# alex-petrenko/megaverse

Hardware: AMD Instinct MI355X
Metric: agent observations/sec (whole node), TowerBuilding 128x128 obs, random policy (higher is better)
Workload: dtype f32

## Files before the change

### include/megaverse_hip.h

```cpp
#ifndef MEGAVERSE_HIP_H
#define MEGAVERSE_HIP_H

#include <stdint.h>

#ifdef __cplusplus
extern "C" {
#endif

typedef struct mv_gym mv_gym;

typedef struct mv_config {
    const char *scenario;
    int32_t obs_width, obs_height;
    int32_t num_envs;
    int32_t num_agents_per_env;
    int32_t num_simulation_threads;
    int32_t use_vulkan;
    int32_t device;
    const char *const *param_keys;
    const float *param_vals;
    int32_t num_params;
    int32_t env_offset, total_envs;
    int32_t env_stride;
} mv_config;
// ... 81 lines not shown
int mv_get_pixel_mode(const mv_gym *g);

enum { MV_OBS_RGBA = 0, MV_OBS_RGB_PLANAR = 1 };
int mv_set_obs_layout(mv_gym *g, int32_t layout);
int mv_get_obs_layout(const mv_gym *g);

int mv_set_pipelining(mv_gym *g, int32_t on);
int mv_get_pipelining(const mv_gym *g);

int mv_set_render_resolution(mv_gym *g, int32_t w, int32_t h);
int mv_draw_hires(mv_gym *g);
int mv_get_hires_observation(mv_gym *g, int32_t env_idx, int32_t agent_idx, uint8_t *out_host);
int mv_draw_overview(mv_gym *g);

int mv_num_reward_shaping_keys(const mv_gym *g);
const char *mv_reward_shaping_key(const mv_gym *g, int32_t i);
int mv_get_reward_shaping(mv_gym *g, int32_t env_idx, int32_t agent_idx, const char *key, float *out);
int mv_set_reward_shaping(mv_gym *g, int32_t env_idx, int32_t agent_idx, const char *key, float value);

int mv_synchronize(mv_gym *g);

typedef struct mv_episode_record {
    int32_t agent;
    int32_t length;
    uint32_t end_tick;
    float true_objective;
    double ret;
} mv_episode_record;
int mv_set_episode_log(mv_gym *g, int32_t capacity);
int mv_get_episode_log_capacity(const mv_gym *g);
int mv_flush_episode_log(mv_gym *g);
int mv_episode_log_count(mv_gym *g, uint32_t *count, uint32_t *dropped);
int mv_drain_episode_log(mv_gym *g, mv_episode_record *out_host, int32_t max_records, uint32_t *dropped);
void *mv_episode_log_records_device_ptr(mv_gym *g);
void *mv_episode_log_count_device_ptr(mv_gym *g);
void *mv_episode_returns_device_ptr(mv_gym *g);
void *mv_episode_lengths_device_ptr(mv_gym *g);
int64_t mv_ticks_since_reset(const mv_gym *g);

int mv_profile_begin(mv_gym *g, int32_t max_steps);
int mv_profile_end(mv_gym *g, float *avg_ms4, int32_t *counts4);

int mv_debug_set_agent_pos(mv_gym *g, int32_t env_idx, int32_t agent_idx, float x, float y, float z);
int mv_debug_launch_counts(mv_gym *g, int64_t out[2]);
int mv_debug_set_agent_yaw(mv_gym *g, int32_t env_idx, int32_t agent_idx, float c, float s);
int mv_debug_set_agent_velocity(mv_gym *g, int32_t env_idx, int32_t agent_idx, float hvx, float hvz, float vvel);
int mv_debug_snapshot_size(const mv_gym *g);
int mv_debug_snapshot(mv_gym *g, int32_t env_idx, void *out_host);
int mv_debug_boxagone_state(mv_gym *g, int32_t env_idx, void *out_host);
int mv_debug_football_state(mv_gym *g, int32_t env_idx, void *out_host);
int mv_debug_set_football_state(mv_gym *g, int32_t env_idx, const void *in_host);
int mv_debug_rng(int32_t device, uint32_t seed, int32_t what, const int32_t *lo, const int32_t *hi, int32_t n, void *out_host);
int mv_debug_math(int32_t device, int32_t what, const float *a, const float *b, int32_t n, float *out_host);
int mv_debug_generate_episode(const char *scenario, int32_t num_agents, int32_t env_seed, int32_t n, float base_episode_len,
                              void *out, int32_t out_bytes);
int mv_debug_feeder_selftest(const char *scenario, int32_t num_envs, int32_t num_agents, int32_t threads, int32_t rounds);
int mv_debug_generate_sokoban(int32_t num_agents, int32_t env_seed, int32_t n, float base_episode_len, void *out, int32_t out_bytes);
int mv_debug_generate_football(int32_t num_agents, int32_t env_seed, int32_t n, float base_episode_len, void *out, int32_t out_bytes);

int mv_debug_collect_draw_host(int32_t num_agents, int32_t env_seed, int32_t n, float base_episode_len, void *out, int32_t out_bytes);
int mv_debug_episode_log_host(const float *rewards, const uint8_t *dones, const float *true_objectives, int32_t k, int32_t N, int32_t A, int32_t capacity,
                              uint32_t first_tick, double *ret, int32_t *len, void *records, uint32_t *count, uint32_t *dropped);
int mv_debug_episode_log_masked_host(const float *rewards, const uint8_t *dones, const float *true_objectives, int32_t k, int32_t N, int32_t A,
                                     int32_t capacity, uint32_t first_tick, double *ret, int32_t *len, void *records, uint32_t *count, uint32_t *dropped,
                                     const uint8_t *step_mask );
int mv_debug_episode_log_budget_host(const float *rewards, const uint8_t *dones, const float *true_objectives, int32_t k, int32_t N, int32_t A,
                                     int32_t capacity, uint32_t first_tick, double *ret, int32_t *len, void *records, uint32_t *count, uint32_t *dropped,
                                     const uint8_t *step_mask , int32_t *left );
int mv_debug_episode_budget_host(const uint8_t *dones, const uint8_t *mask, const int32_t *left_in, int32_t k, int32_t N, uint8_t *steps_out,
                                 int32_t *left_out);
int mv_debug_episode_log_cut_host(const uint8_t *mask, int32_t N, int32_t A, double *ret, int32_t *len);
int mv_debug_fork_plan_host(const int32_t *src_of, int32_t N, int32_t *resolved , int32_t *invalid );
int mv_debug_resample_plan_host(const int32_t *src_of, int32_t N, int32_t *resolved , int32_t *staged ,
                                int32_t *invalid );
int mv_debug_resample_apply_host(const int32_t *src_of, int32_t N, int32_t bytes_per_env, uint8_t *state, int32_t order);
int mv_debug_env_store_plan_host(const int32_t *slot_of, int32_t N, int32_t slots, int32_t is_save, int32_t *resolved , int32_t *invalid );
int64_t mv_debug_env_record_layout_host(const uint32_t *array_bytes, int32_t count, int32_t A, uint32_t *offsets);
int mv_debug_env_record_pack_host(const uint32_t *array_bytes, int32_t count, int32_t A, uint64_t layout_word, int32_t log_on, const uint8_t *env_state_in,
                                  uint8_t *record_out);
int mv_debug_env_record_unpack_host(const uint32_t *array_bytes, int32_t count, int32_t A, uint64_t layout_word, int32_t log_on, const uint8_t *record_in,
                                    uint8_t *env_state_inout);
int mv_debug_episodes_consumed(mv_gym *g, int32_t *out_host);
int mv_debug_collect_draw_device(int32_t device, int32_t num_agents, const int32_t *env_seeds, int32_t count, int32_t n, float base_episode_len, void *out,
                                 int64_t out_bytes, float *ms_per_launch);

#ifdef __cplusplus
}
#endif
#endif
```

### megaverse_amd/csrc/mv_api.hip

```cpp
#include "mv_api_internal.h"

thread_local std::string mvapi::g_err;

static const char *SHAPING_KEYS_TOWER[4] = {"teamSpirit", "towerPickedUpObject", "towerVisitedBuildingZoneWithObject",
                                           "towerBuildingReward"};
static const float SHAPING_DEFAULT_TOWER[4] = {0.1f, 0.1f, 0.1f, 1.0f};
static const char *SHAPING_KEYS_OBST[5] = {"teamSpirit", "obstaclesAgentAtExit", "obstaclesAllAgentsAtExit", "obstaclesExtraReward",
                                          "obstaclesAgentCarriedObjectToExit"};
static const float SHAPING_DEFAULT_OBST[5] = {0.0f, 1.0f, 5.0f, 0.5f, 0.0f};
static const char *SHAPING_KEYS_REARRANGE[3] = {"teamSpirit", "rearrangeOneMoreObjectCorrectPosition", "rearrangeAllObjectsCorrectPosition"};
static const float SHAPING_DEFAULT_REARRANGE[3] = {0.0f, 1.0f, 10.0f};
static const char *SHAPING_KEYS_SOKOBAN[4] = {"teamSpirit", "sokobanBoxOnTarget", "sokobanBoxLeavesTarget", "sokobanAllBoxesOnTarget"};
static const float SHAPING_DEFAULT_SOKOBAN[4] = {0.0f, 1.0f, -1.0f, 10.0f};
static const char *SHAPING_KEYS_EMPTY[1] = {"teamSpirit"};
static const char *SHAPING_KEYS_HEX_MEMORY[3] = {"teamSpirit", "memoryCollectGood", "memoryCollectBad"};
static const float SHAPING_DEFAULT_HEX_MEMORY[3] = {0.0f, 1.0f, -1.0f};
static const char *SHAPING_KEYS_HEX_EXPLORE[2] = {"teamSpirit", "exploreSolved"};
static const float SHAPING_DEFAULT_HEX_EXPLORE[2] = {0.0f, 5.0f};
static const char *SHAPING_KEYS_COLLECT[5] = {"teamSpirit", "collectSingleGood", "collectSingleBad", "collectAll", "collectAbyss"};
static const float SHAPING_DEFAULT_COLLECT[5] = {0.0f, 1.0f, -1.0f, 5.0f, -0.5f};
static const char *SHAPING_KEYS_BOXAGONE[3] = {"teamSpirit", "boxagoneTouchedFloor", "boxagonePerStepReward"};
static const float SHAPING_DEFAULT_BOXAGONE[3] = {0.0f, -0.1f, 0.01f};
static const int ACTION_SPACE[6] = {3, 3, 3, 2, 2, 3};

// ... 278 lines not shown

    mv_gym *g = new mv_gym();
    g->device = cfg->device;
    g->w = cfg->obs_width; g->h = cfg->obs_height;
    g->N = cfg->num_envs; g->A = cfg->num_agents_per_env;
    g->scenario = scenario;
    g->numShaping = scenario == SCN_TOWER || scenario == SCN_SOKOBAN ? 4 : scenario == SCN_REARRANGE || scenario == SCN_HEX_MEMORY || scenario == SCN_BOXAGONE ? 3
                  : scenario == SCN_HEX_EXPLORE ? 2 : scenario == SCN_EMPTY || scenario == SCN_FOOTBALL ? 1 : 5;
    g->shapingKeys = scenario == SCN_TOWER ? SHAPING_KEYS_TOWER : scenario == SCN_OBSTACLES ? SHAPING_KEYS_OBST
                   : scenario == SCN_COLLECT ? SHAPING_KEYS_COLLECT : scenario == SCN_SOKOBAN ? SHAPING_KEYS_SOKOBAN
                   : scenario == SCN_HEX_MEMORY ? SHAPING_KEYS_HEX_MEMORY : scenario == SCN_HEX_EXPLORE ? SHAPING_KEYS_HEX_EXPLORE
                   : scenario == SCN_EMPTY || scenario == SCN_FOOTBALL ? SHAPING_KEYS_EMPTY : scenario == SCN_BOXAGONE ? SHAPING_KEYS_BOXAGONE : SHAPING_KEYS_REARRANGE;
    g->spares = scenario == SCN_TOWER || scenario == SCN_EMPTY || scenario == SCN_FOOTBALL ? 2 : 3;
    g->envOffset = cfg->total_envs > 0 ? cfg->env_offset : 0;
    g->envStride = cfg->total_envs > 0 && cfg->env_stride > 1 ? cfg->env_stride : 1;
    g->gv.sample_on = 0; g->gv.sample_seed = g->gv.sample_step = 0;
    g->gv.env_offset = g->envOffset; g->gv.env_stride = g->envStride;
    g->totalEnvs = cfg->total_envs > 0 ? cfg->total_envs : cfg->num_envs;
    const size_t N = g->N, NA = (size_t)g->N * g->A;

    GymView &gv = g->gv;
    gv.num_envs = g->N; gv.num_agents = g->A;
    const bool obstacles = scenario == SCN_OBSTACLES || scenario == SCN_EMPTY, collect = scenario == SCN_COLLECT,
            rearrange = scenario == SCN_REARRANGE, sokoban = scenario == SCN_SOKOBAN;
    const bool hex = scenario == SCN_HEX_MEMORY || scenario == SCN_HEX_EXPLORE, boxagone = scenario == SCN_BOXAGONE, football = scenario == SCN_FOOTBALL;
    const bool hostEpisodes = obstacles || collect || rearrange || sokoban || hex || boxagone || football;
    gv.scenario = scenario;
    gv.box_stride = collect ? COLLECT_MAX_BOXES : MAX_BOXES;
    gv.reward_stride = collect ? COLLECT_MAX_REWARDS : MAX_REWARDS;
    g->blobBytes = collect ? sizeof(CollectBlob) : obstacles ? sizeof(EpisodeBlob) : rearrange ? sizeof(RearrangeBlob)
                                    : sokoban ? sizeof(SokobanBlob) : hex ? sizeof(HexBlob) : boxagone ? sizeof(BoxAGoneBlob) : football ? sizeof(FootballBlob) : sizeof(TowerBlob);
    auto up = [](size_t v) { return (v + 4095) & ~size_t(4095); };
    const size_t szHdr = up(N * sizeof(EnvHeader)), szBoxes = up(N * (size_t)gv.box_stride * sizeof(LayoutBox)),
                 szObj = up(N * MAX_OBJECTS * sizeof(MovableObject)), szAg = up(NA * sizeof(AgentState)),
                 szChunk = up(N * (size_t)CHUNK_BYTES), szAct = up(NA * sizeof(int32_t)), szRew = up(NA * sizeof(float)),
                 szDone = up(N), szObjv = up(NA * sizeof(float)), szMd = up(NA * 6 * sizeof(int32_t)),
                 szObs = up(NA * frame_bytes(g->w, g->h, MV_OBS_RGBA));
    const size_t szTerrain = obstacles ? up(N * MAX_TERRAIN * sizeof(TerrainBox)) : 0,
                 szRewObj = hostEpisodes ? up(N * (size_t)gv.reward_stride * sizeof(MovableObject)) : 0,
                 szHeight = collect ? up(N * (size_t)HM_BYTES) : 0, szItems = rearrange ? up(N * MAX_ITEMS * sizeof(ArrangementItem))
                                         : 0, szCells = sokoban ? up(N * (size_t)(SOKO_DIM * SOKO_DIM)) : 0,
                 szHexB = hex || boxagone || football ? up(N * (size_t)HEX_MAX_BOXES * sizeof(HexRec)) : 0,
                 szHexO = hex || football ? up(N * (size_t)HEX_MAX_OBJS * sizeof(HexRec)) : 0,
                 szBag = boxagone ? up(N * sizeof(BoxAGoneState)) : 0, szFb = football ? up(N * sizeof(FootballState)) : 0,
                                   szBlobs = up(N * g->blobBytes * (size_t)g->spares), szCnt = up((N + 2) * sizeof(int32_t)),
                                                szGen = hostEpisodes ? 0 : up(N * sizeof(TowerGen));
    gv.vis_stride = hex ? 2048 : collect || boxagone ? 1024 : 256;
    if (const char *e = getenv("MV_DEBUG_VIS_STRIDE")) gv.vis_stride = std::min(gv.vis_stride, std::max(8, atoi(e)));
    gv.debug_redo = getenv("MV_DEBUG_FORCE_REDO") && atoi(getenv("MV_DEBUG_FORCE_REDO")) ? 1 : 0;
    gv.spares = g->spares;
    const size_t szVisP = up(NA * (size_t)gv.vis_stride * 32), szVisR = up(NA * (size_t)gv.vis_stride * 8), szVisC = up(NA * sizeof(int32_t)),
                 szLpt = up(NA * sizeof(int32_t)) + up((NA + 1) * sizeof(int32_t)) + up(NA * (size_t)FRAME_HDR_BYTES)
                            + up((size_t)LPT_BUCKETS * LPT_SUBS * lpt_sub_capacity(NA) * sizeof(int32_t));
    const size_t szParity = szVisP + szVisR + szVisC + szLpt + szRew + szDone + szObjv;
    g->batch = (size_t)PIPE_GROUPS * 16 * szParity <= (size_t(9) << 28) ? 16 : 8;
    if (const char *e = getenv("MV_PIPE_BATCH")) g->batch = std::min((int)PIPE_BATCH_MAX, std::max(1, atoi(e)));
    g->slots = PIPE_GROUPS * g->batch;
    g->hists = g->slots + 1;
    g->histClean.assign((size_t)g->hists, 1);
    g->gvp.resize((size_t)g->slots);
    g->parity = g->slots - 1;
    g->group = PIPE_GROUPS - 1;
    const size_t szHist = up((size_t)g->hists * (LPT_BUCKETS * LPT_SUBS + 1) * sizeof(int32_t));
    gv.lpt_hists = g->hists;
    const bool depthSortOn = !(getenv("MV_DEPTH_SORT") && atoi(getenv("MV_DEPTH_SORT")) == 0);
    const size_t szSort = gv.vis_stride > 256 && depthSortOn ? up(NA * (size_t)gv.vis_stride * 40) : 0;
    const size_t total = szSort + szHdr + szBoxes + szObj + szAg + szAct + szRew + szDone + szObjv + szMd + (hostEpisodes ? 0 : szChunk) + szObs + szTerrain +
                         szRewObj + szHeight + szItems + szCells + szHexB + szHexO + szBag + szFb + szBlobs + szCnt + szGen + (size_t)g->slots * szParity + szHist;
    {
        hipError_t e_ = hipMalloc((void **)&g->arena, total);
        if (e_ != hipSuccess) {
            const int b = g->batch;
            mv_destroy(g);
            return fail("hipMalloc arena (" + std::to_string(total >> 20) + " MiB, of which "
                        + std::to_string(((size_t)PIPE_GROUPS * b * szParity) >> 20) + " MiB are the " +
                        std::to_string(PIPE_GROUPS * b) + " hand-over slots of " + std::to_string(b)
                                       + " ticks per call: a smaller MV_PIPE_BATCH shrinks them): " + hipGetErrorString(e_));
        }
        g->arenaBytes = total;
        (void)hipMemset(g->arena, 0, total);
    }
    {
        uint8_t *p = g->arena;
        gv.hdr = (EnvHeader *)p; p += szHdr;
        gv.boxes = (LayoutBox *)p; p += szBoxes;
        gv.objects = (MovableObject *)p; p += szObj;
        gv.agents = (AgentState *)p; p += szAg;
        gv.actions = (int32_t *)p; p += szAct;
        gv.rewards = (float *)p; p += szRew;
        gv.done = p; p += szDone;
        gv.true_objective = (float *)p; p += szObjv;
        g->dMultiDiscrete = (int32_t *)p; p += szMd;
        if (!hostEpisodes) { gv.chunk = p; p += szChunk; }
        g->ownedObs = (uint32_t *)p; p += szObs;
        g->dStatus = (int *)p; p += szCnt;
        gv.episode_status = g->dStatus;
        if (obstacles) { gv.terrain = (TerrainBox *)p; p += szTerrain; }
        if (hostEpisodes) { gv.rewards_obj = (MovableObject *)p; p += szRewObj; }
        g->dBlobs = p; p += szBlobs;
        gv.blobs = g->dBlobs;
        if (!hostEpisodes) { gv.tower_gen = (TowerGen *)p; p += szGen; }
        if (collect) { gv.heightmap = (int8_t *)p; p += szHeight; }
        if (rearrange) { gv.items = (ArrangementItem *)p; p += szItems; }
        if (sokoban) { gv.soko_cells = p; p += szCells; }
        if (hex) { gv.hex_boxes = (HexRec *)p; p += szHexB; gv.hex_objs = (HexRec *)p; p += szHexO; }
        if (boxagone) { gv.hex_boxes = (HexRec *)p; p += szHexB; gv.bag = (BoxAGoneState *)p; p += szBag; }
        if (football) { gv.hex_boxes = (HexRec *)p; p += szHexB; gv.hex_objs = (HexRec *)p; p += szHexO; gv.fb = (FootballState *)p; p += szFb; }
        {
            fork::Table &ft = g->forkTable;
            ft = fork::Table{};
            ft.hdr = gv.hdr;
            fork::table_add(ft, gv.boxes, (size_t)gv.box_stride * sizeof(LayoutBox));
            fork::table_add(ft, gv.objects, MAX_OBJECTS * sizeof(MovableObject));
            fork::table_add(ft, gv.agents, (size_t)g->A * sizeof(AgentState));
            fork::table_add(ft, gv.chunk, CHUNK_BYTES);
            fork::table_add(ft, gv.terrain, MAX_TERRAIN * sizeof(TerrainBox));
            fork::table_add(ft, gv.rewards_obj, (size_t)gv.reward_stride * sizeof(MovableObject));
            fork::table_add(ft, gv.heightmap, HM_BYTES);
            fork::table_add(ft, gv.items, MAX_ITEMS * sizeof(ArrangementItem));
            fork::table_add(ft, gv.soko_cells, SOKO_DIM * SOKO_DIM);
            fork::table_add(ft, gv.hex_boxes, HEX_MAX_BOXES * sizeof(HexRec));
            fork::table_add(ft, gv.hex_objs, HEX_MAX_OBJS * sizeof(HexRec));
            fork::table_add(ft, gv.bag, sizeof(BoxAGoneState));
            fork::table_add(ft, gv.fb, sizeof(FootballState));
            static_assert(13 + 2 <= fork::MAX_ARRAYS, "the table holds every per-env array and the episode log's two");
        }
        gv.lpt_hist = (int32_t *)p; p += szHist;
        gv.sort_scratch = szSort ? p : nullptr; p += szSort;
        gv.depth_sort = 0;
        for (int q = 0; q < g->slots; ++q) {
            GymView &v = g->gvp[q];
            v = gv;
            v.vis_prims = p; p += szVisP;
            v.vis_rects = p; p += szVisR;
            v.vis_count = (int32_t *)p; p += szVisC;
            v.lpt_bucket = (int32_t *)p; p += up(NA * sizeof(int32_t));
            v.lpt_order = (int32_t *)p; p += up((NA + 1) * sizeof(int32_t));
            v.vis_hdr = p; p += up(NA * (size_t)FRAME_HDR_BYTES);
            v.lpt_list = (int32_t *)p; p += up((size_t)LPT_BUCKETS * LPT_SUBS * lpt_sub_capacity(NA) * sizeof(int32_t));
            v.rewards = (float *)p; p += szRew;
            v.done = p; p += szDone;
            v.true_objective = (float *)p; p += szObjv;
        }
    }
    if (getenv("MV_TICK_TIMING") && atoi(getenv("MV_TICK_TIMING"))) {
        if (hipMalloc((void **)&g->gv.dbg, N * 64 * sizeof(unsigned long long)) == hipSuccess)
            (void)hipMemset(g->gv.dbg, 0, N * 64 * sizeof(unsigned long long));
        else g->gv.dbg = nullptr;
        for (int q = 0; q < g->slots; ++q) g->gvp[q].dbg = g->gv.dbg;
    }
    if (const char *e = getenv("MV_PIXEL_MODE")) g->fastPixels = lower(e) == "exact" ? 0 : 1;
    if (const char *e = getenv("MV_PIPELINE")) g->pipelined = atoi(e) != 0;
    g->obs = g->ownedObs;
    for (int b = 0; b < 2; ++b) {
        if (hipHostMalloc((void **)&g->hActions[b], NA * sizeof(int32_t), hipHostMallocDefault) != hipSuccess ||
            hipEventCreateWithFlags(&g->actionsCopied[b], hipEventDisableTiming) != hipSuccess) {
            mv_destroy(g);
            return fail("mv_create: pinned staging allocation failed");
        }
        std::memset(g->hActions[b], 0, NA * sizeof(int32_t));
    }
    g->hRewards.assign(NA, 0.0f); g->hTrueObj.assign(NA, 0.0f); g->hDone.assign(N, 0);

    float episodeLen = sokoban ? 80.0f : boxagone ? 300.0f : 60.0f, lookLimit = boxagone ? 0.75f : 0.2f;
    for (int k = 0; k < cfg->num_params; ++k) {
        const char *key = cfg->param_keys[k];
        const float v = cfg->param_vals[k];
        if (!std::strcmp(key, "episodeLengthSec")) episodeLen = v;
        if (!std::strcmp(key, "verticalLookLimitRad")) lookLimit = v;
        auto ip = [&](const char *name, int &dst) { if (!std::strcmp(key, name)) dst = int(std::lround(v)); };
        ip("obstaclesMinNumPlatforms", oc.min_platforms); ip("obstaclesMaxNumPlatforms", oc.max_platforms);
        ip("obstaclesMinGap", oc.min_gap); ip("obstaclesMaxGap", oc.max_gap); ip("obstaclesMinLava", oc.min_lava);
        ip("obstaclesMaxLava", oc.max_lava); ip("obstaclesMinHeight", oc.min_height); ip("obstaclesMaxHeight", oc.max_height);
        if (!std::strcmp(key, "obstaclesNumAllowedMaxDifficulty")) oc.num_allowed_max_difficulty = int(v);
    }
    g->obst = oc;
    g->baseEpisodeLen = episodeLen;
    g->envRecordLayout = env_record_layout_word(g, scen, cfg);
    {
        bool ok = hipHostMalloc((void **)&g->hStatus, (N + 2) * sizeof(int), hipHostMallocDefault) == hipSuccess &&
                  hipStreamCreateWithFlags(&g->copyStream, hipStreamNonBlocking) == hipSuccess &&
                  create_sim_stream(&g->simStream) == hipSuccess &&
                  hipEventCreateWithFlags(&g->userMark[0], hipEventDisableTiming) == hipSuccess &&
                  hipEventCreateWithFlags(&g->userMark[1], hipEventDisableTiming) == hipSuccess &&
                  hipEventCreateWithFlags(&g->userMark[2], hipEventDisableTiming) == hipSuccess &&
                  hipEventCreateWithFlags(&g->userNow, hipEventDisableTiming) == hipSuccess &&
                  hipEventCreateWithFlags(&g->simDone, hipEventDisableTiming) == hipSuccess &&
                  hipEventCreateWithFlags(&g->stepDone, hipEventDisableTiming) == hipSuccess &&
                  hipEventCreateWithFlags(&g->statusCopied, hipEventDisableTiming) == hipSuccess;
        if (!ok) {
            mv_destroy(g);
            return fail("mv_create: status staging / copy stream allocation failed");
        }
        std::memset(g->hStatus, 0, (N + 2) * sizeof(int));
    }
// ... 804 lines not shown
```

### megaverse_amd/csrc/mv_api_debug.hip

```cpp
#include "mv_api_internal.h"

__global__ void set_agent_pos_kernel(AgentState *agents, int idx, float x, float y,
                                     float z) { agents[idx].pos[0] = x; agents[idx].pos[1] = y; agents[idx].pos[2] = z; }
__global__ void set_agent_yaw_kernel(AgentState *agents, int idx, float c,
                                     float s) { agents[idx].m00 = c; agents[idx].m02 = s; agents[idx].m20 = -s; agents[idx].m22 = c; }
__global__ void set_agent_velocity_kernel(AgentState *agents, int idx, float hvx, float hvz,
                                          float vvel) { agents[idx].hvx = hvx; agents[idx].hvz = hvz; agents[idx].vvel = vvel; }

__global__ void debug_rng_kernel(uint32_t seed, int what, const int32_t *lo, const int32_t *hi, int n, void *out)
{
    __shared__ uint32_t s_mt[624];
    __shared__ uint16_t s_items[4096];
    Mt19937 g{s_mt, 624};
    mt_seed(g, seed);
    const int lane = threadIdx.x & 63;
    if (what == 0) {
        for (int i = 0; i < n; ++i) { const uint32_t v = mt_next(g); if (lane == 0) ((uint32_t *)out)[i] = v; }
    } else if (what == 1) {
        for (int i = 0; i < n; ++i) { const int v = rand_range(g, lo[i], hi[i]); if (lane == 0) ((int32_t *)out)[i] = v; }
    } else if (what == 2) {
        for (int i = 0; i < n; ++i) { const float v = frand(g); if (lane == 0) ((float *)out)[i] = v; }
    } else if (what == 3) {
        for (int i = lane; i < n; i += 64) s_items[i] = (uint16_t)i;
        __syncthreads();
// ... 326 lines not shown
int mv_debug_generate_sokoban(int32_t num_agents, int32_t env_seed, int32_t n, float base_episode_len, void *out, int32_t out_bytes)
{
    if (!out) return (int)sizeof(SokobanBlob);
    if (num_agents < 1 || num_agents > MAX_AGENTS || n < 1 || (size_t)out_bytes < (size_t)n * sizeof(SokobanBlob))
        return fail("mv_debug_generate_sokoban: bad arguments");
    const std::vector<std::string> files = find_boxoban_level_files();
    if (files.empty()) return fail("mv_debug_generate_sokoban: no Boxoban levels found (BOXOBAN_LEVELS)");
    std::mt19937 rng;
    rng.seed((unsigned long)env_seed);
    SokobanLevels levels;
    for (int i = 0; i < n; ++i)
        if (!generate_sokoban_episode(rng, levels, files, num_agents, base_episode_len, reinterpret_cast<SokobanBlob *>(out)[i]))
            return fail("mv_debug_generate_sokoban: unreadable level file");
    return n;
}

int mv_debug_rng(int32_t device, uint32_t seed, int32_t what, const int32_t *lo, const int32_t *hi, int32_t n, void *out)
{
    HIP_TRY(hipSetDevice(device));
    if (what == 3 && n > 4096) return fail("mv_debug_rng: shuffle n <= 4096");
    int32_t *dlo = nullptr, *dhi = nullptr;
    void *dout = nullptr;
    HIP_TRY(hipMalloc(&dout, (size_t)n * 4));
    if (what == 1) {
        HIP_TRY(hipMalloc((void **)&dlo, (size_t)n * 4));
        HIP_TRY(hipMalloc((void **)&dhi, (size_t)n * 4));
        HIP_TRY(hipMemcpy(dlo, lo, (size_t)n * 4, hipMemcpyHostToDevice));
        HIP_TRY(hipMemcpy(dhi, hi, (size_t)n * 4, hipMemcpyHostToDevice));
    }
    hipLaunchKernelGGL(debug_rng_kernel, dim3(1), dim3(64), 0, nullptr, seed, what, dlo, dhi, n, dout);
    HIP_TRY(hipGetLastError());
    HIP_TRY(hipMemcpy(out, dout, (size_t)n * 4, hipMemcpyDeviceToHost));
    (void)hipFree(dout); (void)hipFree(dlo); (void)hipFree(dhi);
    return 0;
}

int mv_debug_math(int32_t device, int32_t what, const float *a, const float *b, int32_t n, float *out)
{
    HIP_TRY(hipSetDevice(device));
    float *da = nullptr, *db = nullptr, *dout = nullptr;
    const size_t outN = (what == 2) ? 2 * (size_t)n : (size_t)n;
    HIP_TRY(hipMalloc((void **)&da, (size_t)n * 4));
    HIP_TRY(hipMalloc((void **)&db, (size_t)n * 4));
    HIP_TRY(hipMalloc((void **)&dout, outN * 4));
    HIP_TRY(hipMemcpy(da, a, (size_t)n * 4, hipMemcpyHostToDevice));
    HIP_TRY(hipMemcpy(db, b ? b : a, (size_t)n * 4, hipMemcpyHostToDevice));
    hipLaunchKernelGGL(debug_math_kernel, dim3((n + 255) / 256), dim3(256), 0, nullptr, what, da, db, n, dout);
    HIP_TRY(hipGetLastError());
    HIP_TRY(hipMemcpy(out, dout, outN * 4, hipMemcpyDeviceToHost));
    (void)hipFree(da); (void)hipFree(db); (void)hipFree(dout);
    return 0;
}

}
```

### megaverse_amd/csrc/mv_api_step.hip

```cpp
#include "mv_api_internal.h"

extern "C" {

enum : int { QUIET_OFF = 0, QUIET_NONE = 1, QUIET_LAST = 2 };
static int step_gyms(mv_gym *const *gs, int n, bool render, int k, int policy, uint32_t seed, uint32_t first_index, int kCall, int quiet = QUIET_OFF)
{
    mv_gym *const L = gs[0];
    int batch = L->batch;
    bool mustWait = false, allFast = true, anyHostEpisodes = false, anyLog = false;
    for (int i = 0; i < n; ++i) {
        mv_gym *g = gs[i];
        if (check(g)) return -1;
        if (!g->wasReset) return fail("mv_step: call mv_reset first");
        batch = std::min(batch, g->batch);
        mustWait = mustWait || g->simMustWaitUser;
        allFast = allFast && g->fastPixels != 0;
        anyHostEpisodes = anyHostEpisodes || g->hostEpisodes();
        anyLog = anyLog || g->logCapacity > 0;
        if (policy == POLICY_SEQUENCE && (!g->actRing || g->actRingCount < 1))
            return fail(n > 1 ? "mv_group_step: MV_POLICY_SEQUENCE: gym " + std::to_string(i) + " of the group has no action ring (mv_set_action_ring)"
                              : std::string("mv_step_n: MV_POLICY_SEQUENCE: the gym has no action ring (mv_set_action_ring)"));
    }
    if (k < 1 || k > batch) return fail("mv_step_n: 1 <= k <= " + std::to_string(batch) + " (MV_PIPE_BATCH) required");
    HIP_TRY(hipSetDevice(L->device));
// ... 51 lines not shown
    const bool profiling = render && L->profCount < L->profMax;
    hipEvent_t *callEv = nullptr;
    if (profiling && canMultiTick && canBatchRaster && k <= MAX_STEP_TICKS) {
        callEv = &L->profEvents[(size_t)L->profCount * 5];
        L->profTicks[(size_t)L->profCount] = k;
        ++L->profCount;
    }
    const bool multiTick = canMultiTick && (!profiling || callEv);
    bool groupBatch = n > 1 && !ticksOff && own && render && allFast && k >= 2 && k <= MAX_STEP_TICKS && policy != POLICY_NONE
            && !profiling && raster_union_batch_applicable(k, n, L->w, L->h);
    for (int i = 0; i < n && groupBatch; ++i) groupBatch = gs[i]->A == 1 && gs[i]->ringObs && gs[i]->ringCount >= k && !gs[i]->gv.dbg;
    {
        int envs = 0;
        for (int i = 0; i < n; ++i) envs += gs[i]->N;
        groupBatch = groupBatch && envs <= 1024;
    }
    bool sideWaits = anyHostEpisodes;
    for (int i = 0; i < n; ++i)
        sideWaits = sideWaits || (gs[i]->genStream && gs[i]->ticksSinceDraw + k >= gs[i]->drawPeriod) || gs[i]->stepsSinceStatus + k >= gs[i]->statusPeriod;
    bool stepDoneRodeAlong = false;
    for (int j = 0; j < k; ++j) {
        const bool prof = !callEv && render && L->profCount < L->profMax;
        evs[j] = prof ? &L->profEvents[(size_t)L->profCount * 5] : nullptr;
        if (prof) { L->profTicks[(size_t)L->profCount] = 1; ++L->profCount; }
        UnionStepArgs ua;
        ua.n = n;
        int envs = 0;
        for (int i = 0; i < n; ++i) {
            mv_gym *g = gs[i];
            if (policy == POLICY_SEQUENCE) g->gv.sample_on = POLICY_NONE;
            else if (policy != POLICY_NONE) { g->gv.sample_on = policy; g->gv.sample_seed = seed; g->gv.sample_step = first_index + (uint32_t)j; }
            else { g->gv.sample_on = (j == 0 && g->samplePending) ? g->samplePolicy : (int)POLICY_NONE; }
            g->parity = g->group * g->batch + j;
            if ((render || (drawLast && j == k - 1)) && take_hist(g, sim, !(multiTick || groupBatch || simTicks))) return -1;
            OutPtrs &o = outs[(size_t)j * n + i];
            o = outputs_of(g, g->ringTick++);
            GymView &v = views[(size_t)j * n + i];
            v = view(g, g->parity, staged ? nullptr : &o);
            v.step_mask = g->stepMask;
            if (g->budgetOn) { v.budget = g->budgetLeft; v.halted = g->budgetHalted; }
            if (policy == POLICY_SEQUENCE)
                v.md_actions = g->actRing + (size_t)action_ring_entry(first_index, j, (uint32_t)g->actRingCount) * ((size_t)g->N * g->A * 6);
            else if (j == 0 && g->gv.sample_on == POLICY_NONE) v.md_actions = g->mdActions;
            if (groupBatch) v.lpt_no_clear = 1;
            if (n > 1) { ua.first[i] = envs; ua.gv[i] = v; envs += g->N; }
        }
        if (evs[j]) HIP_TRY(hipEventRecord(evs[j][0], sim));
        bool simDoneRides = false;
        if (multiTick) {
            views[(size_t)j].lpt_no_clear = 1;
            if (j == k - 1) {
                if (callEv) HIP_TRY(hipEventRecord(callEv[0], sim));
                hipEvent_t rides = own && !callEv ? L->simDone : nullptr;
                const int chunkTicks = 8;
                for (int j0 = 0; j0 < k; j0 += chunkTicks) {
                    const int kk = std::min(chunkTicks, k - j0);
                    const GymView *vw = views.data() + j0;
                    hipEvent_t r = j0 + kk == k ? rides : nullptr;
                    launch_step_ticks(vw, kk, sim, L->w, L->h, r);
                    ++L->launchCount[0];
                }
                if (callEv) HIP_TRY(hipEventRecord(callEv[1], sim));
                simDoneRides = rides != nullptr;
            }
        } else if (simTicks) {
            if (drawLast && j == k - 1) views[(size_t)j].lpt_no_clear = 1;
            if (j == k - 1) {
                hipEvent_t rides = own ? L->simDone : nullptr;
                const int chunkTicks = 8;
                for (int j0 = 0; j0 < k; j0 += chunkTicks) {
                    const int kk = std::min(chunkTicks, k - j0);
                    const bool last = j0 + kk == k;
                    launch_step_ticks_sim(views.data() + j0, kk, last && drawLast ? 1u << (kk - 1) : 0u, sim, L->w, L->h, last ? rides : nullptr);
                    ++L->launchCount[0];
                }
                simDoneRides = rides != nullptr;
            }
        } else if (n == 1) {
            hipEvent_t rides = j == k - 1 && !evs[j] ? (own ? L->simDone : sideWaits ? L->stepDone : nullptr) : nullptr;
            const bool rode = launch_step(views[(size_t)j * n], sim, L->w, L->h, drawLast && j == k - 1 ? 1 : fused, rides);
            ++L->launchCount[0];
            simDoneRides = rode && own;
            stepDoneRodeAlong = rode && !own;
        }
        else if (groupBatch) {
            if (j == k - 1) {
                UnionTicksArgs ta;
                ta.n = n; ta.k = k;
                ta.act_first = first_index;
                for (int i = 0; i < n; ++i) {
                    ta.first[i] = ua.first[i];
                    ta.gv[i] = views[(size_t)i];
                    ta.slot_stride[i] = (int64_t)((const uint8_t *)views[(size_t)n + i].vis_prims - (const uint8_t *)views[(size_t)i].vis_prims);
                    const bool seq = policy == POLICY_SEQUENCE;
                    ta.act_base[i] = seq ? gs[i]->actRing : nullptr;
                    ta.act_count[i] = seq ? (uint32_t)gs[i]->actRingCount : 0u;
                    ta.act_stride[i] = gs[i]->N * gs[i]->A * 6;
                }
                for (int i = n; i <= MAX_UNION; ++i) ta.first[i] = envs;
                for (int i = n; i < MAX_UNION; ++i) {
                    ta.gv[i] = views[0]; ta.slot_stride[i] = 0;
                    ta.act_base[i] = nullptr; ta.act_count[i] = 0; ta.act_stride[i] = 0;
                }
                launch_step_union_ticks(ta, sim, L->w, L->h, own ? L->simDone : nullptr);
                ++L->launchCount[0];
                simDoneRides = own;
            }
        } else {
            for (int i = n; i <= MAX_UNION; ++i) ua.first[i] = envs;
            launch_step_union(ua, sim, L->w, L->h, fused);
            ++L->launchCount[0];
        }
        if (evs[j]) HIP_TRY(hipEventRecord(evs[j][1], sim));
        simDoneRodeAlong = simDoneRodeAlong || simDoneRides;
// ... 381 lines not shown
```

### megaverse_amd/csrc/mv_raster.h

```cpp
#pragma once
#include <hip/hip_runtime.h>

#include "mv_types.h"

namespace mv {

struct PublishTo { float *rewards; uint8_t *done; float *true_objective; };
int launch_raster(const GymView &gv, uint32_t *obs, int W, int H, hipStream_t stream, hipEvent_t between = nullptr, int fast = 1, int setup_done = 0,
                  const PublishTo *publish = nullptr, hipEvent_t done = nullptr);

int launch_raster_union(const GymView *views, uint32_t *const *obs, const PublishTo *publish, int n,
                        int W, int H, hipStream_t stream, hipEvent_t between = nullptr,
                        hipEvent_t done = nullptr);

int launch_raster_batch(const GymView *views, uint32_t *const *obs, const PublishTo *publish, int k,
                        int W, int H, hipStream_t stream, hipEvent_t done = nullptr);

bool raster_union_batch_applicable(int k, int n, int W, int H);
int launch_raster_union_batch(const GymView *views, uint32_t *const *obs, const PublishTo *publish, int k,
                              int n, int W, int H, hipStream_t stream, hipEvent_t done = nullptr);

}
```

### megaverse_amd/csrc/mv_raster.hip

```cpp
#include <hip/hip_runtime.h>
#include <hip/hip_ext.h>
#include <math.h>
#include <stdlib.h>

#include <algorithm>
#include <cstring>
#include <numeric>
#include <type_traits>
#include <vector>
#include <stdio.h>

#include "../../include/megaverse_hip.h"
#include "mv_frame.h"
#include "mv_math.h"
#include "mv_raster.h"
#include "mv_rearrange.h"
#include "mv_types.h"
#include "mv_union.h"

namespace mv {

namespace {

template <bool ANYZERO>
// ... 168 lines not shown

__device__ __forceinline__ unsigned to_u8(float v)
{
    v = fmin_sel(fmax_sel(v, 0.0f), 1.0f);
    return (unsigned)(int)(v * 255.0f + 0.5f);
}

__device__ __forceinline__ V3 safe_inv(V3 d)
{
    return v3(d.x == 0.0f ? 0.0f : 1.0f / d.x, d.y == 0.0f ? 0.0f : 1.0f / d.y, d.z == 0.0f ? 0.0f : 1.0f / d.z);
}


}


__global__ __launch_bounds__(256) void frame_setup_kernel(GymView gv, int W, int H)
{
    __shared__ FrameScratch s_fs;
    __shared__ DepthSortScratch s_ds;
    frame_setup_body<256, false>(gv, blockIdx.x, W, H, s_fs, &s_ds);
}

__global__ __launch_bounds__(1024) void frame_order_kernel(GymView gv, int frames, int *order)
{
    __shared__ int s_hist[LPT_BUCKETS], s_start[LPT_BUCKETS], s_wsum[LPT_BUCKETS / 64];
    const int tid = threadIdx.x;
    if (tid < LPT_BUCKETS) s_hist[tid] = 0;
    __syncthreads();
    for (int f = tid; f < frames; f += 1024) atomicAdd(&s_hist[gv.lpt_bucket[f]], 1);
    __syncthreads();
    {
        const int lane = tid & 63, wave = tid >> 6;
        const int b = LPT_BUCKETS - 1 - tid;
        const int h = tid < LPT_BUCKETS ? s_hist[b] : 0;
        int x = h;
#pragma unroll
        for (int off = 1; off < 64; off <<= 1) {
            const int y = __shfl_up(x, off, 64);
            if (lane >= off) x += y;
        }
        if (lane == 63 && tid < LPT_BUCKETS) s_wsum[wave] = x;
        __syncthreads();
        if (tid < LPT_BUCKETS) {
            int base = 0;
            for (int w = 0; w < wave; ++w) base += s_wsum[w];
            s_start[b] = base + x - h;
        }
    }
    __syncthreads();
    for (int f = tid; f < frames; f += 1024) order[atomicAdd(&s_start[gv.lpt_bucket[f]], 1)] = f;
}

namespace {

template <bool CHW>
struct PixOutT {
    __amdgpu_buffer_rsrc_t rsrc;
    int W, H, W4;
    bool edgeless;
    int plane;
};
typedef PixOutT<false> PixOut;
#ifndef MV_PIXEL_PLAIN
constexpr int PIXEL_AUX = 2;
#else
constexpr int PIXEL_AUX = 0;
#endif
#ifndef MV_PLANAR_PIXEL_AUX
#define MV_PLANAR_PIXEL_AUX 0
#endif
constexpr int PLANAR_AUX = MV_PLANAR_PIXEL_AUX;

template <bool CHW>
__device__ __forceinline__ PixOutT<CHW> frame_out(uint32_t *obs, int frame, int W, int H, bool edgeless)
{
    PixOutT<CHW> po;
    const unsigned bytes = CHW ? 3u * W * H : 4u * W * H;
    po.rsrc = __builtin_amdgcn_make_buffer_rsrc(reinterpret_cast<unsigned char *>(obs) + (size_t)frame * bytes,  0, (int)bytes, 0x00020000);
    po.W = W; po.H = H; po.W4 = CHW ? W : 4 * W;
    po.edgeless = edgeless;
    po.plane = W * H;
    return po;
}

__device__ __forceinline__ void put_px(const PixOut &po, int px, int py, unsigned rgba)
{
    const unsigned off = (unsigned)(__mul24(py, po.W4) + px * 4);
    if (__builtin_expect(po.edgeless, 1)) __builtin_amdgcn_raw_buffer_store_b32(rgba, po.rsrc, off, 0, PIXEL_AUX);
    else {
        asm volatile("" ::: "memory");
        if (px < po.W && py < po.H) __builtin_amdgcn_raw_buffer_store_b32(rgba, po.rsrc, off, 0, PIXEL_AUX);
    }
}

__device__ __forceinline__ unsigned quad_transpose_bytes(unsigned x, int q)
{
    const unsigned y = (unsigned)__builtin_amdgcn_mov_dpp((int)x, 0x4e, 0xf, 0xf, false);
    const unsigned s = __builtin_amdgcn_perm(y, x, q < 2 ? 0x05040100u : 0x03020706u);
    const unsigned z = (unsigned)__builtin_amdgcn_mov_dpp((int)s, 0xb1, 0xf, 0xf, false);
    return __builtin_amdgcn_perm(z, s, (q & 1) ? 0x03070105u : 0x06020400u);
}

__device__ __forceinline__ void put_px(const PixOutT<true> &po, int px, int py, unsigned rgba)
{
    const unsigned row = (unsigned)__mul24(py, po.W);
    if ((po.W & 3) == 0) {
        const int q = px & 3;
        const unsigned t = quad_transpose_bytes(rgba, q);
        const unsigned off = (unsigned)__mul24(q, po.plane) + row + (unsigned)(px - q);
        if (q < 3 && (po.edgeless || (px < po.W && py < po.H))) __builtin_amdgcn_raw_buffer_store_b32(t, po.rsrc, off, 0, PLANAR_AUX);
        return;
    }
    if (px < po.W && py < po.H) {
        const unsigned off = row + (unsigned)px;
        __builtin_amdgcn_raw_buffer_store_b8((unsigned char)rgba, po.rsrc, off, 0, PLANAR_AUX);
        __builtin_amdgcn_raw_buffer_store_b8((unsigned char)(rgba >> 8), po.rsrc, off + (unsigned)po.plane, 0, PLANAR_AUX);
        __builtin_amdgcn_raw_buffer_store_b8((unsigned char)(rgba >> 16), po.rsrc, off + 2u * (unsigned)po.plane, 0, PLANAR_AUX);
    }
}

}

template <int MAXVIS, bool SHAPES, bool CHW = false>
__global__ __launch_bounds__(256, MAXVIS <= 256 && !SHAPES ? MV_RASTER_WAVES : MAXVIS <= 256 ? 5 : MAXVIS <= 1024 ? 2
                             : 1) void raster_kernel(GymView gv, uint32_t *obs, int W, int H, int split, const int *order)
{
    constexpr int ROUNDS = MAXVIS / 64;
    extern __shared__ __attribute__((aligned(16))) unsigned char s_dyn[];
    __shared__ Prim s_vis[MAXVIS];
    __shared__ short4 s_rect[MAXVIS];
    __shared__ CamL s_cam[MAX_CAMS];
    __shared__ float s_lutA[256], s_lutD[256];

    float4 *s_col = reinterpret_cast<float4 *>(s_dyn);
    float4 *s_row = s_col + W;
    float *s_colinv = reinterpret_cast<float *>(s_row + H);
    float *s_rowinv = s_colinv + W;

    const int A = gv.num_agents;
    int frame, part;
    {
// ... 186 lines not shown
                unsigned ch[3];
#pragma unroll
                for (int c = 0; c < 3; ++c) {
                    const unsigned byte = (q.color >> (16 - 8 * c)) & 255u;
                    ch[c] = to_u8((s_lutA[byte] + s_lutD[byte] * intensity) + spec);
                }
                rgba = ch[0] | (ch[1] << 8) | (ch[2] << 16) | 0xff000000u;
            }
            const int py = pyBase + TILE_H * k;
            if constexpr (CHW) put_px(frame_out<true>(obs, frame, W, H, false), px, py, rgba);
            else if (px < W && py < H) out[(size_t)py * W + px] = rgba;
        }
    }
}

namespace {

#ifndef MV_GLIST_WAVES_NP2
#define MV_GLIST_WAVES_NP2 5
#endif
#ifndef MV_GLIST_WAVES_NP1
#define MV_GLIST_WAVES_NP1 6
#endif
constexpr int GLIST_WAVES_NP2 = MV_GLIST_WAVES_NP2, GLIST_WAVES_NP1 = MV_GLIST_WAVES_NP1;
#ifndef MV_FAST_PPL_DEFAULT
#define MV_FAST_PPL_DEFAULT 2
#endif
constexpr float SPEC_COS2 = 0.97f * 0.97f;

#ifndef MV_PIXEL_PLAIN
#define PIXEL_STORE(dst, v) __builtin_nontemporal_store((uint32_t)(v), &(dst))
#else
#define PIXEL_STORE(dst, v) ((dst) = (v))
#endif

struct FastArgs {
    const unsigned char *vis_hdr;
    const Prim *vis_prims;
    const short4 *vis_rects;
    const int *hist, *list;
    int num_agents, vis_stride, frames;
    const float *stage_rewards, *stage_true;
    const uint8_t *stage_done;
    float *pub_rewards, *pub_true;
    uint8_t *pub_done;
    int pub_n;
#ifdef MV_RASTER_TIMING
    unsigned long long *rdbg;
#endif
    int *hist_done;
    int wg_total;
    int tail_div, tail_split;
    int planar;
};

__device__ __forceinline__ void fast_publish(const FastArgs &fa, int blk)
{
    if (fa.pub_n == 0) return;
    const int i = blk * (int)blockDim.x + (int)threadIdx.x;
    if (i >= fa.pub_n) return;
    fa.pub_rewards[i] = fa.stage_rewards[i];
    const int e = i / fa.num_agents;
    if (fa.stage_done[e]) fa.pub_true[i] = fa.stage_true[i];
    if (i < fa.pub_n / fa.num_agents) fa.pub_done[i] = fa.stage_done[i];
}

__device__ __forceinline__ unsigned long long uniform_u64(unsigned long long v)
{
    const unsigned lo = (unsigned)__builtin_amdgcn_readfirstlane((unsigned)v), hi = (unsigned)__builtin_amdgcn_readfirstlane((unsigned)(v >> 32));
    return ((unsigned long long)hi << 32) | lo;
}

__device__ __forceinline__ float uniform_f32(float v)
{
    return __uint_as_float(__builtin_amdgcn_readfirstlane(__float_as_uint(v)));
}

typedef __attribute__((address_space(3))) const float lds_float;
__device__ __forceinline__ lds_float *local_lds(const float *p)
{
    lds_float *q = (lds_float *)p;
    asm volatile("" : "+v"(q));
    return q;
}
__device__ __forceinline__ V3 lds_tmul(lds_float *m, V3 v)
{
    return v3((m[0] * v.x + m[3] * v.y) + m[6] * v.z, (m[1] * v.x + m[4] * v.y) + m[7] * v.z, (m[2] * v.x + m[5] * v.y) + m[8] * v.z);
}
__device__ __forceinline__ V3 lds_mul(lds_float *m, V3 v)
{
    return v3((m[0] * v.x + m[1] * v.y) + m[2] * v.z, (m[3] * v.x + m[4] * v.y) + m[5] * v.z, (m[6] * v.x + m[7] * v.y) + m[8] * v.z);
}

constexpr unsigned KEY_NEAR = 0x3c23d70au;
constexpr unsigned KEY_FAR = 0x42f00000u - KEY_NEAR;
static_assert(NEAR_Z == 0.01f && FAR_Z == 120.0f, "update KEY_NEAR / KEY_FAR");

template <unsigned POS_MASK>
__device__ __forceinline__ unsigned box_key(V3 inv, const float4 lo, const float4 hi, int pos, unsigned depthMask = ~POS_MASK)
{
    const float t1x = lo.x * inv.x, t2x = hi.x * inv.x, t1y = lo.y * inv.y, t2y = hi.y * inv.y, t1z = lo.z * inv.z, t2z = hi.z * inv.z;
    const float tn = __builtin_fmaxf(__builtin_fmaxf(__builtin_fminf(t1x, t2x), __builtin_fminf(t1y, t2y)), __builtin_fminf(t1z, t2z));
    const float tf = __builtin_fminf(__builtin_fminf(__builtin_fmaxf(t1x, t2x), __builtin_fmaxf(t1y, t2y)), __builtin_fmaxf(t1z, t2z));
    const unsigned key = ((__float_as_uint(tn) - KEY_NEAR) & depthMask) | (unsigned)pos;
    return tn <= tf ? key : ~0u;
}
template <unsigned POS_MASK>
__device__ __forceinline__ unsigned hit_key(bool hit, float t, int pos)
{
    return hit ? (((__float_as_uint(t) - KEY_NEAR) & ~POS_MASK) | (unsigned)pos) : ~0u;
}

__device__ __forceinline__ bool fast_box(V3 inv, const float4 lo, const float4 hi, float &t_out)
{
    const float t1x = lo.x * inv.x, t2x = hi.x * inv.x, t1y = lo.y * inv.y, t2y = hi.y * inv.y, t1z = lo.z * inv.z, t2z = hi.z * inv.z;
    const float tn = __builtin_fmaxf(__builtin_fmaxf(__builtin_fminf(t1x, t2x), __builtin_fminf(t1y, t2y)), __builtin_fminf(t1z, t2z));
    const float tf = __builtin_fminf(__builtin_fminf(__builtin_fmaxf(t1x, t2x), __builtin_fmaxf(t1y, t2y)), __builtin_fmaxf(t1z, t2z));
    t_out = tn;
// ... 86 lines not shown
            const int axis = tnx == t ? 0 : tny == t ? 1 : 2;
            const float dk = axis == 0 ? d.x : axis == 1 ? d.y : d.z;
            const float lk = s_hdr[FH_LREL + 4 * qfr + axis];
            nv = t * __builtin_fabsf(dk);
            ndl = nv - __uint_as_float(__float_as_uint(lk) ^ (__float_as_uint(dk) & 0x80000000u));
        } else {
            t = tkey;
            V3 N;
            lds_float *cc = local_lds(camv + 3);
            if (!SHAPES || qkind < PRIM_SPHERE_S || qfr == 0) N = lds_tmul(cc, bn);
            else if (qfr == 1 + viewer) N = bn;
            else N = lds_tmul(cc, lds_mul(local_lds(s_hdr + FH_CAM + FH_CAM_STRIDE * (qfr - 1) + 3), bn));
            const V3 P = dc * t;
            nv = -dot(N, P);
            ndl = dot(N, v3(0.0f - P.x, 4.0f - P.y, 2.0f - P.z));
        }
        rgba = phong_tail(t, ndl, nv, a2, ldc, float((color >> 16) & 255u), float((color >> 8) & 255u), float(color & 255u));
    }
    return rgba;
}

template <bool SHAPES, unsigned POS_MASK>
__device__ __forceinline__ unsigned fast_shade(unsigned best, V3 bn, const float4 *s_vis, const float *s_hdr, const float *camv,
                                               int viewer, V3 dw, V3 inv, float dcx, float dcy, float a2, float ldc)
{
    unsigned rgba = 0xff000000u;
    if (best <= (KEY_FAR | POS_MASK)) {
        const int pos = (int)(best & POS_MASK);
        rgba = shade_rec<SHAPES>(s_vis[2 * pos], s_vis[2 * pos + 1], __uint_as_float((best & ~POS_MASK) + KEY_NEAR),
                                 bn, s_hdr, camv, viewer, dw, inv, dcx, dcy, a2, ldc);
    }
    return rgba;
}

struct FastFrame { int frame, part, viewer, nVis, split; };

__host__ __device__ inline int tail_frames(int frames, int div) { return (frames / div) & ~7; }

template <int MAXVIS, bool GLIST = false, int NT = 256>
__device__ __forceinline__ FastFrame fast_prologue(const FastArgs &fa, int blk, int W, int H, int split,
                                                   float4 *s_vis, short4 *s_rect, float *s_hdr, float4 *s_col,
                                                   float4 *s_row, float2 *s_rowq, float *s_colq, unsigned char *s_cls = nullptr)
{
    const int A = fa.num_agents;
    const int tid = threadIdx.x, lane = tid & 63, wave = __builtin_amdgcn_readfirstlane(tid >> 6);
    int position, part;
    {
        int b = blk, first = 0, frames = fa.frames;
        if (fa.tail_div) {
            const int q = tail_frames(frames, fa.tail_div), head = frames - q;
            if (b < split * head) frames = head;
            else { b -= split * head; first = head; split = fa.tail_split; frames = q; }
        }
        const int per = 8 * split, group = b / per, r = b - group * per;
        position = group * 8 + (r & 7); part = r >> 3;
        if (group * 8 + 8 > frames) { const int nf = frames - group * 8; position = group * 8 + r % nf; part = r / nf; }
        position += first;
    }
    __shared__ int s_wsum[4], s_frame, s_lastWG;
    {
        static_assert(LPT_SUBS == 4, "the bin's counters are read as one int4");
        const bool binThread = NT == 256 || tid < LPT_BUCKETS;
        const int4 c0 = binThread ? *reinterpret_cast<const int4 *>(fa.hist + (LPT_BUCKETS - 1 - tid) * LPT_SUBS) : make_int4(0, 0, 0, 0);
        const int h = (c0.x + c0.y) + (c0.z + c0.w);
        int x = h;
#pragma unroll
        for (int off = 1; off < 64; off <<= 1) {
            const int y = __shfl_up(x, off, 64);
            if (lane >= off) x += y;
        }
        if (lane == 63 && binThread) s_wsum[wave] = x;
        __syncthreads();
        int base = 0;
        for (int w = 0; w < wave && w < 4; ++w) base += s_wsum[w];
        const int end = base + x, start = end - h;
        if (binThread && position >= start && position < end) {
            const int cs[LPT_SUBS] = {c0.x, c0.y, c0.z, c0.w};
            int off = position - start, sub = 0;
#pragma unroll
            for (int q = 0; q < LPT_SUBS - 1; ++q)
                if (sub == q && off >= cs[q]) { off -= cs[q]; sub = q + 1; }
            s_frame = fa.list[(size_t)((LPT_BUCKETS - 1 - tid) * LPT_SUBS + sub) * lpt_sub_capacity(fa.frames) + off];
        }
        __syncthreads();
    }
#ifdef MV_HIST_FENCE
    if (tid == 0) s_lastWG = fa.hist_done != nullptr && __hip_atomic_fetch_add(fa.hist_done, 1, __ATOMIC_ACQ_REL, __HIP_MEMORY_SCOPE_AGENT) == fa.wg_total - 1;
#else
    if (tid == 0) s_lastWG = fa.hist_done != nullptr && __hip_atomic_fetch_add(fa.hist_done, 1, __ATOMIC_RELAXED, __HIP_MEMORY_SCOPE_AGENT) == fa.wg_total - 1;
#endif
    const int frame = __builtin_amdgcn_readfirstlane(s_frame);
    const int viewer = frame % A;
    const float *gh = reinterpret_cast<const float *>(fa.vis_hdr + (size_t)frame * FRAME_HDR_BYTES);
    const int nVis = __builtin_amdgcn_readfirstlane(min(__float_as_int(gh[FH_COUNT]), (int)MAXVIS));

    if (tid < FH_FLOATS) s_hdr[tid] = gh[tid];
    {
        const float4 *src = reinterpret_cast<const float4 *>(fa.vis_prims + (size_t)frame * fa.vis_stride);
        if (!GLIST) for (int i = tid; i < nVis * 2; i += NT) s_vis[i] = src[i];
        else
            for (int i = tid; i < nVis; i += NT) {
                const unsigned ml = __float_as_uint(reinterpret_cast<const float *>(src)[8 * i + 3]);
                const unsigned fl = (ml >> 4) & 15u;
                s_cls[i] = (ml & 15u) != (unsigned)PRIM_BOX ? 4 : fl == 0u ? 0 : fl > (unsigned)MAX_AGENTS ? (unsigned char)(fl - (unsigned)MAX_AGENTS) : 4;
            }
        const short4 *rs = fa.vis_rects + (size_t)frame * fa.vis_stride;
        for (int i = tid; i < nVis; i += NT) s_rect[i] = rs[i];
        const float *c = gh + FH_CAM + FH_CAM_STRIDE * viewer + 3;
        for (int i = tid; i < W; i += NT) {
            const float dcx = (((float(i) + 0.5f) / float(W)) * 2.0f - 1.0f) * TAN_HALF_FOV;
            s_col[i] = make_float4(dcx, c[0] * dcx, c[3] * dcx, c[6] * dcx);
            s_colq[i] = dcx * dcx;
        }
        for (int j = tid; j < H; j += NT) {
            const float dcy = (((float(j) + 0.5f) / float(H)) * 2.0f - 1.0f) * TAN_HALF_FOV_Y;
            s_row[j] = make_float4(dcy, c[1] * dcy, c[4] * dcy, c[7] * dcy);
            s_rowq[j] = make_float2(dcy * dcy + 1.0f, 4.0f * dcy - 2.0f);
        }
    }
    __syncthreads();
    if (s_lastWG) {
        int *h = const_cast<int *>(fa.hist);
        for (int i = tid; i < LPT_BUCKETS * LPT_SUBS; i += NT) h[i] = 0;
        if (tid == 0) __hip_atomic_store(fa.hist_done, 0, __ATOMIC_RELAXED, __HIP_MEMORY_SCOPE_AGENT);
    }

    return FastFrame{frame, part, viewer, nVis, split};
}

template <unsigned POS_MASK, int SGN>
__device__ __forceinline__ unsigned box_key_signed(V3 inv, const float4 lo, const float4 hi, int pos, unsigned depthMask)
{
    const float nx = (SGN & 1) ? hi.x : lo.x, fx = (SGN & 1) ? lo.x : hi.x, ny = (SGN & 2) ? hi.y : lo.y, fy = (SGN & 2)
                      ? lo.y : hi.y, nz = (SGN & 4) ? hi.z : lo.z, fz = (SGN & 4) ? lo.z : hi.z;
    const float tn = __builtin_fmaxf(__builtin_fmaxf(nx * inv.x, ny * inv.y), nz * inv.z);
    const float tf = __builtin_fminf(__builtin_fminf(fx * inv.x, fy * inv.y), fz * inv.z);
    const unsigned key = ((__float_as_uint(tn) - KEY_NEAR) & depthMask) | (unsigned)pos;
    return tn <= tf ? key : ~0u;
}

template <unsigned POS_MASK, int NP, int SGN = -1>
__device__ __forceinline__ void box_run(unsigned long long m, int k, const V3 (&inv)[NP], const float4 *s_vis, unsigned (&best)[NP])
{
    if (!m) return;
    int p0 = __ffsll((long long)m) - 1 + 64 * k, p1 = 0;
    m &= m - 1;
    float4 lo0 = s_vis[2 * p0], hi0 = s_vis[2 * p0 + 1], lo1 = lo0, hi1 = hi0;
    unsigned depthMask = ~POS_MASK;
    asm volatile("" : "+v"(depthMask));
    for (;;) {
        bool more = m != 0ull;
        if (more) { p1 = __ffsll((long long)m) - 1 + 64 * k; m &= m - 1; lo1 = s_vis[2 * p1]; hi1 = s_vis[2 * p1 + 1]; }
#pragma unroll
        for (int j = 0; j < NP; ++j) best[j] = min(best[j], SGN >= 0 ? box_key_signed<POS_MASK, (SGN >= 0 ? SGN : 0)>(inv[j], lo0, hi0, p0, depthMask)
             : box_key<POS_MASK>(inv[j], lo0, hi0, p0, depthMask));
        if (!more) break;
        more = m != 0ull;
        if (more) { p0 = __ffsll((long long)m) - 1 + 64 * k; m &= m - 1; lo0 = s_vis[2 * p0]; hi0 = s_vis[2 * p0 + 1]; }
#pragma unroll
        for (int j = 0; j < NP; ++j) best[j] = min(best[j], SGN >= 0 ? box_key_signed<POS_MASK, (SGN >= 0 ? SGN : 0)>(inv[j], lo1, hi1, p1, depthMask)
             : box_key<POS_MASK>(inv[j], lo1, hi1, p1, depthMask));
        if (!more) break;
    }
}

}

constexpr float PLANAR_MARGIN = 2e-4f;
enum : unsigned { TC_EMPTY = 0, TC_PLANAR = 1, TC_PLANAR_SPEC = 2, TC_OVERLAY = 3, TC_GENERAL = 4 };
constexpr int CLS_MAX_TILES = 128;

template <int TH, int NT>
__device__ __forceinline__ void classify_tiles(uint4 *s_tile, float4 *s_line, const float4 *s_vis, const short4 *s_rect,
                                               const float *s_hdr, const float *camv, int nVis, unsigned long long wb0,
                                               int W, int H, int part, int split, int tilesX, int numTiles,
                                                       int perWG, bool overlayOn, int *s_cnt, unsigned *s_txy, bool bulkClear)
{
    constexpr int NW = NT / 64;
    constexpr int PPR = 16 / NW;
    const int tid = threadIdx.x, lane = tid & 63, wave = __builtin_amdgcn_readfirstlane(tid >> 6);
    if (tid < CLS_MAX_TILES) s_tile[tid] = make_uint4(0u, 0u, 0u, 0u);
    if (tid < 8) s_cnt[tid] = 0;
    const float sx = 2.0f * TAN_HALF_FOV / float(W), ox = (1.0f / float(W) - 1.0f) * TAN_HALF_FOV;
    const float sy = 2.0f * TAN_HALF_FOV_Y / float(H), oy = (1.0f / float(H) - 1.0f) * TAN_HALF_FOV_Y;
    const int q = lane & 15, es = lane >> 4;
    const int ek = min(q >> 2, 2);
    int em = ek + 1 + ((q >> 1) & 1);
    em = em >= 3 ? em - 3 : em;
    const bool ehi = q & 1, eactive = q < 12;
    const float Ak = camv[3 + 3 * ek] * sx, Bk = camv[4 + 3 * ek] * sy, Ck = (camv[3 + 3 * ek] * ox + camv[4 + 3 * ek] * oy) - camv[5 + 3 * ek];
    const float Am = camv[3 + 3 * em] * sx, Bm = camv[4 + 3 * em] * sy, Cm = (camv[3 + 3 * em] * ox + camv[4 + 3 * em] * oy) - camv[5 + 3 * em];
    float4 *myLines = s_line + 16 * PPR * wave;
    constexpr float WX = float(TILE_W - 1), WY = float(TH - 1);
    __syncthreads();
    constexpr int CH = CLS_MAX_TILES / 64;
    int tX0[CH], tY0[CH], tX1[CH], tY1[CH];
    bool tvalid[CH];
    unsigned mlo[CH], mhi[CH], cover[CH];
#pragma unroll
    for (int c = 0; c < CH; ++c) {
        const int u = 64 * c + lane;
        const int tile = ((u >> 2) * split + part) * 4 + (u & 3);
        tvalid[c] = u < perWG && tile < numTiles;
        const int tyi = tile / tilesX, txi = tile - tyi * tilesX;
        tX0[c] = txi * TILE_W; tY0[c] = tyi * TH;
        tX1[c] = min(tX0[c] + TILE_W, W) - 1; tY1[c] = min(tY0[c] + TH, H) - 1;
        mlo[c] = mhi[c] = cover[c] = 0u;
    }
    for (int base = PPR * wave; base < nVis; base += 16) {
        const int P = min(base + min(es, PPR - 1), nVis - 1);
        const bool isBox = es < PPR && base + es < nVis && ((wb0 >> P) & 1ull) != 0ull;
        const float4 lo4 = s_vis[2 * P], hi4 = s_vis[2 * P + 1];
        const float lok = ek == 0 ? lo4.x : ek == 1 ? lo4.y : lo4.z, hik = ek == 0 ? hi4.x : ek == 1 ? hi4.y : hi4.z;
        const float lom = em == 0 ? lo4.x : em == 1 ? lo4.y : lo4.z, him = em == 0 ? hi4.x : em == 1 ? hi4.y : hi4.z;
        const float bnd = ehi ? him : lom;
        const bool cand = isBox && eactive && (lok > 0.0f || hik < 0.0f);
        const float pk = lok > 0.0f ? lok : hik;
        const float far1 = (__builtin_fmaxf(__builtin_fabsf(lo4.x), __builtin_fabsf(hi4.x)) + __builtin_fmaxf(__builtin_fabsf(lo4.y), __builtin_fabsf(hi4.y))) +
                           __builtin_fmaxf(__builtin_fabsf(lo4.z), __builtin_fabsf(hi4.z));
        const bool coverOK = cand && __builtin_fabsf(pk) >= 4.0f * NEAR_Z && far1 <= 0.5f * FAR_Z;
        const float sg = ((pk > 0.0f) != ehi) ? 1.0f : -1.0f;
        const float ea = sg * (pk * Am - bnd * Ak), eb = sg * (pk * Bm - bnd * Bk), ec = sg * (pk * Cm - bnd * Ck);
        const float mg = PLANAR_MARGIN * (__builtin_fabsf(pk) + __builtin_fabsf(bnd));
        const float cin = ((ec + __builtin_fminf(0.0f, ea * WX)) + __builtin_fminf(0.0f, eb * WY)) - mg;
        const float span = (__builtin_fabsf(ea) * WX + __builtin_fabsf(eb) * WY) + 2.0f * mg;
        if (es < PPR) myLines[lane] = cand ? make_float4(ea, eb, cin, span) : make_float4(0.0f, 0.0f, -1.0f, 0.0f);
        const unsigned long long candMask = __ballot(cand), coverMask = __ballot(coverOK);
        __builtin_amdgcn_fence(__ATOMIC_RELEASE, "wavefront");
        __builtin_amdgcn_wave_barrier();
        __builtin_amdgcn_fence(__ATOMIC_ACQUIRE, "wavefront");
#pragma unroll
        for (int sl = 0; sl < PPR; ++sl) {
            const int Q = base + sl;
            if (Q >= nVis) break;
            const uint2 rr = *reinterpret_cast<const uint2 *>(&s_rect[Q]);
            const bool worldBox = (wb0 >> Q) & 1ull;
#pragma unroll
            for (int c = 0; c < CH; ++c) {
                if (64 * c >= perWG) break;
                const bool ov = tvalid[c] & ((int)(rr.x & 0xffffu) <= tX1[c]) & ((int)(rr.x >> 16) >= tX0[c])
                                             & ((int)(rr.y & 0xffffu) <= tY1[c]) & ((int)(rr.y >> 16) >= tY0[c]);
                if (!__any(ov)) continue;
                bool hit = ov;
                unsigned cov = 0u;
                if (worldBox) {
                    const float fx0 = float(tX0[c]), fy0 = float(tY0[c]);
                    bool missAll = true;
#pragma unroll
                    for (int f = 0; f < 3; ++f) {
                        if (!((candMask >> (16 * sl + 4 * f)) & 1ull)) continue;
                        bool ins = true, mis = false;
#pragma unroll
                        for (int e = 0; e < 4; ++e) {
                            const float4 L = myLines[16 * sl + 4 * f + e];
                            const float g = __builtin_fmaf(L.x, fx0, __builtin_fmaf(L.y, fy0, L.z));
                            ins = ins && g >= 0.0f;
                            mis = mis || g + L.w <= 0.0f;
                        }
                        if (ins && ((coverMask >> (16 * sl + 4 * f)) & 1ull)) cov = (unsigned)f + 1u;
// ... 45 lines not shown
                        const float plane = lok > 0.0f ? lok : hik;
                        const float m0 = k == 0 ? 2.0f * plane - L0 : L0, m1 = k == 1 ? 2.0f * plane - L1 : L1, m2 = k == 2 ? 2.0f * plane - L2 : L2;
                        const float xc = float(tX0[c]) + 0.5f * WX, yc = float(tY0[c]) + 0.5f * WY;
                        const float dcx = sx * xc + ox, dcy = sy * yc + oy;
                        const float d0 = (camv[3] * dcx + camv[4] * dcy) - camv[5], d1 = (camv[6] * dcx + camv[7] * dcy) - camv[8],
                                          d2 = (camv[9] * dcx + camv[10] * dcy) - camv[11];
                        const float dot = (d0 * m0 + d1 * m1) + d2 * m2;
                        const float dd = (d0 * d0 + d1 * d1) + d2 * d2, mm = (m0 * m0 + m1 * m1) + m2 * m2;
                        maybe = dot > 0.0f && dot * dot >= cosT2 * (dd * mm);
                    }
                    info = (maybe ? (unsigned)TC_PLANAR_SPEC : (unsigned)TC_PLANAR) | ((unsigned)k << 3) | ((unsigned)pos << 5);
                } else if ((others & nonBox) == 0ull && overlayOn) info = (unsigned)TC_OVERLAY | ((unsigned)k << 3) | ((unsigned)pos << 5);
            }
            if (info == TC_GENERAL) {
                const float xa = float(tX0[c]), xb = float(tX1[c]), ya = float(tY0[c]), yb = float(tY1[c]);
                unsigned sg = 8u;
#pragma unroll
                for (int a = 0; a < 3; ++a) {
                    const float Aa = camv[3 + 3 * a] * sx, Ba = camv[4 + 3 * a] * sy, Ca = (camv[3 + 3 * a] * ox + camv[4 + 3 * a] * oy) - camv[5 + 3 * a];
                    const float v00 = __builtin_fmaf(Aa, xa, __builtin_fmaf(Ba, ya, Ca)), v10 = __builtin_fmaf(Aa, xb, __builtin_fmaf(Ba, ya, Ca));
                    const float v01 = __builtin_fmaf(Aa, xa, __builtin_fmaf(Ba, yb, Ca)), v11 = __builtin_fmaf(Aa, xb, __builtin_fmaf(Ba, yb, Ca));
                    const float lo4 = __builtin_fminf(__builtin_fminf(v00, v10), __builtin_fminf(v01, v11)),
                                                      hi4 = __builtin_fmaxf(__builtin_fmaxf(v00, v10), __builtin_fmaxf(v01, v11));
                    if (hi4 < -1e-4f) sg |= 1u << a;
                    else if (!(lo4 > 1e-4f)) sg = 0u;
                    if (sg == 0u) break;
                }
                info |= sg << 11;
            }
            s_tile[u].w = info;
            const unsigned tclass = info & 7u, cat = tclass == TC_GENERAL ? 0u : tclass == TC_OVERLAY ? 1u
                    : tclass == TC_PLANAR_SPEC ? 2u : tclass == TC_PLANAR ? 3u : 4u;
            const bool runs = tclass == TC_PLANAR || tclass == TC_PLANAR_SPEC || (tclass == TC_EMPTY && !bulkClear);
            const unsigned txy = (unsigned)tX0[c] | ((unsigned)tY0[c] << 16);
            const unsigned prevInfo = (unsigned)__shfl_up((int)info, 1, 64), prevTxy = (unsigned)__shfl_up((int)txy, 1, 64);
            const bool natHead = !runs || lane == 0 || prevInfo != info || prevTxy + (unsigned)TILE_W != txy;
            const unsigned long long nat = __ballot(natHead), below = nat & ((2ull << lane) - 1ull);
            const int posInRun = lane - (63 - __clzll((long long)below));
            const bool head = natHead || (posInRun & 7) == 0;
            const unsigned long long heads = __ballot(head), valid = __ballot(true), above = lane < 63 ? heads >> (lane + 1) : 0ull;
            const int nextHead = above ? lane + __ffsll((long long)above) : 64;
            const int len = min(nextHead, (int)__popcll(valid)) - lane;
            s_tile[u].z = head ? cat | ((unsigned)len << 3) | ((unsigned)atomicAdd(&s_cnt[cat], 1) << 7) : 7u;
            s_txy[u] = txy;
        }
        __syncthreads();
    }
}

template <int NP, bool SPEC, class PO>
__device__ __forceinline__ void planar_run(int pos, int k, int n, const float4 *s_vis, const float *s_hdr, const float4 *s_col, const float4 *s_row,
                                           const float2 *s_rowq, const float *s_colq, float nzk, int tx0, int ty0, int lane, const PO &po)
{
    const int W = po.W, H = po.H;
    const float lok = uniform_f32(reinterpret_cast<const float *>(s_vis)[8 * pos + k]),
                                  hik = uniform_f32(reinterpret_cast<const float *>(s_vis)[8 * pos + 4 + k]);
    const float plane = lok > 0.0f ? lok : hik;
    const unsigned color = (unsigned)__builtin_amdgcn_readfirstlane(__float_as_uint(reinterpret_cast<const float *>(s_vis)[8 * pos + 7]));
    const float cr = float((color >> 16) & 255u), cg = float((color >> 8) & 255u), cb = float(color & 255u);
    const float lk = uniform_f32(s_hdr[FH_LREL + k]);
    const float lks = plane > 0.0f ? lk : 0.0f - lk;
    int lpx = lane;
    asm volatile("" : "+v"(lpx));
    const int lx = lpx & (TILE_W - 1), py0 = ty0 + lpx / TILE_W;
    float rowk[NP];
    float2 rq[NP];
#pragma unroll
    for (int j = 0; j < NP; ++j) {
        const int pyc = min(py0 + TILE_H * j, H - 1);
        rowk[j] = reinterpret_cast<const float *>(s_row)[4 * pyc + 1 + k];
        rq[j] = s_rowq[pyc];
    }
#pragma unroll 1
    for (int q = 0; q < n; ++q) {
        const int px = tx0 + TILE_W * q + lx, pxc = min(px, W - 1);
        const float colk = reinterpret_cast<const float *>(s_col)[4 * pxc + 1 + k];
        const float cq = s_colq[pxc];
#pragma unroll
        for (int j = 0; j < NP; ++j) {
            const float dk = (colk + rowk[j]) + nzk;
            const float t = plane * __builtin_amdgcn_rcpf(dk);
            const float nv = t * __builtin_fabsf(dk);
            const unsigned rgba = phong_tail<SPEC>(t, nv - lks, nv, cq + rq[j].x, rq[j].y, cr, cg, cb);
            put_px(po, px, py0 + TILE_H * j, rgba);
        }
    }
}

template <int NP, bool SPEC, class PO>
__device__ __forceinline__ void planar_tile(int pos, int k, const float4 *s_vis, const float *s_hdr, const float4 *s_col, const float4 *s_row,
                                            const float2 *s_rowq, const float *s_colq, float nzk, int px, int py0, const PO &po)
{
    const int W = po.W, H = po.H;
    const float lok = uniform_f32(reinterpret_cast<const float *>(s_vis)[8 * pos + k]),
                                  hik = uniform_f32(reinterpret_cast<const float *>(s_vis)[8 * pos + 4 + k]);
    const float plane = lok > 0.0f ? lok : hik;
    const unsigned color = (unsigned)__builtin_amdgcn_readfirstlane(__float_as_uint(reinterpret_cast<const float *>(s_vis)[8 * pos + 7]));
    const float cr = float((color >> 16) & 255u), cg = float((color >> 8) & 255u), cb = float(color & 255u);
    const float lk = uniform_f32(s_hdr[FH_LREL + k]);
    const float lks = plane > 0.0f ? lk : 0.0f - lk;
    const int pxc = min(px, W - 1);
    const float colk = reinterpret_cast<const float *>(s_col)[4 * pxc + 1 + k];
    const float cq = s_colq[pxc];
#pragma unroll
    for (int j = 0; j < NP; ++j) {
        const int py = py0 + TILE_H * j, pyc = min(py, H - 1);
        const float rowk = reinterpret_cast<const float *>(s_row)[4 * pyc + 1 + k];
        const float2 rq = s_rowq[pyc];
        const float dk = (colk + rowk) + nzk;
        const float t = plane * __builtin_amdgcn_rcpf(dk);
        const float nv = t * __builtin_fabsf(dk);
        const unsigned rgba = phong_tail<SPEC>(t, nv - lks, nv, cq + rq.x, rq.y, cr, cg, cb);
        put_px(po, px, py, rgba);
    }
}

typedef unsigned v4u_t __attribute__((ext_vector_type(4)));
template <int NP>
__device__ __forceinline__ void clear_tile(const PixOut &po, int tx0, int ty0, int lane)
{
    constexpr int TH = TILE_H * NP;
    unsigned c = 0xff000000u;
    asm volatile("" : "+v"(lane), "+v"(c));
    if ((po.W & 3) == 0 && tx0 + TILE_W <= po.W) {
        const int row = ty0 + (lane >> 2), col = tx0 + 4 * (lane & 3);
        const v4u_t v = {c, c, c, c};
        if (lane < 4 * TH && row < po.H) __builtin_amdgcn_raw_buffer_store_b128(v, po.rsrc, (unsigned)(__mul24(row, po.W4) + col * 4), 0, PIXEL_AUX);
        return;
    }
    const int px = tx0 + (lane & (TILE_W - 1)), py0 = ty0 + lane / TILE_W;
#pragma unroll
    for (int j = 0; j < NP; ++j) {
        const int py = py0 + TILE_H * j;
        if (px < po.W && py < po.H) __builtin_amdgcn_raw_buffer_store_b32(c, po.rsrc, (unsigned)(__mul24(py, po.W4) + px * 4), 0, PIXEL_AUX);
    }
}
template <int NP>
__device__ __forceinline__ void clear_tile(const PixOutT<true> &po, int tx0, int ty0, int lane)
{
    constexpr int TH = TILE_H * NP;
    if ((po.W & 15) == 0 && tx0 + TILE_W <= po.W) {
        const int c = lane / TH, row = ty0 + (lane - c * TH);
        const v4u_t z = {0u, 0u, 0u, 0u};
        if (c < 3 && row < po.H)
            __builtin_amdgcn_raw_buffer_store_b128(z, po.rsrc, (unsigned)(__mul24(c, po.plane) + __mul24(row, po.W) + tx0), 0, PLANAR_AUX);
        return;
    }
    const int px = tx0 + (lane & (TILE_W - 1)), py0 = ty0 + lane / TILE_W;
#pragma unroll
    for (int j = 0; j < NP; ++j) put_px(po, px, py0 + TILE_H * j, 0xff000000u);
}

template <bool SHAPES, unsigned POS_MASK, int NP, class PO>
__device__ __forceinline__ void overlay_tile(int posA, int k, unsigned long long rest, const float4 *s_vis,
                                             const float *s_hdr, const float *camv, int viewer, const float4 *s_col,
                                             const float4 *s_row, const float2 *s_rowq, const float *s_colq,
                                                     float nzm0, float nzm1, float nzm2, int px, int py0, const PO &po)
{
    const int W = po.W, H = po.H;
    const float lok = uniform_f32(reinterpret_cast<const float *>(s_vis)[8 * posA + k]),
                                  hik = uniform_f32(reinterpret_cast<const float *>(s_vis)[8 * posA + 4 + k]);
    const float plane = lok > 0.0f ? lok : hik;
    const unsigned color = (unsigned)__builtin_amdgcn_readfirstlane(__float_as_uint(reinterpret_cast<const float *>(s_vis)[8 * posA + 7]));
    const float cr = float((color >> 16) & 255u), cg = float((color >> 8) & 255u), cb = float(color & 255u);
    const float lk = uniform_f32(s_hdr[FH_LREL + k]);
    const float lks = plane > 0.0f ? lk : 0.0f - lk;
    const int pxc = min(px, W - 1);
    const float4 cx = s_col[pxc];
    const float cq = s_colq[pxc];
#pragma unroll
    for (int j = 0; j < NP; ++j) {
        const int py = py0 + TILE_H * j, pyc = min(py, H - 1);
        const float4 ry = s_row[pyc];
        const float2 rq = s_rowq[pyc];
        const V3 dw = v3((cx.y + ry.y) + nzm0, (cx.z + ry.z) + nzm1, (cx.w + ry.w) + nzm2);
        const float dk = k == 0 ? dw.x : k == 1 ? dw.y : dw.z;
        const float t = plane * __builtin_amdgcn_rcpf(dk);
        const unsigned keyA = ((__float_as_uint(t) - KEY_NEAR) & ~POS_MASK) | (unsigned)posA;
        unsigned best = keyA;
        unsigned long long m = rest;
        while (m) {
            const int pos = __ffsll((long long)m) - 1;
            m &= m - 1;
            const float4 lo = s_vis[2 * pos], hi = s_vis[2 * pos + 1];
            const int qfr = (int)((__builtin_amdgcn_readfirstlane(__float_as_uint(lo.w)) >> 4) & 15);
            float tb;
            const bool hit = other_box(lo, hi, qfr, s_hdr, viewer, dw, cx.x, ry.x, tb);
            best = min(best, hit_key<POS_MASK>(hit, tb, pos));
        }
        const float a2 = cq + rq.x, ldc = rq.y;
        unsigned rgba;
        if (best == keyA) {
            const float nv = t * __builtin_fabsf(dk);
            rgba = phong_tail<true>(t, nv - lks, nv, a2, ldc, cr, cg, cb);
        } else rgba = fast_shade<SHAPES, POS_MASK>(best, v3(0.0f, 0.0f, 0.0f), s_vis, s_hdr, camv, viewer, dw, v3(0.0f, 0.0f, 0.0f), cx.x, ry.x, a2, ldc);
        put_px(po, px, py, rgba);
    }
}

template <bool SHAPES, unsigned POS_MASK, int NP, class PO>
__device__ __forceinline__ void general_tile(unsigned long long mv0, unsigned long long wb0, unsigned signs, const float4 *s_vis,
                                             const float *s_hdr, const float *camv, int viewer, const float4 *s_col,
                                             const float4 *s_row, const float2 *s_rowq, const float *s_colq,
                                                     float nzm0, float nzm1, float nzm2, int px, int py0, const PO &po)
{
    const int W = po.W, H = po.H;
    const int pxc = min(px, W - 1);
    const float4 cx = s_col[pxc];
    const float cq = s_colq[pxc];
    const float dcx = cx.x;
    V3 dw[NP], inv[NP], bn[NP];
    float dcy[NP], a2[NP], ldc[NP];
    unsigned best[NP];
#pragma unroll
    for (int j = 0; j < NP; ++j) {
        const int pyc = min(py0 + TILE_H * j, H - 1);
        const float4 ry = s_row[pyc];
        const float2 rq = s_rowq[pyc];
        dcy[j] = ry.x;
        dw[j] = v3((cx.y + ry.y) + nzm0, (cx.z + ry.z) + nzm1, (cx.w + ry.w) + nzm2);
        inv[j] = v3(__builtin_amdgcn_rcpf(dw[j].x), __builtin_amdgcn_rcpf(dw[j].y), __builtin_amdgcn_rcpf(dw[j].z));
        a2[j] = cq + rq.x; ldc[j] = rq.y;
        bn[j] = v3(0.0f, 0.0f, 0.0f);
        best[j] = ~0u;
    }
    const unsigned long long wbm = mv0 & wb0;
    switch (signs) {
    case 8: box_run<POS_MASK, NP, 0>(wbm, 0, inv, s_vis, best); break;
    case 9: box_run<POS_MASK, NP, 1>(wbm, 0, inv, s_vis, best); break;
    case 10: box_run<POS_MASK, NP, 2>(wbm, 0, inv, s_vis, best); break;
    case 11: box_run<POS_MASK, NP, 3>(wbm, 0, inv, s_vis, best); break;
    case 12: box_run<POS_MASK, NP, 4>(wbm, 0, inv, s_vis, best); break;
    case 13: box_run<POS_MASK, NP, 5>(wbm, 0, inv, s_vis, best); break;
    case 14: box_run<POS_MASK, NP, 6>(wbm, 0, inv, s_vis, best); break;
    case 15: box_run<POS_MASK, NP, 7>(wbm, 0, inv, s_vis, best); break;
    default: box_run<POS_MASK, NP>(wbm, 0, inv, s_vis, best); break;
    }
    unsigned long long rest = mv0 & ~wb0;
    while (rest) {
        const int pos = __ffsll((long long)rest) - 1;
        rest &= rest - 1;
#pragma unroll
        for (int j = 0; j < NP; ++j) {
            V3 n = v3(0, 0, 0);
            const unsigned key = fast_other<SHAPES, POS_MASK>(pos, s_vis, s_hdr, camv, viewer, dw[j], dcx, dcy[j], n);
            if (key < best[j]) { best[j] = key; bn[j] = n; }
        }
    }
#pragma unroll
    for (int j = 0; j < NP; ++j) {
        const unsigned rgba = fast_shade<SHAPES, POS_MASK>(best[j], bn[j], s_vis, s_hdr, camv, viewer, dw[j], inv[j], dcx, dcy[j], a2[j], ldc[j]);
        put_px(po, px, py0 + TILE_H * j, rgba);
    }
}

constexpr int fast_lds_bytes(int maxvis) { return 40 * maxvis + 4 * FH_FLOATS; }
constexpr int glist_lds_bytes(int maxvis) { return 9 * maxvis + 4 * FH_FLOATS; }

#ifdef MV_RASTER_TIMING
#define RT_COUNT(i, n) do { const unsigned long long n_ = (unsigned long long)(n); if (fa.rdbg && lane == 0) atomicAdd(fa.rdbg + (size_t)16384 * 4 * 8 + (i), n_); } while (0)
#else
#define RT_COUNT(i, n) do { } while (0)
#endif
template <bool SHAPES, unsigned POS_MASK, int NP, bool LISTED, class PO>
__device__ __forceinline__ void classified_tile(const FastArgs &fa, const int u, const int tx0, const int ty0, const uint4 *s_tile,
                                                const float4 *s_vis, const float *s_hdr, const float *camv, int viewer,
                                            const float4 *s_col, const float4 *s_row, const float2 *s_rowq,
                                                    const float *s_colq, float nzm0, float nzm1, float nzm2, unsigned long long wb0,
                                            int lane, const PO &po)
{
    const unsigned info = (unsigned)__builtin_amdgcn_readfirstlane(s_tile[u].w), tclass = info & 7u;
    const int run = LISTED ? (int)(((unsigned)__builtin_amdgcn_readfirstlane(s_tile[u].z) >> 3) & 15u) : 1;
    RT_COUNT(0, run);
    if (tclass == TC_EMPTY) {
        RT_COUNT(1, run);
        for (int q = 0; q < run; ++q) clear_tile<NP>(po, tx0 + TILE_W * q, ty0, lane);
        return;
    }
    if (LISTED && tclass <= TC_PLANAR_SPEC) {
        const int k = (int)((info >> 3) & 3u), posA = (int)(info >> 5);
        const float nzk = k == 0 ? nzm0 : k == 1 ? nzm1 : nzm2;
        RT_COUNT(2, run);
        RT_COUNT(12, tclass == TC_PLANAR ? run : 0);
        if (tclass == TC_PLANAR) planar_run<NP, false>(posA, k, run, s_vis, s_hdr, s_col, s_row, s_rowq, s_colq, nzk, tx0, ty0, lane, po);
        else planar_run<NP, true>(posA, k, run, s_vis, s_hdr, s_col, s_row, s_rowq, s_colq, nzk, tx0, ty0, lane, po);
        return;
    }
    int lpx = lane;
    asm volatile("" : "+v"(lpx));
    const int px = tx0 + (lpx & (TILE_W - 1)), py0 = ty0 + lpx / TILE_W;
    if (tclass <= TC_OVERLAY) {
#if defined(MV_RASTER_DEBUG_SKIP) && MV_RASTER_DEBUG_SKIP == 3
        return;
#endif
        const int k = (int)((info >> 3) & 3u), posA = (int)(info >> 5);
        const float nzk = k == 0 ? nzm0 : k == 1 ? nzm1 : nzm2;
        RT_COUNT(2, tclass != TC_OVERLAY);
        RT_COUNT(12, tclass == TC_PLANAR);
        RT_COUNT(13, tclass == TC_OVERLAY);
        if (tclass == TC_PLANAR) planar_tile<NP, false>(posA, k, s_vis, s_hdr, s_col, s_row, s_rowq, s_colq, nzk, px, py0, po);
        else if (tclass == TC_PLANAR_SPEC) planar_tile<NP, true>(posA, k, s_vis, s_hdr, s_col, s_row, s_rowq, s_colq, nzk, px, py0, po);
        else {
            const uint2 tm = *reinterpret_cast<const uint2 *>(&s_tile[u]);
            const unsigned long long others = (((unsigned long long)(unsigned)__builtin_amdgcn_readfirstlane(tm.y) << 32)
                                               | (unsigned)__builtin_amdgcn_readfirstlane(tm.x)) & ~wb0;
            overlay_tile<SHAPES, POS_MASK, NP>(posA, k, others, s_vis, s_hdr, camv, viewer, s_col, s_row, s_rowq, s_colq, nzm0, nzm1, nzm2, px, py0, po);
        }
        return;
    }
#if defined(MV_RASTER_DEBUG_SKIP) && MV_RASTER_DEBUG_SKIP == 2
    return;
#endif
    const uint2 tm = *reinterpret_cast<const uint2 *>(&s_tile[u]);
    const unsigned long long mv0 = ((unsigned long long)(unsigned)__builtin_amdgcn_readfirstlane(tm.y) << 32) | (unsigned)__builtin_amdgcn_readfirstlane(tm.x);
    RT_COUNT(4, 1);
    RT_COUNT(5, __popcll(mv0 & wb0));
    RT_COUNT(6, __popcll(mv0 & ~wb0));
    general_tile<SHAPES, POS_MASK, NP>(mv0, wb0, fa.planar == 3 ? 0u : (info >> 11) & 15u, s_vis, s_hdr, camv,
                                       viewer, s_col, s_row, s_rowq, s_colq, nzm0, nzm1, nzm2, px, py0, po);
}

template <int MAXVIS, bool SHAPES, bool HEXF, int NP, bool CLS = true, int NT = 256, bool CHW = false>
__device__ __forceinline__ void raster_fast_body(const FastArgs &fa, uint32_t *obs, int W, int H, int split, int blk, unsigned char *lds)
{
    constexpr unsigned POS_MASK = MAXVIS - 1;
    constexpr int TH = TILE_H * NP;
    extern __shared__ __attribute__((aligned(16))) unsigned char s_dyn[];
    float4 *s_vis = reinterpret_cast<float4 *>(lds);
    short4 *s_rect = reinterpret_cast<short4 *>(lds + 32 * MAXVIS);
    float *s_hdr = reinterpret_cast<float *>(lds + 40 * MAXVIS);
    static_assert(MAXVIS / 64 <= 16, "world-box masks: 16 x 64 positions");

    float4 *s_col = reinterpret_cast<float4 *>(s_dyn);
    float4 *s_row = s_col + W;
    float2 *s_rowq = reinterpret_cast<float2 *>(s_row + H);
    float *s_colq = reinterpret_cast<float *>(s_rowq + H);

    const int tid = threadIdx.x, lane = tid & 63, wave = __builtin_amdgcn_readfirstlane(tid >> 6);
#ifdef MV_RASTER_TIMING
    unsigned long long rt_[6];
    rt_[0] = __builtin_amdgcn_s_memtime(); rt_[5] = __builtin_amdgcn_s_memrealtime();
#define RT_MARK(i) rt_[i] = __builtin_amdgcn_s_memtime()
#else
#define RT_MARK(i) do { } while (0)
#endif
    fast_publish(fa, blk);
    const FastFrame ff = fast_prologue<MAXVIS, false, NT>(fa, blk, W, H, split, s_vis, s_rect, s_hdr, s_col, s_row, s_rowq, s_colq);
    RT_MARK(1);
    const int frame = ff.frame, part = ff.part, viewer = ff.viewer, nVis = ff.nVis;
    split = ff.split;

    const float *camv = s_hdr + FH_CAM + FH_CAM_STRIDE * viewer;
    const float nzm0 = uniform_f32(-camv[3 + 2]), nzm1 = uniform_f32(-camv[3 + 5]), nzm2 = uniform_f32(-camv[3 + 8]);
    uint32_t *out = obs + (size_t)frame * W * H;
    const int tilesX = (W + TILE_W - 1) / TILE_W, tilesY = (H + TH - 1) / TH;
    const int numTiles = tilesX * tilesY;
    PixOutT<CHW> po;
    if constexpr (CHW) po = frame_out<true>(obs, frame, W, H, (W % TILE_W) == 0 && (H % TH) == 0);
    else {
        po.rsrc = __builtin_amdgcn_make_buffer_rsrc(out,  0, W * H * 4, 0x00020000);
        po.W = W; po.H = H; po.W4 = 4 * W;
        po.edgeless = (W % TILE_W) == 0 && (H % TH) == 0;
    }

    uint2 rr0 = make_uint2(0u, 0u);
    if (NP == 1) rr0 = *reinterpret_cast<const uint2 *>(&s_rect[min(lane, max(nVis - 1, 0))]);
    const unsigned long long wb0 = uniform_u64(*reinterpret_cast<const unsigned long long *>(s_hdr + FH_WB));

    constexpr bool PLANAR = !HEXF && CLS;
    static_assert(!PLANAR || (MAXVIS == 256 && CLS_MAX_TILES == 128), "classification tables: 256 edge functions + 128 tiles = 192 records");
    float4 *s_line = s_vis + 2 * 64;
    uint4 *s_tile = reinterpret_cast<uint4 *>(s_vis + 2 * 64 + 256);
    const int perWG = (numTiles - part * 4 + 4 * split - 1) / (4 * split) * 4;
    const bool cls = PLANAR && fa.planar && nVis <= 64 && perWG <= CLS_MAX_TILES && perWG >= 32;
    __shared__ int s_next;
    __shared__ int s_cnt[8];
    __shared__ unsigned s_txy[CLS_MAX_TILES];
    __shared__ unsigned short s_order[CLS_MAX_TILES], s_empty[CLS_MAX_TILES];
    if (tid == 0) s_next = NT / 64;
    int nList = 0;
#ifndef MV_TILE_LIST
#define MV_TILE_LIST 1
#endif
    constexpr bool LISTED = PLANAR && MV_TILE_LIST != 0;
    const bool bulk = LISTED && po.edgeless && (W & 3) == 0;
    if (PLANAR && cls && !LISTED) classify_tiles<TH, NT>(s_tile, s_line, s_vis, s_rect, s_hdr, camv, nVis, wb0, W, H,
        part, split, tilesX, numTiles, perWG, fa.planar != 2, s_cnt, s_txy, true);
    else if (PLANAR && cls) {
        classify_tiles<TH, NT>(s_tile, s_line, s_vis, s_rect, s_hdr, camv, nVis, wb0, W, H, part, split,
                               tilesX, numTiles, perWG, fa.planar != 2, s_cnt, s_txy, bulk);
        const int c0 = s_cnt[0], c1 = s_cnt[1], c2 = s_cnt[2], c3 = s_cnt[3], nE = s_cnt[4];
        nList = __builtin_amdgcn_readfirstlane(c0 + c1 + c2 + c3 + (bulk ? 0 : nE));
        if (tid < CLS_MAX_TILES) {
            const int tile = ((tid >> 2) * split + part) * 4 + (tid & 3);
            if (tid < perWG && tile < numTiles) {
                const unsigned z = s_tile[tid].z, cat = z & 7u, place = z >> 7;
                const int base = cat == 0u ? 0 : cat == 1u ? c0 : cat == 2u ? c0 + c1 : cat == 3u ? c0 + c1 + c2 : c0 + c1 + c2 + c3;
                if (cat == 4u && bulk) s_empty[place] = (unsigned short)tid;
                else if (cat != 7u) s_order[base + (int)place] = (unsigned short)tid;
            }
        }
        __syncthreads();
        if (bulk) {
            constexpr int CPT = TH * 4;
            static_assert(NT % CPT == 0, "threads per empty tile");
            const int sub = tid % CPT;
            unsigned c = 0xff000000u;
            asm volatile("" : "+v"(c));
            const v4u_t v = {c, c, c, c};
            if constexpr (CHW) {
                const v4u_t z = {0u, 0u, 0u, 0u};
                const int c = sub / TH;
                const unsigned inoff = (unsigned)__mul24(c, po.plane) + (unsigned)__mul24(sub - c * TH, po.W);
                if (c < 3)
                    for (int e = tid / CPT; e < nE; e += NT / CPT) {
                        const unsigned txy = s_txy[s_empty[e]];
                        __builtin_amdgcn_raw_buffer_store_b128(z, po.rsrc, (unsigned)__mul24((int)(txy >> 16), po.W) + (txy & 0xffffu) + inoff, 0, PLANAR_AUX);
                    }
            } else {
            const unsigned inoff = (unsigned)__mul24(sub >> 2, po.W4) + (unsigned)(sub & 3) * 16u;
            for (int e = tid / CPT; e < nE; e += NT / CPT) {
                const unsigned txy = s_txy[s_empty[e]];
                __builtin_amdgcn_raw_buffer_store_b128(v, po.rsrc, (unsigned)__mul24((int)(txy >> 16), po.W4) + (txy & 0xffffu) * 4u + inoff, 0, PIXEL_AUX);
            }
            }
            if (wave == 0) { RT_COUNT(0, nE); RT_COUNT(1, nE); }
        }
    } else __syncthreads();
    RT_MARK(2);
#if defined(MV_RASTER_DEBUG_SKIP) && MV_RASTER_DEBUG_SKIP == 1
    return;
#endif

    int unext = 0;
    if (LISTED && cls)
        for (int it = wave; it < nList; it = __builtin_amdgcn_readfirstlane(unext)) {
            const int u = __builtin_amdgcn_readfirstlane((int)s_order[it]);
            if (lane == 0) unext = atomicAdd(&s_next, 1);
            const unsigned txy = (unsigned)__builtin_amdgcn_readfirstlane(s_txy[u]);
            classified_tile<SHAPES, POS_MASK, NP, LISTED>(fa, u, (int)(txy & 0xffffu), (int)(txy >> 16), s_tile, s_vis, s_hdr,
                                                          camv, viewer, s_col, s_row, s_rowq, s_colq, nzm0, nzm1, nzm2, wb0, lane, po);
        }
    const unsigned tilesXinv = (unsigned)((0x100000000ull + (unsigned)tilesX - 1u) / (unsigned)tilesX);
    for (int u = wave; !(LISTED && cls); u = __builtin_amdgcn_readfirstlane(unext)) {
        const int tile = ((u >> 2) * split + part) * 4 + (u & 3);
        if (tile >= numTiles) break;
        if (lane == 0) unext = atomicAdd(&s_next, 1);
        const int ty = (int)__umulhi((unsigned)tile, tilesXinv), tx = tile - ty * tilesX;
        const int tx0 = tx * TILE_W, ty0 = ty * TH;
        const int tx1 = min(tx0 + TILE_W, W) - 1, ty1 = min(ty0 + TH, H) - 1;
        if (PLANAR && !LISTED && cls) {
            classified_tile<SHAPES, POS_MASK, NP, LISTED>(fa, u, tx0, ty0, s_tile, s_vis, s_hdr, camv, viewer,
                                                          s_col, s_row, s_rowq, s_colq, nzm0, nzm1, nzm2, wb0, lane, po);
            continue;
        }
        unsigned long long mv0;
        int lpx = lane;
        asm volatile("" : "+v"(lpx));
        const int px = tx0 + (lpx & (TILE_W - 1)), py0 = ty0 + lpx / TILE_W;
        const int pxc = min(px, W - 1);
        {
            int l2 = lane;
            asm volatile("" : "+v"(l2));
            const int cpos = min(l2, max(nVis - 1, 0));
            const uint2 rr = NP == 1 ? rr0 : *reinterpret_cast<const uint2 *>(&s_rect[cpos]);
            const bool v = (lane < nVis) & ((int)(rr.x & 0xffffu) <= tx1) & ((int)(rr.x >> 16) >= tx0)
                            & ((int)(rr.y & 0xffffu) <= ty1) & ((int)(rr.y >> 16) >= ty0);
            mv0 = __ballot(v);
            RT_COUNT(3, 1);
        }
        RT_COUNT(4, 1);
        RT_COUNT(5, __popcll(mv0 & wb0));
        RT_COUNT(6, __popcll(mv0 & ~wb0));
        V3 dw[NP], inv[NP];
        V3 ih0[NP], ih1[NP], ih2[NP];
        float dcx = 0.0f, dcy[NP], a2[NP], ldc[NP];
        unsigned best[NP];
        V3 bn[NP];
#pragma unroll
        for (int j = 0; j < NP; ++j) {
            dw[j] = inv[j] = bn[j] = v3(0, 0, 0);
            ih0[j] = ih1[j] = ih2[j] = v3(0, 0, 0);
            dcy[j] = a2[j] = ldc[j] = 0.0f;
            best[j] = ~0u;
        }
        bool rayReady = false;
#pragma unroll 1
        for (int k = 0; k * 64 < nVis; ++k) {
            const int cpos = min(lane + 64 * k, nVis - 1);
            unsigned long long mvis = mv0;
            bool v = (mv0 >> lane) & 1ull;
            if (k > 0) {
                const uint2 rr = *reinterpret_cast<const uint2 *>(&s_rect[cpos]);
                v = (lane + 64 * k < nVis) & ((int)(rr.x & 0xffffu) <= tx1) & ((int)(rr.x >> 16) >= tx0)
                     & ((int)(rr.y & 0xffffu) <= ty1) & ((int)(rr.y >> 16) >= ty0);
                mvis = __ballot(v);
            }
            if (mvis == 0ull) continue;
            if (!rayReady) {
                rayReady = true;
                const float4 cx = s_col[pxc];
                const float cq = s_colq[pxc];
                dcx = cx.x;
#pragma unroll
                for (int j = 0; j < NP; ++j) {
                    const int pyc = min(py0 + TILE_H * j, H - 1);
                    const float4 ry = s_row[pyc];
                    const float2 rq = s_rowq[pyc];
                    dcy[j] = ry.x;
                    dw[j] = v3((cx.y + ry.y) + nzm0, (cx.z + ry.z) + nzm1, (cx.w + ry.w) + nzm2);
                    inv[j] = v3(__builtin_amdgcn_rcpf(dw[j].x), __builtin_amdgcn_rcpf(dw[j].y), __builtin_amdgcn_rcpf(dw[j].z));
                    a2[j] = cq + rq.x; ldc[j] = rq.y;
                    if (HEXF) {
                        const float cx8 = 0.8660254f * dw[j].x, cz8 = 0.8660254f * dw[j].z, hx5 = 0.5f * dw[j].x, hz5 = 0.5f * dw[j].z;
                        ih0[j] = v3(__builtin_amdgcn_rcpf(cx8 - hz5), inv[j].y, __builtin_amdgcn_rcpf(hx5 + cz8));
                        ih1[j] = v3(__builtin_amdgcn_rcpf(cx8 + hz5), inv[j].y, __builtin_amdgcn_rcpf(cz8 - hx5));
                        ih2[j] = v3(0.0f - inv[j].z, inv[j].y, inv[j].x);
                    }
                }
            }
            unsigned long long rest;
            if (HEXF) {
                const unsigned ml = __float_as_uint(s_vis[2 * cpos].w);
                const bool box = v && (ml & 15u) == (unsigned)PRIM_BOX;
                const unsigned fl = (ml >> 4) & 15u;
                const unsigned long long m0 = __ballot(box && fl == 0u), m1 = __ballot(box && fl == (unsigned)MAX_AGENTS + 1u),
                                         m2 = __ballot(box && fl == (unsigned)MAX_AGENTS + 2u), m3 = __ballot(box && fl == (unsigned)MAX_AGENTS + 3u);
                box_run<POS_MASK, NP>(m0, k, inv, s_vis, best);
                box_run<POS_MASK, NP>(m1, k, ih0, s_vis, best);
                box_run<POS_MASK, NP>(m2, k, ih1, s_vis, best);
                box_run<POS_MASK, NP>(m3, k, ih2, s_vis, best);
                rest = mvis & ~(m0 | m1 | m2 | m3);
            } else {
                const unsigned long long wb = k == 0 ? wb0 : uniform_u64(*reinterpret_cast<const unsigned long long *>(s_hdr + FH_WB + 2 * k));
                box_run<POS_MASK, NP>(mvis & wb, k, inv, s_vis, best);
                rest = mvis & ~wb;
            }
            while (rest) {
                const int pos = __ffsll((long long)rest) - 1 + 64 * k;
                rest &= rest - 1;
#pragma unroll
                for (int j = 0; j < NP; ++j) {
                    V3 n = v3(0, 0, 0);
                    const unsigned key = fast_other<SHAPES, POS_MASK>(pos, s_vis, s_hdr, camv, viewer, dw[j], dcx, dcy[j], n);
                    if (key < best[j]) { best[j] = key; bn[j] = n; }
                }
            }
        }
#pragma unroll
        for (int j = 0; j < NP; ++j) {
            RT_COUNT(7, __ballot(best[j] <= (KEY_FAR | POS_MASK)) != 0ull);
            RT_COUNT(8, __popcll(__ballot(best[j] <= (KEY_FAR | POS_MASK))));
            RT_COUNT(9, __ballot(best[j] <= (KEY_FAR | POS_MASK) && !((wb0 >> (best[j] & 63u)) & 1ull)) != 0ull);
            const unsigned rgba = fast_shade<SHAPES, POS_MASK>(best[j], bn[j], s_vis, s_hdr, camv, viewer, dw[j], inv[j], dcx, dcy[j], a2[j], ldc[j]);
            put_px(po, px, py0 + TILE_H * j, rgba);
        }
    }
#ifdef MV_RASTER_TIMING
    if (fa.rdbg && lane == 0 && blk < 16384 / (NT / 256)) {
// ... 205 lines not shown
#endif
            more = false;
#pragma unroll 1
            for (++k; k * 64 < nVis; ++k) {
                if (depthSorted && k < 31) {
                    const unsigned wd = (unsigned)__builtin_amdgcn_readfirstlane(__float_as_uint(s_hdr[FH_WB + k]));
                    const float floorD = __uint_as_float(((wd & 63u) + (120u << 2)) << 21) * (1.0f - 1e-4f);
                    const unsigned bound = floorD > NEAR_Z ? __float_as_uint(floorD) - KEY_NEAR : 0u;
                    bool covered = true;
#pragma unroll
                    for (int j = 0; j < NP; ++j) covered = covered && (best[j].d < bound || px >= W || py0 + GT_H * j >= H);
                    if (__all(covered)) { RT_COUNT(15, 1); break; }
                }
                RT_COUNT(11, 1);
                mvis = cull_round_g(s_rect, lane, k, nVis, tx0, tx1, ty0, ty1, cpos, v);
                if (mvis) { more = true; break; }
            }
        }
#ifdef MV_RASTER_TIMING
        RT_COUNT(9, metTotal == 1 && metWorld == 1);
        RT_COUNT(8, metTotal == 2);
        RT_COUNT(7, metTotal >= 3 && metTotal <= 5);
        RT_COUNT(6, metTotal >= 6);
#endif
#pragma unroll
        for (int j = 0; j < NP; ++j) {
            unsigned rgba = 0xff000000u;
#if defined(MV_GLIST_DEBUG_SKIP) && MV_GLIST_DEBUG_SKIP >= 1
            rgba = best[j].d ^ best[j].p;
            if (false)
#else
            if (best[j].d <= KEY_FAR)
#endif
            {
                const unsigned wpos = best[j].p & 2047u;
                const float4 lo = gp[2 * wpos], hi = gp[2 * wpos + 1];
                rgba = shade_rec<SHAPES>(lo, hi, __uint_as_float(best[j].d + KEY_NEAR), bn[j], s_hdr, camv, viewer, dw[j], inv[j], dcx, dcy[j], a2[j], ldc[j]);
            }
            RT_COUNT(3, __popcll(__ballot(best[j].d <= KEY_FAR)));
            const int py = py0 + GT_H * j;
            if constexpr (CHW) put_px(pc, px, py, rgba);
            else if (px < W && py < H) PIXEL_STORE(out[(unsigned)(py * W + px)], rgba);
        }
    }
}

template <int MAXVIS, bool SHAPES, int WAVES, bool HEXF, int NP, bool CHW = false>
__global__ __launch_bounds__(256, WAVES) void raster_glist_kernel(FastArgs fa, uint32_t *obs, int W, int H, int split)
{
    __shared__ __attribute__((aligned(16))) unsigned char s_buf[glist_lds_bytes(MAXVIS)];
    raster_glist_body<MAXVIS, SHAPES, HEXF, NP, CHW>(fa, obs, W, H, split, (int)blockIdx.x, s_buf);
}

template <int MAXVIS, bool SHAPES, int WAVES, bool HEXF = false, int NP = 1, int NT = 256, bool CHW = false>
__global__ __launch_bounds__(NT, WAVES) void raster_fast_kernel(FastArgs fa, uint32_t *obs, int W, int H, int split)
{
    __shared__ __attribute__((aligned(16))) unsigned char s_buf[fast_lds_bytes(MAXVIS)];
    raster_fast_body<MAXVIS, SHAPES, HEXF, NP, true, NT, CHW>(fa, obs, W, H, split, (int)blockIdx.x, s_buf);
}

struct UnionRasterArgs {
    int32_t n;
    int32_t first[MAX_UNION + 1];
    uint32_t *obs[MAX_UNION];
    FastArgs fa[MAX_UNION];
};

template <int MAXVIS, bool SHAPES, int WAVES, bool HEXF, int NP, bool CHW = false>
__global__ __launch_bounds__(256, WAVES) void raster_fast_union_kernel(UnionRasterArgs ua, int W, int H, int split)
{
    int s = 0;
#pragma unroll
    for (int i = 1; i < MAX_UNION; ++i)
        if (i < ua.n && (int)blockIdx.x >= ua.first[i]) s = i;
    __shared__ __attribute__((aligned(16))) unsigned char s_buf[fast_lds_bytes(MAXVIS)];
    raster_fast_body<MAXVIS, SHAPES, HEXF, NP, true, 256, CHW>(ua.fa[s], ua.obs[s], W, H, split, (int)blockIdx.x - ua.first[s], s_buf);
}

struct TicksRasterArgs {
    int32_t k, per_tick;
    int32_t hists, parity0;
    int64_t slot_stride;
    const int *hist_base;
    int *done_base;
    uint32_t *obs[MAX_STEP_TICKS];
    float *pub_rewards[MAX_STEP_TICKS];
    uint8_t *pub_done[MAX_STEP_TICKS];
    FastArgs fa;
};

__device__ __forceinline__ FastArgs ticks_raster_args(const TicksRasterArgs &a, int t)
{
    FastArgs f = a.fa;
    const int64_t d = a.slot_stride * t;
    f.vis_hdr += d;
    f.vis_prims = reinterpret_cast<const Prim *>(reinterpret_cast<const unsigned char *>(f.vis_prims) + d);
    f.vis_rects = reinterpret_cast<const short4 *>(reinterpret_cast<const unsigned char *>(f.vis_rects) + d);
    f.list = reinterpret_cast<const int *>(reinterpret_cast<const unsigned char *>(f.list) + d);
    f.stage_rewards = reinterpret_cast<const float *>(reinterpret_cast<const unsigned char *>(f.stage_rewards) + d);
    f.stage_true = reinterpret_cast<const float *>(reinterpret_cast<const unsigned char *>(f.stage_true) + d);
    f.stage_done += d;
    const int par = (a.parity0 + t) % a.hists;
    f.hist = a.hist_base + par * (LPT_BUCKETS * LPT_SUBS);
    f.hist_done = a.done_base ? a.done_base + par : nullptr;
    f.pub_rewards = a.pub_rewards[t];
    f.pub_done = a.pub_done[t];
    return f;
}

template <int MAXVIS, bool SHAPES, int WAVES, int NP, int NT = 256, bool CHW = false>
__global__ __launch_bounds__(NT, WAVES) void raster_fast_batch_kernel(TicksRasterArgs a, int W, int H, int split)
{
    int j = 0, r = (int)blockIdx.x;
    while (r >= a.per_tick) { r -= a.per_tick; ++j; }
    if (j == 0)
        for (int t = 0; t < a.k; ++t) fast_publish(ticks_raster_args(a, t), r);
    __shared__ __attribute__((aligned(16))) unsigned char s_buf[fast_lds_bytes(MAXVIS)];
    FastArgs fa = ticks_raster_args(a, j);
    fa.pub_n = 0;
    raster_fast_body<MAXVIS, SHAPES, false, NP, true, NT, CHW>(fa, a.obs[j], W, H, split, r, s_buf);
}

template <int MAXVIS, bool SHAPES, int WAVES, bool HEXF, int NP, bool CHW = false>
__global__ __launch_bounds__(256, WAVES) void raster_glist_batch_kernel(TicksRasterArgs a, int W, int H, int split)
{
    int j = 0, r = (int)blockIdx.x;
    while (r >= a.per_tick) { r -= a.per_tick; ++j; }
    if (j == 0)
        for (int t = 0; t < a.k; ++t) fast_publish(ticks_raster_args(a, t), r);
    __shared__ __attribute__((aligned(16))) unsigned char s_buf[glist_lds_bytes(MAXVIS)];
    FastArgs fa = ticks_raster_args(a, j);
    fa.pub_n = 0;
    raster_glist_body<MAXVIS, SHAPES, HEXF, NP, CHW>(fa, a.obs[j], W, H, split, r, s_buf);
}

template <int MAXVIS, bool SHAPES, int WAVES, bool HEXF, int NP, bool CHW = false>
__global__ __launch_bounds__(256, WAVES) void raster_glist_union_kernel(UnionRasterArgs ua, int W, int H, int split)
{
    int s = 0;
#pragma unroll
    for (int i = 1; i < MAX_UNION; ++i)
        if (i < ua.n && (int)blockIdx.x >= ua.first[i]) s = i;
    __shared__ __attribute__((aligned(16))) unsigned char s_buf[glist_lds_bytes(MAXVIS)];
    raster_glist_body<MAXVIS, SHAPES, HEXF, NP, CHW>(ua.fa[s], ua.obs[s], W, H, split, (int)blockIdx.x - ua.first[s], s_buf);
}

struct UnionRasterAllArgs {
    UnionRasterArgs u;
    int32_t large[MAX_UNION];
    int32_t split_small, split_large;
};

#ifndef MV_UNION_CLS
#define MV_UNION_CLS (NPS >= 2)
#endif
template <int WAVES, int NPS, bool CHW = false>
__global__ __launch_bounds__(256, WAVES) void raster_union_all_kernel(UnionRasterAllArgs a, int W, int H)
{
    int s = 0;
#pragma unroll
    for (int i = 1; i < MAX_UNION; ++i)
        if (i < a.u.n && (int)blockIdx.x >= a.u.first[i]) s = i;
    constexpr int LDS = fast_lds_bytes(VIS_SMALL) > glist_lds_bytes(VIS_XL) ? fast_lds_bytes(VIS_SMALL) : glist_lds_bytes(VIS_XL);
    __shared__ __attribute__((aligned(16))) unsigned char s_buf[LDS];
    const int blk = (int)blockIdx.x - a.u.first[s];
    if (a.large[s]) raster_glist_body<VIS_XL, true, true, 1, CHW>(a.u.fa[s], a.u.obs[s], W, H, a.split_large, blk, s_buf);
    else raster_fast_body<VIS_SMALL, true, false, NPS, MV_UNION_CLS, 256, CHW>(a.u.fa[s], a.u.obs[s], W, H, a.split_small, blk, s_buf);
}

struct UnionBatchArgs {
    int32_t n, k, per_tick;
    int32_t first[MAX_UNION + 1];
    int32_t large[MAX_UNION];
// ... 102 lines not shown
    if (!spread.empty()) fprintf(stderr, "raster timing: within a workgroup, last wave's end - first wave's end (us): mean %.1f p50 %.1f p90 %.1f max %.1f\n",
                                 std::accumulate(spread.begin(), spread.end(), 0.0) / spread.size(),
                                                 spread[spread.size() / 2], spread[spread.size() * 9 / 10], spread.back());
    {
        std::vector<std::pair<double, size_t>> byLife;
        for (size_t w = 0; w < (size_t)16384 * 4; ++w) { const unsigned long long *o = &h[w * 8]; if (o[0]) byLife.push_back({double(o[5] - o[4]) * 0.01, w}); }
        std::sort(byLife.begin(), byLife.end(), [](auto &a, auto &b) { return a.first > b.first; });
        for (size_t q = 0; q < std::min<size_t>(byLife.size(), 12); q += 1) {
            const size_t w = byLife[q].second; const unsigned long long *o = &h[w * 8];
            fprintf(stderr, "raster timing: long wave #%zu: life %.1f us (start +%.1f us), workgroup %zu of the launch, frame %llu, nVis %llu, classified "
                    "%llu, cycles prologue %llu cls %llu tiles %llu\n", q,
                    byLife[q].first, double(o[4] - r0) * 0.01, w / 4, o[7], o[6] & 0xffffffffull, o[6] >> 32, o[1] - o[0], o[2] - o[1], o[3] - o[2]);
        }
        const size_t nw = byLife.size();
        std::vector<double> sum(10, 0.0); std::vector<int> cnt(10, 0);
        size_t maxw = 0; for (auto &p : byLife) maxw = std::max(maxw, p.second);
        for (auto &p : byLife) { const int d = (int)std::min<size_t>(9, p.second * 10 / (maxw + 1)); sum[d] += p.first; ++cnt[d]; }
        fprintf(stderr, "raster timing: mean wave life by decile of the launch order (us):");
        for (int d = 0; d < 10; ++d) fprintf(stderr, " %.1f", cnt[d] ? sum[d] / cnt[d] : 0.0);
        fprintf(stderr, "  (%zu waves)\n", nw);
        {
            std::vector<double> pp(10, 0.0), pc(10, 0.0), pt(10, 0.0), ps(10, 0.0), pn(10, 0.0);
            for (auto &p : byLife) {
                const int d = (int)std::min<size_t>(9, p.second * 10 / (maxw + 1)); const unsigned long long *o = &h[p.second * 8];
                pp[d] += double(o[1] - o[0]); pc[d] += double(o[2] - o[1]); pt[d] += double(o[3] - o[2]);
                                ps[d] += double(o[4] - r0) * 0.01; pn[d] += double(o[6] & 0xffffffffull);
            }
            fprintf(stderr, "raster timing: by decile: prologue kcyc");
            for (int d = 0; d < 10; ++d) fprintf(stderr, " %.1f", cnt[d] ? pp[d] / cnt[d] / 1e3 : 0.0);
            fprintf(stderr, " | classification kcyc");
            for (int d = 0; d < 10; ++d) fprintf(stderr, " %.1f", cnt[d] ? pc[d] / cnt[d] / 1e3 : 0.0);
            fprintf(stderr, " | tiles kcyc");
            for (int d = 0; d < 10; ++d) fprintf(stderr, " %.1f", cnt[d] ? pt[d] / cnt[d] / 1e3 : 0.0);
            fprintf(stderr, " | start us");
            for (int d = 0; d < 10; ++d) fprintf(stderr, " %.1f", cnt[d] ? ps[d] / cnt[d] : 0.0);
            fprintf(stderr, " | nVis");
            for (int d = 0; d < 10; ++d) fprintf(stderr, " %.0f", cnt[d] ? pn[d] / cnt[d] : 0.0);
            fprintf(stderr, "\n");
        }
    }
    std::sort(life.begin(), life.end()); std::sort(endAt.begin(), endAt.end());
    auto pct = [](const std::vector<double> &v, double p) { return v[std::min(v.size() - 1, (size_t)(p * v.size()))]; };
    fprintf(stderr, "raster timing (last launch, %zu waves): cycles per wave: prologue %.0f, classification %.0f, tile loop %.0f | wave life us: mean %.1f "
            "p10 %.1f p50 %.1f p90 %.1f max %.1f | "
                    "launch %.1f us; waves ended by (us): 10%% %.1f, 25%% %.1f, 50%% %.1f, 75%% %.1f, 90%% %.1f, 99%% %.1f\n",
            n, sumP / n, sumC / n, sumT / n, std::accumulate(life.begin(), life.end(), 0.0) / life.size(),
                                                             pct(life, 0.1), pct(life, 0.5), pct(life, 0.9), life.back(),
            double(r1 - r0) * 0.01, pct(endAt, 0.1), pct(endAt, 0.25), pct(endAt, 0.5), pct(endAt, 0.75), pct(endAt, 0.9), pct(endAt, 0.99));
}
#endif

static void self_clear(struct FastArgs &fa, const GymView &gv, int workgroups);

static FastArgs fast_args_of(const GymView &gv, const PublishTo *publish)
{
    const int frames = gv.num_envs * gv.num_agents;
    FastArgs fa;
    fa.vis_hdr = gv.vis_hdr; fa.vis_prims = reinterpret_cast<const Prim *>(gv.vis_prims); fa.vis_rects = reinterpret_cast<const short4 *>(gv.vis_rects);
    fa.hist = gv.lpt_hist + gv.lpt_parity * (LPT_BUCKETS * LPT_SUBS); fa.list = gv.lpt_list; fa.num_agents = gv.num_agents;
                                             fa.vis_stride = gv.vis_stride; fa.frames = frames;
    fa.stage_rewards = gv.rewards; fa.stage_true = gv.true_objective; fa.stage_done = gv.done;
    fa.pub_rewards = publish ? publish->rewards : nullptr; fa.pub_true = publish ? publish->true_objective
            : nullptr; fa.pub_done = publish ? publish->done : nullptr;
    fa.pub_n = publish ? frames : 0;
    const char *pe = getenv("MV_PLANAR");
    fa.planar = pe && *pe ? atoi(pe) : 1;
    fa.tail_div = 0; fa.tail_split = 0;
    fa.hist_done = nullptr; fa.wg_total = 0;
#ifdef MV_RASTER_TIMING
    if (!g_rdbg && hipMalloc((void **)&g_rdbg, (size_t)(16384 * 4 * 8 + 64) * 8) == hipSuccess) { (void)hipMemset(g_rdbg,
        0, (size_t)(16384 * 4 * 8 + 64) * 8); atexit(rdbg_dump); }
    fa.rdbg = g_rdbg;
#endif
    return fa;
}

static void self_clear(FastArgs &fa, const GymView &gv, int workgroups)
{
    if (!gv.lpt_no_clear) return;
    fa.hist_done = gv.lpt_hist + (size_t)gv.lpt_hists * (LPT_BUCKETS * LPT_SUBS) + gv.lpt_parity;
    fa.wg_total = workgroups;
}

static int fast_pixels_per_lane(int W, int H, bool longList = false, bool batch = false)
{
    const char *e = getenv("MV_FAST_PPL");
    if (e && *e) return atoi(e) >= 2 ? 2 : 1;
    return (!longList || batch) && MV_FAST_PPL_DEFAULT >= 2 && W * H >= 8192 ? 2 : 1;
}

static int fast_split(int W, int H, int np, int frames, bool longList = false, bool batch = false)
{
    const int ftiles = ((W + TILE_W - 1) / TILE_W) * ((H + TILE_H * np - 1) / (TILE_H * np));
    const int want = ((np >= 2 ? 2048 : 4096) + frames - 1) / std::max(frames, 1), lo = (batch || frames >= 4096) && np >= 2
                      && !longList ? 1 : batch && !longList ? 1 : np >= 2 ? 2 : 4, hi = np >= 2 ? 8 : 16;
    int split = lo;
    while (split < hi && split < want) split <<= 1;
    while (split > 1 && ftiles < 4 * split * (longList ? 1 : 2)) split >>= 1;
    return split;
}

template <class K, class... A>
static void launch_done(K kernel, dim3 grid, dim3 block, size_t dyn, hipStream_t stream, hipEvent_t done, A... args)
{
    if (done) hipExtLaunchKernelGGL(kernel, grid, block, dyn, stream, nullptr, done, 0, args...);
    else hipLaunchKernelGGL(kernel, grid, block, dyn, stream, args...);
}

template <class Pick>
static auto by_layout(int layout, Pick pick)
{
    return layout == MV_OBS_RGB_PLANAR ? pick(std::true_type{}) : pick(std::false_type{});
}

int launch_raster_union(const GymView *views, uint32_t *const *obs, const PublishTo *publish, int n, int W,
                        int H, hipStream_t stream, hipEvent_t between, hipEvent_t done)
{
    if (W > MAX_W || H > MAX_H || n > MAX_UNION) return -1;
    const size_t dyn = (size_t)(W + H) * sizeof(float4) + (size_t)W * sizeof(float) + (size_t)H * sizeof(float2);
    const int np = fast_pixels_per_lane(W, H);
    const int layout = n > 0 ? views[0].obs_layout : MV_OBS_RGBA;
    int unionFrames[2] = {0, 0};
    for (int i = 0; i < n; ++i) unionFrames[views[i].vis_stride > VIS_SMALL ? 1 : 0] += views[i].num_envs * views[i].num_agents;
    if (between) (void)hipEventRecord(between, stream);
    if (unionFrames[0] > 0 && unionFrames[1] > 0) {
        UnionRasterAllArgs a;
        a.u.n = 0;
        a.split_small = fast_split(W, H, np, unionFrames[0] + unionFrames[1], false);
        a.split_large = fast_split(W, H, 1, unionFrames[0] + unionFrames[1], true);
        int wgs = 0;
        for (int large = 1; large >= 0; --large)
            for (int i = 0; i < n; ++i) {
                if ((views[i].vis_stride > VIS_SMALL) != (large != 0)) continue;
                a.u.first[a.u.n] = wgs;
                a.u.obs[a.u.n] = obs[i];
                a.u.fa[a.u.n] = fast_args_of(views[i], publish ? &publish[i] : nullptr);
                a.large[a.u.n] = large;
                wgs += views[i].num_envs * views[i].num_agents * (large ? a.split_large : a.split_small);
                ++a.u.n;
            }
        for (int i = a.u.n; i <= MAX_UNION; ++i) a.u.first[i] = wgs;
        for (int i = a.u.n; i < MAX_UNION; ++i) a.large[i] = 0;
        const auto fn = by_layout(layout, [&](auto chw) {
            return np == 2 ? raster_union_all_kernel<6, 2, decltype(chw)::value> : raster_union_all_kernel<7, 1, decltype(chw)::value>;
        });
        launch_done(fn, dim3(wgs), dim3(256), dyn, stream, done, a, W, H);
        return 0;
    }
    for (int large = 1; large >= 0; --large) {
        UnionRasterArgs ua;
        ua.n = 0;
        int wgs = 0;
        const int lnp = large ? fast_pixels_per_lane(W, H, true) : np;
        const int split = fast_split(W, H, lnp, unionFrames[large], large != 0);
        for (int i = 0; i < n; ++i) {
            const bool isLarge = views[i].vis_stride > VIS_SMALL;
            if (isLarge != (large != 0)) continue;
            ua.first[ua.n] = wgs;
            ua.obs[ua.n] = obs[i];
            ua.fa[ua.n] = fast_args_of(views[i], publish ? &publish[i] : nullptr);
            wgs += views[i].num_envs * views[i].num_agents * split;
            ++ua.n;
        }
        if (!ua.n) continue;
        for (int i = ua.n; i <= MAX_UNION; ++i) ua.first[i] = wgs;
        const auto fn = by_layout(layout, [&](auto chw) {
            constexpr bool C = decltype(chw)::value;
            return large ? (lnp == 2 ? raster_glist_union_kernel<VIS_XL, true, GLIST_WAVES_NP2, true, 2, C> : raster_glist_union_kernel<VIS_XL, true, GLIST_WAVES_NP1, true, 1, C>)
                         : (lnp == 2 ? raster_fast_union_kernel<VIS_SMALL, true, 6, false, 2, C> : raster_fast_union_kernel<VIS_SMALL, true, 8, false, 1, C>);
        });
        launch_done(fn, dim3(wgs), dim3(256), dyn, stream, nullptr, ua, W, H, split);
    }
    if (done) (void)hipEventRecord(done, stream);
    return 0;
}

bool raster_union_batch_applicable(int k, int n, int W, int H)
{
    static const int off = getenv("MV_RASTER_BATCH") && atoi(getenv("MV_RASTER_BATCH")) == 0;
    return !off && W <= MAX_W && H <= MAX_H && k >= 2 && k <= MAX_GROUP_TICKS && n >= 1 && n <= MAX_UNION;
}

int launch_raster_union_batch(const GymView *views, uint32_t *const *obs, const PublishTo *publish,
                              int k, int n, int W, int H, hipStream_t stream, hipEvent_t done)
{
    if (!raster_union_batch_applicable(k, n, W, H)) return 1;
    const size_t dyn = (size_t)(W + H) * sizeof(float4) + (size_t)W * sizeof(float) + (size_t)H * sizeof(float2);
    const int np = fast_pixels_per_lane(W, H);
    int unionFrames[2] = {0, 0};
    for (int i = 0; i < n; ++i) unionFrames[views[i].vis_stride > VIS_SMALL ? 1 : 0] += views[i].num_envs * views[i].num_agents;
    UnionBatchArgs a;
    std::memset(&a, 0, sizeof a);
    a.n = 0; a.k = k;
    a.split_small = fast_split(W, H, np, (unionFrames[0] + unionFrames[1]) * k, false, true);
    a.split_large = fast_split(W, H, 1, (unionFrames[0] + unionFrames[1]) * k, true, true);
    if (const char *e = getenv("MV_UNION_SPLIT_SMALL")) a.split_small = std::max(1, atoi(e));
    if (const char *e = getenv("MV_UNION_SPLIT_LARGE")) a.split_large = std::max(1, atoi(e));
    int wgs = 0;
    for (int large = 1; large >= 0; --large)
        for (int i = 0; i < n; ++i) {
            const GymView &v0 = views[i];
            if ((v0.vis_stride > VIS_SMALL) != (large != 0)) continue;
            const int q = a.n++;
            const int frames = v0.num_envs * v0.num_agents, split = large ? a.split_large : a.split_small;
            a.first[q] = wgs;
            a.large[q] = large;
            a.fa[q] = fast_args_of(v0, publish ? &publish[i] : nullptr);
            a.fa[q].wg_total = frames * split;
            a.hists[q] = v0.lpt_hists; a.parity0[q] = v0.lpt_parity;
            a.hist_base[q] = v0.lpt_hist;
            a.done_base[q] = v0.lpt_no_clear ? v0.lpt_hist + (size_t)v0.lpt_hists * (LPT_BUCKETS * LPT_SUBS) : nullptr;
            a.slot_stride[q] = k > 1 ? (int64_t)(reinterpret_cast<const unsigned char *>(views[n + i].vis_prims) - reinterpret_cast<const unsigned char *>(v0.vis_prims)) : 0;
            for (int j = 0; j < k; ++j) {
                const GymView &vj = views[(size_t)j * n + i], want = tick_view(v0, a.slot_stride[q], j);
                if (vj.vis_prims != want.vis_prims || vj.vis_hdr != want.vis_hdr || vj.lpt_list != want.lpt_list
                    || vj.rewards != want.rewards || vj.done != want.done ||
                    vj.true_objective != want.true_objective || vj.lpt_parity != want.lpt_parity || vj.lpt_no_clear != v0.lpt_no_clear)
                    return -2;
                a.obs[j][q] = obs[(size_t)j * n + i];
                a.pub_rewards[j][q] = publish ? publish[(size_t)j * n + i].rewards : nullptr;
                a.pub_done[j][q] = publish ? publish[(size_t)j * n + i].done : nullptr;
            }
            wgs += frames * split;
        }
    for (int i = a.n; i <= MAX_UNION; ++i) a.first[i] = wgs;
    a.per_tick = wgs;
    const auto fn = by_layout(views[0].obs_layout, [&](auto chw) {
        return np == 2 ? raster_union_batch_kernel<6, 2, decltype(chw)::value> : raster_union_batch_kernel<7, 1, decltype(chw)::value>;
    });
    launch_done(fn, dim3(wgs * k), dim3(256), dyn, stream, done, a, W, H);
    return 0;
}

int launch_raster_batch(const GymView *views, uint32_t *const *obs, const PublishTo *publish, int k, int W, int H, hipStream_t stream, hipEvent_t done)
{
    if (W > MAX_W || H > MAX_H || k < 2 || k > MAX_STEP_TICKS) return 1;
    const GymView &gv = views[0];
    static const int off = getenv("MV_RASTER_BATCH") && atoi(getenv("MV_RASTER_BATCH")) == 0;
    if (off) return 1;
    const size_t dyn = (size_t)(W + H) * sizeof(float4) + (size_t)W * sizeof(float) + (size_t)H * sizeof(float2);
    const int frames = gv.num_envs * gv.num_agents;
    const bool hexScen = gv.scenario == SCN_HEX_MEMORY || gv.scenario == SCN_HEX_EXPLORE, longList = gv.vis_stride > VIS_SMALL || hexScen;
    const int np = longList ? fast_pixels_per_lane(W, H, true, true) : fast_pixels_per_lane(W, H);
    const int split = fast_split(W, H, np, frames * k, longList, true);
    int64_t slotStride = 0;
    if (!slot_stride_of(views, k, slotStride)) return 1;
    TicksRasterArgs a;
    std::memset(&a, 0, sizeof a);
    a.k = k; a.per_tick = frames * split;
    a.hists = gv.lpt_hists; a.parity0 = gv.lpt_parity;
    a.slot_stride = slotStride;
    a.hist_base = gv.lpt_hist;
    a.done_base = gv.lpt_no_clear ? gv.lpt_hist + (size_t)gv.lpt_hists * (LPT_BUCKETS * LPT_SUBS) : nullptr;
    a.fa = fast_args_of(gv, publish ? &publish[0] : nullptr);
    a.fa.wg_total = frames * split;
    for (int j = 0; j < k; ++j) {
        a.obs[j] = obs[j];
        a.pub_rewards[j] = publish ? publish[j].rewards : nullptr;
        a.pub_done[j] = publish ? publish[j].done : nullptr;
    }
    const dim3 grid(k * frames * split), block(256);
    const bool shapes = gv.scenario == SCN_REARRANGE || gv.scenario == SCN_FOOTBALL;
    const auto fn = by_layout(gv.obs_layout, [&](auto chw) {
        constexpr bool C = decltype(chw)::value;
        if (longList)
            return np == 2 ? (hexScen ? raster_glist_batch_kernel<VIS_XL, true, GLIST_WAVES_NP2, true, 2, C> : raster_glist_batch_kernel<VIS_LARGE, false, GLIST_WAVES_NP2, false, 2, C>)
                           : (hexScen ? raster_glist_batch_kernel<VIS_XL, true, GLIST_WAVES_NP1, true, 1, C> : raster_glist_batch_kernel<VIS_LARGE, false, GLIST_WAVES_NP1, false, 1, C>);
        return np == 2 ? (shapes ? raster_fast_batch_kernel<VIS_SMALL, true, 6, 2, 256, C> : raster_fast_batch_kernel<VIS_SMALL, false, 7, 2, 256, C>)
                       : (shapes ? raster_fast_batch_kernel<VIS_SMALL, true, 8, 1, 256, C> : raster_fast_batch_kernel<VIS_SMALL, false, 8, 1, 256, C>);
    });
    launch_done(fn, grid, block, dyn, stream, done, a, W, H, split);
    return 0;
}

int launch_raster(const GymView &gv, uint32_t *obs, int W, int H, hipStream_t stream, hipEvent_t between,
                  int fast, int setup_done, const PublishTo *publish, hipEvent_t done)
{
    if (W > MAX_W || H > MAX_H) return -1;
    const int tiles = ((W + TILE_W - 1) / TILE_W) * ((H + TILE_H * PPL - 1) / (TILE_H * PPL));
    const int frames = gv.num_envs * gv.num_agents;
    if (!setup_done) hipLaunchKernelGGL(frame_setup_kernel, dim3(frames), dim3(256), 0, stream, gv, W, H);
    if (!fast) hipLaunchKernelGGL(frame_order_kernel, dim3(1), dim3(1024), 0, stream, gv, frames, gv.lpt_order);
    if (between) (void)hipEventRecord(between, stream);
    if (fast) {
        const size_t dyn = (size_t)(W + H) * sizeof(float4) + (size_t)W * sizeof(float) + (size_t)H * sizeof(float2);
        const int np = fast_pixels_per_lane(W, H, gv.vis_stride > VIS_SMALL);
        const int split = fast_split(W, H, np, frames, gv.vis_stride > VIS_SMALL);
        using KernelFn = void (*)(FastArgs, uint32_t *, int, int, int);
        FastArgs fa = fast_args_of(gv, publish);
        const bool hexScen = gv.scenario == SCN_HEX_MEMORY || gv.scenario == SCN_HEX_EXPLORE;
        const bool shapes = gv.scenario == SCN_REARRANGE || gv.scenario == SCN_FOOTBALL, large = gv.vis_stride > VIS_SMALL;
        const KernelFn fn = by_layout(gv.obs_layout, [&](auto chw) -> KernelFn {
            constexpr bool C = decltype(chw)::value;
            if (np == 2)
                return hexScen ? raster_glist_kernel<VIS_XL, true, GLIST_WAVES_NP2, true, 2, C> : large ? raster_glist_kernel<VIS_LARGE, false, GLIST_WAVES_NP2, false, 2, C>
                     : shapes ? raster_fast_kernel<VIS_SMALL, true, 6, false, 2, 256, C> : raster_fast_kernel<VIS_SMALL, false, 7, false, 2, 256, C>;
            return hexScen ? raster_glist_kernel<VIS_XL, true, GLIST_WAVES_NP1, true, 1, C> : large ? raster_glist_kernel<VIS_LARGE, false, GLIST_WAVES_NP1, false, 1, C>
                 : shapes ? raster_fast_kernel<VIS_SMALL, true, 8, false, 1, 256, C> : raster_fast_kernel<VIS_SMALL, false, 8, false, 1, 256, C>;
        });
        const int ftiles = ((W + TILE_W - 1) / TILE_W) * ((H + TILE_H * np - 1) / (TILE_H * np));
        constexpr int TAIL_DIV = 8, TAIL_SPLIT = 8;
        if (split <= 2 && gv.vis_stride <= VIS_SMALL && ftiles >= 16 * TAIL_SPLIT && tail_frames(frames, TAIL_DIV) > 0) {
            const int q = tail_frames(frames, TAIL_DIV);
            fa.tail_div = TAIL_DIV; fa.tail_split = TAIL_SPLIT;
            self_clear(fa, gv, (frames - q) * split + q * TAIL_SPLIT);
            launch_done(fn, dim3((frames - q) * split + q * TAIL_SPLIT), dim3(256), dyn, stream, done, fa, obs, W, H, split);
            return 0;
        }
        self_clear(fa, gv, frames * split);
        launch_done(fn, dim3(frames * split), dim3(256), dyn, stream, done, fa, obs, W, H, split);
        return 0;
    }
    const size_t dyn = (size_t)(W + H) * sizeof(float4) + (size_t)(W + H) * sizeof(float);
    int split = 4;
    while (split > 1 && tiles < 4 * split * 2) split >>= 1;
    const dim3 grid(frames * split), block(256);
    const bool hexScen = gv.scenario == SCN_HEX_MEMORY || gv.scenario == SCN_HEX_EXPLORE, shapes = gv.scenario == SCN_REARRANGE || gv.scenario == SCN_FOOTBALL;
    const auto fn = by_layout(gv.obs_layout, [&](auto chw) {
        constexpr bool C = decltype(chw)::value;
        return hexScen ? raster_kernel<VIS_XL, true, C> : gv.vis_stride > VIS_SMALL ? raster_kernel<VIS_LARGE, false, C>
             : shapes ? raster_kernel<VIS_SMALL, true, C> : raster_kernel<VIS_SMALL, false, C>;
    });
    launch_done(fn, grid, block, dyn, stream, nullptr, gv, obs, W, H, split, (const int *)gv.lpt_order);
    if (done) (void)hipEventRecord(done, stream);
    return 0;
}

}
```

### megaverse_amd/csrc/mv_types.h

```cpp
#pragma once
#include <hip/hip_runtime.h>
#include <stdint.h>

namespace mv {

enum : int {
    CX = 32, CY = 16, CZ = 32, CHUNK_BYTES = CX * CY * CZ,
    MAX_BOXES = 128,
    TOWER_BOXES = 16,
    MAX_OBJECTS = 80, MAX_AGENTS = 8, MAX_TERRAIN = 16, MAX_REWARDS = 16,
    NUM_SHAPING = 8,
    COLLECT_MAX_BOXES = 1024, COLLECT_MAX_REWARDS = 96, HM_DIM = 42, HM_BYTES = 1792,
    HEX_MAX_BOXES = 2048, HEX_MAX_OBJS = 128, HEX_FRAMES = 3,
    MAX_CAMS = MAX_AGENTS + HEX_FRAMES,
};

enum : int { FRAME_HDR_BYTES = 1024 };
enum : int { PIPE_GROUPS = 3, PIPE_BATCH_MAX = 16 };
enum : int { POLICY_NONE = 0, POLICY_MULTIDISCRETE = 1, POLICY_SINGLE_BIT = 2, POLICY_SEQUENCE = 3 };
__host__ __device__ inline uint32_t action_ring_entry(uint32_t first, int j, uint32_t count) { return (first + (uint32_t)j) % count; }

enum : int { ST_STARVED = 1, ST_CANDIDATES = 2, ST_VISIBLE = 4, ST_CHUNK = 8, ST_FORK = 32, ST_RESAMPLE = 64, ST_ENV_STORE = 128 };

enum : int { SCN_TOWER = 0, SCN_OBSTACLES = 1, SCN_COLLECT = 2, SCN_REARRANGE = 3, SCN_SOKOBAN = 4,
// ... 77 lines not shown
__host__ __device__ constexpr int lpt_sub_capacity(int frames) { return (frames + LPT_SUBS - 1) / LPT_SUBS; }


struct GymView {
    int32_t num_envs, num_agents;
    int32_t box_stride, reward_stride;
    int32_t scenario;
    int32_t env_offset, env_stride;
    int32_t sample_on;
    uint32_t sample_seed, sample_step;
    EnvHeader *hdr;
    LayoutBox *boxes;
    MovableObject *objects;
    AgentState *agents;
    uint8_t *chunk;
    TerrainBox *terrain;
    MovableObject *rewards_obj;
    int8_t *heightmap;
    ArrangementItem *items;
    uint8_t *soko_cells;
    HexRec *hex_boxes;
    HexRec *hex_objs;
    int32_t *episode_status;
    const void *blobs;
    int32_t spares;
    int32_t *actions;
    const int32_t *md_actions;
    float *rewards;
    uint8_t *done;
    float *true_objective;
    void *vis_prims;
    void *vis_rects;
    int32_t *vis_count;
    int32_t vis_stride;
    int32_t *lpt_bucket;
    int32_t *lpt_order;
    int32_t *lpt_hist;
    int32_t lpt_hists;
    int32_t *lpt_list;
    int32_t lpt_parity;
    uint8_t *vis_hdr;
    unsigned long long *dbg;
    int32_t debug_redo;
    int32_t obs_layout;
    uint8_t *sort_scratch;
    int32_t depth_sort;
    int32_t lpt_no_clear;
    struct TowerGen *tower_gen;
    struct BoxAGoneState *bag;
    struct FootballState *fb;
    const uint8_t *step_mask;
    int32_t *budget;
    uint32_t *halted;
};

struct StepTicksArgs8 {
    int32_t n, pad;
    GymView gv[8];
    __host__ __device__ const GymView &view(int j) const { return gv[j]; }
};
static_assert(sizeof(StepTicksArgs8) + 16 <= 4096, "StepTicksArgs8 + (W, H) must fit the 4 KB kernel-argument segment");

__host__ __device__ inline GymView tick_view(const GymView &base, int64_t slot_stride, int j)
{
    GymView v = base;
    const int64_t d = slot_stride * j;
    v.vis_prims = (uint8_t *)base.vis_prims + d;
    v.vis_rects = (uint8_t *)base.vis_rects + d;
    v.vis_count = (int32_t *)((uint8_t *)base.vis_count + d);
    v.lpt_bucket = (int32_t *)((uint8_t *)base.lpt_bucket + d);
    v.lpt_order = (int32_t *)((uint8_t *)base.lpt_order + d);
    v.vis_hdr = base.vis_hdr + d;
    v.lpt_list = (int32_t *)((uint8_t *)base.lpt_list + d);
    v.rewards = (float *)((uint8_t *)base.rewards + d);
    v.done = base.done + d;
    v.true_objective = (float *)((uint8_t *)base.true_objective + d);
    v.sample_step = base.sample_step + (uint32_t)j;
    v.lpt_parity = (base.lpt_parity + j) % base.lpt_hists;
    return v;
}
inline bool slot_stride_of(const GymView *views, int k, int64_t &stride)
{
    stride = k > 1 ? (int64_t)((const uint8_t *)views[1].vis_prims - (const uint8_t *)views[0].vis_prims) : 0;
    for (int j = 1; j < k; ++j) {
        const GymView w = tick_view(views[0], stride, j);
        if (views[j].vis_prims != w.vis_prims || views[j].vis_hdr != w.vis_hdr || views[j].lpt_list != w.lpt_list
            || views[j].rewards != w.rewards || views[j].done != w.done ||
            views[j].true_objective != w.true_objective || views[j].lpt_parity != w.lpt_parity || views[j].lpt_no_clear != w.lpt_no_clear)
            return false;
    }
    return true;
}

struct alignas(16) TowerBlob {
    int32_t seq;
    int32_t L, H, W;
    int32_t bz[4];
    int32_t layout_color, wall_color, draw_walls, num_objects;
    float bz_reward;
    int32_t pad[3];
    int32_t spawn[MAX_AGENTS];
    float yaw_rot[MAX_AGENTS];
    MovableObject objects[MAX_OBJECTS];
};
static_assert(sizeof(TowerBlob) == 448, "TowerBlob: 448 B");

struct alignas(16) TowerGen {
    uint32_t seed;
    int32_t seed_is_env_seed;
    int32_t generated;
    int32_t pad;
};

struct alignas(16) EpisodeBlob {
    int32_t seq;
    int32_t num_boxes, num_terrain, num_objects, num_rewards, num_platforms;
    int32_t layout_color, wall_color, draw_walls;
    int32_t dim[3], org[3];
    float episode_len;
    int32_t spawn[MAX_AGENTS][3];
    float yaw_frand[MAX_AGENTS];
    LayoutBox boxes[MAX_BOXES];
    TerrainBox terrain[MAX_TERRAIN];
    MovableObject objects[MAX_OBJECTS];
    MovableObject rewards[MAX_REWARDS];
};

struct alignas(16) RearrangeBlob {
    int32_t seq;
    int32_t num_boxes, num_items, max_matching, draw_walls;
    int32_t dim[3];
    float episode_len;
    int32_t pad[3];
    int32_t spawn[MAX_AGENTS][3];
    float yaw_frand[MAX_AGENTS];
    LayoutBox boxes[TOWER_BOXES];
    ArrangementItem items[MAX_ITEMS];
    MovableObject objects[MAX_ITEMS];
};

struct alignas(16) SokobanBlob {
// ... 102 lines not shown
```

### megaverse_amd/extension.py

```python
import ctypes as C
import os
import warnings

import numpy as np

from . import build as _build

_LIB = None


class _Config(C.Structure):
    _fields_ = [
        ("scenario", C.c_char_p), ("obs_width", C.c_int32), ("obs_height", C.c_int32), ("num_envs", C.c_int32),
        ("num_agents_per_env", C.c_int32), ("num_simulation_threads", C.c_int32), ("use_vulkan", C.c_int32),
        ("device", C.c_int32), ("param_keys", C.POINTER(C.c_char_p)), ("param_vals", C.POINTER(C.c_float)),
        ("num_params", C.c_int32), ("env_offset", C.c_int32), ("total_envs", C.c_int32), ("env_stride", C.c_int32),
    ]


_P, _I, _U, _F = C.c_void_p, C.c_int32, C.c_uint32, C.c_float
SYMBOLS = [
    ("mv_last_error", C.c_char_p, []), ("mv_device_count", C.c_int, []), ("mv_abi_version", C.c_int, []),
    ("mv_create", C.c_int, [C.POINTER(_Config), C.POINTER(_P)]),
    ("mv_close", C.c_int, [_P]), ("mv_destroy", C.c_int, [_P]),
# ... 13 lines not shown
    ("mv_debug_resample_plan_host", C.c_int, [_P, _I, _P, _P, _P]), ("mv_debug_resample_apply_host", C.c_int, [_P, _I, _I, _P, _I]),
    ("mv_env_record_bytes", C.c_int64, [_P]), ("mv_env_record_layout", C.c_uint64, [_P]),
    ("mv_save_envs", C.c_int, [_P, _P, _P, _I]), ("mv_save_envs_host", C.c_int, [_P, _P, _P, _I]),
    ("mv_load_envs", C.c_int, [_P, _P, _P, _I]), ("mv_load_envs_host", C.c_int, [_P, _P, _P, _I]),
    ("mv_debug_env_store_plan_host", C.c_int, [_P, _I, _I, _I, _P, _P]), ("mv_debug_env_record_layout_host", C.c_int64, [_P, _I, _I, _P]),
    ("mv_debug_env_record_pack_host", C.c_int, [_P, _I, _I, C.c_uint64, _I, _P, _P]),
    ("mv_debug_env_record_unpack_host", C.c_int, [_P, _I, _I, C.c_uint64, _I, _P, _P]),
    ("mv_reset_envs", C.c_int, [_P, _P, _I]), ("mv_reset_envs_host", C.c_int, [_P, _P, _I]), ("mv_debug_episode_log_cut_host", C.c_int, [_P, _I, _I, _P, _P]),
    ("mv_set_output_ring", C.c_int, [_P, _I, _P, _P, _P]),
    ("mv_set_pass_overlap", C.c_int, [_P, _I]),
    ("mv_recommended_ticks_per_call", C.c_int, [_P]), ("mv_recommended_pass_overlap", C.c_int, [_P]), ("mv_arena_bytes", C.c_int64, [_P]),
    ("mv_host_generator_threads", C.c_int, [_P]),
    ("mv_is_done", C.c_int, [_P, _I]), ("mv_get_dones", C.c_int, [_P, _P]),
    ("mv_get_last_rewards", C.c_int, [_P, _P]),
    ("mv_true_objective", C.c_int, [_P, _I, _I, C.POINTER(_F)]), ("mv_get_true_objectives", C.c_int, [_P, _P]),
    ("mv_get_observation", C.c_int, [_P, _I, _I, _P]),
    ("mv_obs_device_ptr", _P, [_P]), ("mv_rewards_device_ptr", _P, [_P]), ("mv_dones_device_ptr", _P, [_P]),
    ("mv_true_objectives_device_ptr", _P, [_P]),
    ("mv_set_obs_buffer", C.c_int, [_P, _P]), ("mv_set_stream", C.c_int, [_P, _P]),
    ("mv_set_pixel_mode", C.c_int, [_P, _I]), ("mv_get_pixel_mode", C.c_int, [_P]),
    ("mv_set_obs_layout", C.c_int, [_P, _I]), ("mv_get_obs_layout", C.c_int, [_P]),
    ("mv_set_render_resolution", C.c_int, [_P, _I, _I]), ("mv_draw_hires", C.c_int, [_P]),
    ("mv_get_hires_observation", C.c_int, [_P, _I, _I, _P]), ("mv_draw_overview", C.c_int, [_P]),
    ("mv_num_reward_shaping_keys", C.c_int, [_P]), ("mv_reward_shaping_key", C.c_char_p, [_P, _I]),
    ("mv_get_reward_shaping", C.c_int, [_P, _I, _I, C.c_char_p, C.POINTER(_F)]),
    ("mv_set_reward_shaping", C.c_int, [_P, _I, _I, C.c_char_p, _F]),
    ("mv_synchronize", C.c_int, [_P]),
    ("mv_profile_begin", C.c_int, [_P, _I]), ("mv_profile_end", C.c_int, [_P, _P, _P]),
    ("mv_set_pipelining", C.c_int, [_P, _I]), ("mv_get_pipelining", C.c_int, [_P]),
    ("mv_debug_set_agent_pos", C.c_int, [_P, _I, _I, _F, _F, _F]),
    ("mv_debug_set_agent_yaw", C.c_int, [_P, _I, _I, _F, _F]), ("mv_debug_set_agent_velocity", C.c_int, [_P, _I, _I, _F, _F, _F]),
    ("mv_debug_snapshot_size", C.c_int, [_P]), ("mv_debug_snapshot", C.c_int, [_P, _I, _P]),
    ("mv_debug_boxagone_state", C.c_int, [_P, _I, _P]),
    ("mv_debug_football_state", C.c_int, [_P, _I, _P]), ("mv_debug_set_football_state", C.c_int, [_P, _I, _P]),
    ("mv_debug_rng", C.c_int, [_I, _U, _I, _P, _P, _I, _P]),
    ("mv_debug_math", C.c_int, [_I, _I, _P, _P, _I, _P]),
    ("mv_debug_generate_episode", C.c_int, [C.c_char_p, _I, _I, _I, _F, _P, _I]),
    ("mv_debug_feeder_selftest", C.c_int, [C.c_char_p, _I, _I, _I, _I]),
    ("mv_debug_generate_sokoban", C.c_int, [_I, _I, _I, _F, _P, _I]),
    ("mv_debug_generate_football", C.c_int, [_I, _I, _I, _F, _P, _I]),
    ("mv_debug_collect_draw_host", C.c_int, [_I, _I, _I, _F, _P, _I]),
    ("mv_debug_collect_draw_device", C.c_int, [_I, _I, _P, _I, _I, _F, _P, C.c_int64, _P]),
    ("mv_set_episode_log", C.c_int, [_P, _I]), ("mv_get_episode_log_capacity", C.c_int, [_P]), ("mv_flush_episode_log", C.c_int, [_P]),
    ("mv_episode_log_count", C.c_int, [_P, C.POINTER(_U), C.POINTER(_U)]), ("mv_drain_episode_log", C.c_int, [_P, _P, _I, C.POINTER(_U)]),
    ("mv_episode_log_records_device_ptr", _P, [_P]), ("mv_episode_log_count_device_ptr", _P, [_P]),
    ("mv_episode_returns_device_ptr", _P, [_P]), ("mv_episode_lengths_device_ptr", _P, [_P]), ("mv_ticks_since_reset", C.c_int64, [_P]),
    ("mv_debug_episode_log_host", C.c_int, [_P, _P, _P, _I, _I, _I, _I, _U, _P, _P, _P, C.POINTER(_U), C.POINTER(_U)]),
    ("mv_set_step_mask", C.c_int, [_P, _P]), ("mv_set_step_mask_host", C.c_int, [_P, _P]), ("mv_get_step_mask", C.c_int, [_P]),
    ("mv_debug_episode_log_masked_host", C.c_int, [_P, _P, _P, _I, _I, _I, _I, _U, _P, _P, _P, C.POINTER(_U), C.POINTER(_U), _P]),
    ("mv_set_episode_budget", C.c_int, [_P, _P]), ("mv_set_episode_budget_host", C.c_int, [_P, _P]), ("mv_get_episode_budget", C.c_int, [_P]),
    ("mv_episode_budget_device_ptr", _P, [_P]), ("mv_halted_count_device_ptr", _P, [_P]), ("mv_halted_count", C.c_int, [_P, C.POINTER(_I)]),
    ("mv_debug_episode_log_budget_host", C.c_int, [_P, _P, _P, _I, _I, _I, _I, _U, _P, _P, _P, C.POINTER(_U), C.POINTER(_U), _P, _P]),
    ("mv_debug_episode_budget_host", C.c_int, [_P, _P, _P, _I, _I, _P, _P]),
]

EPISODE_RECORD_DTYPE = np.dtype({"names": ["agent", "length", "end_tick", "true_objective", "ret"],
                                 "formats": ["<i4", "<i4", "<u4", "<f4", "<f8"], "offsets": [0, 4, 8, 12, 16], "itemsize": 24})


class _DeviceArray:

    def __init__(self, ptr, shape, typestr):
        self.__cuda_array_interface__ = {"shape": tuple(shape), "typestr": typestr, "data": (int(ptr), False), "version": 2, "strides": None}


def debug_episode_log_host(rewards, dones, true_objectives, agents_per_env, capacity, first_tick=0, state=None):
    return _episode_log_host(False, None, rewards, dones, true_objectives, agents_per_env, capacity, first_tick, state)


def debug_episode_log_masked_host(step_mask, rewards, dones, true_objectives, agents_per_env, capacity, first_tick=0, state=None):
    return _episode_log_host(True, step_mask, rewards, dones, true_objectives, agents_per_env, capacity, first_tick, state)


def debug_episode_log_budget_host(step_mask, left, rewards, dones, true_objectives, agents_per_env, capacity, first_tick=0, state=None):
    if left is not None and not (isinstance(left, np.ndarray) and left.dtype == np.int32 and left.flags.c_contiguous and left.ndim == 1):
        raise ValueError("debug_episode_log_budget_host: left is a contiguous int32 numpy array [N], advanced in place")
    return _episode_log_host(True, step_mask, rewards, dones, true_objectives, agents_per_env, capacity, first_tick, state, budget=(left,))


def debug_episode_budget_host(dones, mask, left):
    lib = load_library()
    dones = np.ascontiguousarray(dones, np.uint8)
    k, N = dones.shape
    left = np.ascontiguousarray(left, np.int32).reshape(-1)
    m = None if mask is None else np.ascontiguousarray(mask, np.uint8).reshape(-1)
    if left.size != N or (m is not None and m.size != N):
        raise ValueError("debug_episode_budget_host: dones is [k][N], mask and left are [N]")
    steps, out = np.full((k, N), 9, np.uint8), np.full(N, -9, np.int32)
    if lib.mv_debug_episode_budget_host(dones.ctypes.data, None if m is None else m.ctypes.data, left.ctypes.data, k, N, steps.ctypes.data, out.ctypes.data) != 0:
        raise RuntimeError(lib.mv_last_error().decode())
    return steps, out


def _episode_log_host(masked, step_mask, rewards, dones, true_objectives, agents_per_env, capacity, first_tick, state, budget=None):
    lib = load_library()
    rewards = np.ascontiguousarray(rewards, np.float32)
    dones = np.ascontiguousarray(dones, np.uint8)
    true_objectives = np.ascontiguousarray(true_objectives, np.float32)
    k, N = dones.shape
    A = int(agents_per_env)
    if rewards.shape != (k, N * A) or true_objectives.shape != (k, N * A):
        raise ValueError("debug_episode_log_host: rewards and true_objectives are [k][N*A], dones [k][N]")
    if state is None:
        state = {"ret": np.zeros(N * A, np.float64), "len": np.zeros(N, np.int32), "records": np.zeros(max(int(capacity), 0), EPISODE_RECORD_DTYPE),
                 "count": 0, "dropped": 0}
    count, dropped = _U(state["count"]), _U(state["dropped"])
# ... 692 lines not shown
```

Baseline: 28.81 million.

## Precompute frame order, ray table and raster constants; specialize whole-tile kernels

Adds a separate kernel that builds each tick's LPT frame order once from the histograms, so raster workgroups read their frame index directly instead of each rescanning the histogram. It also uploads a per-column and per-row ray direction table, passes precomputed projection constants, replaces several divisions with shifts or magic multiplies, and adds template variants that drop edge clamping when the image divides evenly into tiles. These aim to cut per-workgroup prologue work in the raster kernels. The cost is an extra kernel launch per step batch, more arena memory, and new debug entry points.

```diff
diff --git a/include/megaverse_hip.h b/include/megaverse_hip.h
--- a/include/megaverse_hip.h
+++ b/include/megaverse_hip.h
@@ -157,6 +157,8 @@
 int mv_debug_set_football_state(mv_gym *g, int32_t env_idx, const void *in_host);
 int mv_debug_rng(int32_t device, uint32_t seed, int32_t what, const int32_t *lo, const int32_t *hi, int32_t n, void *out_host);
 int mv_debug_math(int32_t device, int32_t what, const float *a, const float *b, int32_t n, float *out_host);
+int mv_debug_raster_consts_host(int32_t W, int32_t H, float *consts, uint32_t *tiles_x_inv, float *dcx, float *dcy);
+int mv_debug_raster_div_host(uint32_t d, uint32_t n_end, uint32_t *magic, uint32_t *q);
 int mv_debug_generate_episode(const char *scenario, int32_t num_agents, int32_t env_seed, int32_t n, float base_episode_len,
                               void *out, int32_t out_bytes);
 int mv_debug_feeder_selftest(const char *scenario, int32_t num_envs, int32_t num_agents, int32_t threads, int32_t rounds);
diff --git a/megaverse_amd/csrc/mv_api.hip b/megaverse_amd/csrc/mv_api.hip
--- a/megaverse_amd/csrc/mv_api.hip
+++ b/megaverse_amd/csrc/mv_api.hip
@@ -354,7 +354,9 @@
     const size_t szVisP = up(NA * (size_t)gv.vis_stride * 32), szVisR = up(NA * (size_t)gv.vis_stride * 8), szVisC = up(NA * sizeof(int32_t)),
                  szLpt = up(NA * sizeof(int32_t)) + up((NA + 1) * sizeof(int32_t)) + up(NA * (size_t)FRAME_HDR_BYTES)
                             + up((size_t)LPT_BUCKETS * LPT_SUBS * lpt_sub_capacity(NA) * sizeof(int32_t));
-    const size_t szParity = szVisP + szVisR + szVisC + szLpt + szRew + szDone + szObjv;
+    const bool frameOrderOn = !(getenv("MV_FRAME_ORDER") && atoi(getenv("MV_FRAME_ORDER")) == 0);
+    const size_t szFOrder = frameOrderOn ? up(NA * sizeof(int32_t)) : 0;
+    const size_t szParity = szVisP + szVisR + szVisC + szLpt + szRew + szDone + szObjv + szFOrder;
     g->batch = (size_t)PIPE_GROUPS * 16 * szParity <= (size_t(9) << 28) ? 16 : 8;
     if (const char *e = getenv("MV_PIPE_BATCH")) g->batch = std::min((int)PIPE_BATCH_MAX, std::max(1, atoi(e)));
     g->slots = PIPE_GROUPS * g->batch;
@@ -367,8 +369,10 @@
     gv.lpt_hists = g->hists;
     const bool depthSortOn = !(getenv("MV_DEPTH_SORT") && atoi(getenv("MV_DEPTH_SORT")) == 0);
     const size_t szSort = gv.vis_stride > 256 && depthSortOn ? up(NA * (size_t)gv.vis_stride * 40) : 0;
+    const bool rayTabOn = !(getenv("MV_RAY_TABLE") && atoi(getenv("MV_RAY_TABLE")) == 0);
+    const size_t szRay = rayTabOn ? up((size_t)(g->w + g->h) * sizeof(float)) : 0;
     const size_t total = szSort + szHdr + szBoxes + szObj + szAg + szAct + szRew + szDone + szObjv + szMd + (hostEpisodes ? 0 : szChunk) + szObs + szTerrain +
-                         szRewObj + szHeight + szItems + szCells + szHexB + szHexO + szBag + szFb + szBlobs + szCnt + szGen + (size_t)g->slots * szParity + szHist;
+                         szRewObj + szHeight + szItems + szCells + szHexB + szHexO + szBag + szFb + szBlobs + szCnt + szGen + (size_t)g->slots * szParity + szHist + szRay;
     {
         hipError_t e_ = hipMalloc((void **)&g->arena, total);
         if (e_ != hipSuccess) {
@@ -429,6 +433,14 @@
         }
         gv.lpt_hist = (int32_t *)p; p += szHist;
         gv.sort_scratch = szSort ? p : nullptr; p += szSort;
+        if (szRay) {
+            std::vector<float> tab((size_t)(g->w + g->h));
+            raster_ray_table(g->w, g->h, tab.data());
+            hipError_t e_ = hipMemcpy(p, tab.data(), tab.size() * sizeof(float), hipMemcpyHostToDevice);
+            if (e_ != hipSuccess) { mv_destroy(g); return fail(std::string("mv_create: ray table upload: ") + hipGetErrorString(e_)); }
+            gv.ray_tab = (const float *)p; gv.ray_w = g->w; gv.ray_h = g->h;
+            p += szRay;
+        }
         gv.depth_sort = 0;
         for (int q = 0; q < g->slots; ++q) {
             GymView &v = g->gvp[q];
@@ -443,6 +455,7 @@
             v.rewards = (float *)p; p += szRew;
             v.done = p; p += szDone;
             v.true_objective = (float *)p; p += szObjv;
+            v.lpt_forder = szFOrder ? (int32_t *)p : nullptr; p += szFOrder;
         }
     }
     if (getenv("MV_TICK_TIMING") && atoi(getenv("MV_TICK_TIMING"))) {
diff --git a/megaverse_amd/csrc/mv_api_debug.hip b/megaverse_amd/csrc/mv_api_debug.hip
--- a/megaverse_amd/csrc/mv_api_debug.hip
+++ b/megaverse_amd/csrc/mv_api_debug.hip
@@ -402,4 +402,28 @@
     return 0;
 }
 
-}
+int mv_debug_raster_consts_host(int32_t W, int32_t H, float *consts, uint32_t *tiles_x_inv, float *dcx, float *dcy)
+{
+    if (W < 1 || H < 1 || W > 1024 || H > 1024) return fail("mv_debug_raster_consts_host: size must be within 1..1024");
+    const RasterConsts rc = raster_launch_consts(W, H);
+    if (consts) { consts[0] = rc.sx; consts[1] = rc.ox; consts[2] = rc.sy; consts[3] = rc.oy; }
+    if (tiles_x_inv) *tiles_x_inv = rc.tiles_x_inv;
+    if (dcx && dcy) {
+        std::vector<float> tab((size_t)(W + H));
+        raster_ray_table(W, H, tab.data());
+        std::memcpy(dcx, tab.data(), (size_t)W * sizeof(float));
+        std::memcpy(dcy, tab.data() + W, (size_t)H * sizeof(float));
+    }
+    return 0;
+}
+
+int mv_debug_raster_div_host(uint32_t d, uint32_t n_end, uint32_t *magic, uint32_t *q)
+{
+    if (d < 1) return fail("mv_debug_raster_div_host: d >= 1");
+    const uint32_t m = raster_div_magic(d);
+    if (magic) *magic = m;
+    if (q) for (uint32_t n = 0; n < n_end; ++n) q[n] = raster_div_by_magic(n, m);
+    return 0;
+}
+
+}
diff --git a/megaverse_amd/csrc/mv_api_step.hip b/megaverse_amd/csrc/mv_api_step.hip
--- a/megaverse_amd/csrc/mv_api_step.hip
+++ b/megaverse_amd/csrc/mv_api_step.hip
@@ -127,14 +127,16 @@
             if (j == k - 1) {
                 if (callEv) HIP_TRY(hipEventRecord(callEv[0], sim));
                 hipEvent_t rides = own && !callEv ? L->simDone : nullptr;
+                const bool frameOrder = allFast && views[0].lpt_forder != nullptr;
                 const int chunkTicks = 8;
                 for (int j0 = 0; j0 < k; j0 += chunkTicks) {
                     const int kk = std::min(chunkTicks, k - j0);
                     const GymView *vw = views.data() + j0;
-                    hipEvent_t r = j0 + kk == k ? rides : nullptr;
+                    hipEvent_t r = j0 + kk == k && !frameOrder ? rides : nullptr;
                     launch_step_ticks(vw, kk, sim, L->w, L->h, r);
                     ++L->launchCount[0];
                 }
+                if (frameOrder) launch_frame_order_ticks(views.data(), k, sim, rides);
                 if (callEv) HIP_TRY(hipEventRecord(callEv[1], sim));
                 simDoneRides = rides != nullptr;
             }
diff --git a/megaverse_amd/csrc/mv_raster.h b/megaverse_amd/csrc/mv_raster.h
--- a/megaverse_amd/csrc/mv_raster.h
+++ b/megaverse_amd/csrc/mv_raster.h
@@ -20,4 +20,12 @@
 int launch_raster_union_batch(const GymView *views, uint32_t *const *obs, const PublishTo *publish, int k,
                               int n, int W, int H, hipStream_t stream, hipEvent_t done = nullptr);
 
+void launch_frame_order_ticks(GymView *views, int k, hipStream_t stream, hipEvent_t done = nullptr);
+
+struct RasterConsts { float sx, ox, sy, oy; uint32_t tiles_x_inv; };
+RasterConsts raster_launch_consts(int W, int H);
+void raster_ray_table(int W, int H, float *out);
+inline uint32_t raster_div_magic(uint32_t d) { return d <= 1u ? 0u : (uint32_t)((0x100000000ull + d - 1u) / d); }
+inline uint32_t raster_div_by_magic(uint32_t n, uint32_t m) { return m ? (uint32_t)(((uint64_t)n * m) >> 32) : n; }
+
 }
diff --git a/megaverse_amd/csrc/mv_raster.hip b/megaverse_amd/csrc/mv_raster.hip
--- a/megaverse_amd/csrc/mv_raster.hip
+++ b/megaverse_amd/csrc/mv_raster.hip
@@ -244,16 +244,84 @@
     for (int f = tid; f < frames; f += 1024) order[atomicAdd(&s_start[gv.lpt_bucket[f]], 1)] = f;
 }
 
+struct FrameOrderTicksArgs {
+    int32_t k, frames;
+    int32_t *hist[MAX_STEP_TICKS];
+    const int32_t *list[MAX_STEP_TICKS];
+    int32_t *order[MAX_STEP_TICKS];
+};
+
+__global__ __launch_bounds__(LPT_BUCKETS) void frame_order_ticks_kernel(FrameOrderTicksArgs a)
+{
+    static_assert(LPT_SUBS == 4 && LPT_BUCKETS == 256, "one thread per bin, its counters as one int4");
+    constexpr int ENDS = LPT_BUCKETS * LPT_SUBS;
+    __shared__ int s_end[ENDS], s_wsum[LPT_BUCKETS / 64];
+    const int t = (int)blockIdx.x;
+    if (t >= a.k) return;
+    int32_t *hist = a.hist[t];
+    const int32_t *list = a.list[t];
+    int32_t *order = a.order[t];
+    const int tid = threadIdx.x, lane = tid & 63, wave = tid >> 6;
+    const int4 c0 = *reinterpret_cast<const int4 *>(hist + (LPT_BUCKETS - 1 - tid) * LPT_SUBS);
+    const int h = (c0.x + c0.y) + (c0.z + c0.w);
+    int x = h;
+#pragma unroll
+    for (int off = 1; off < 64; off <<= 1) {
+        const int y = __shfl_up(x, off, 64);
+        if (lane >= off) x += y;
+    }
+    if (lane == 63) s_wsum[wave] = x;
+    __syncthreads();
+    int base = 0;
+    for (int w = 0; w < wave; ++w) base += s_wsum[w];
+    const int start = base + x - h;
+    s_end[4 * tid] = start + c0.x;
+    s_end[4 * tid + 1] = start + c0.x + c0.y;
+    s_end[4 * tid + 2] = start + c0.x + c0.y + c0.z;
+    s_end[4 * tid + 3] = start + h;
+    __syncthreads();
+    const int total = min(s_end[ENDS - 1], a.frames), cap = lpt_sub_capacity(a.frames);
+    for (int pos = tid; pos < total; pos += LPT_BUCKETS) {
+        int lo = 0, hi = ENDS - 1;
+        while (lo < hi) {
+            const int mid = (lo + hi) >> 1;
+            if (s_end[mid] > pos) hi = mid; else lo = mid + 1;
+        }
+        const int off = pos - (lo ? s_end[lo - 1] : 0), bin = LPT_BUCKETS - 1 - (lo >> 2), sub = lo & 3;
+        order[pos] = off < cap ? list[(size_t)(bin * LPT_SUBS + sub) * cap + off] : 0;
+    }
+    for (int pos = total + tid; pos < a.frames; pos += LPT_BUCKETS) order[pos] = 0;
+    for (int i = tid; i < ENDS; i += LPT_BUCKETS) hist[i] = 0;
+}
+
+void launch_frame_order_ticks(GymView *views, int k, hipStream_t stream, hipEvent_t done)
+{
+    FrameOrderTicksArgs a;
+    std::memset(&a, 0, sizeof a);
+    a.k = k; a.frames = views[0].num_envs * views[0].num_agents;
+    for (int j = 0; j < k; ++j) {
+        a.hist[j] = views[j].lpt_hist + (size_t)views[j].lpt_parity * (LPT_BUCKETS * LPT_SUBS);
+        a.list[j] = views[j].lpt_list;
+        a.order[j] = views[j].lpt_forder;
+        views[j].lpt_forder_on = 1;
+    }
+    if (done) hipExtLaunchKernelGGL(frame_order_ticks_kernel, dim3(k), dim3(LPT_BUCKETS), 0, stream, nullptr, done, 0, a);
+    else hipLaunchKernelGGL(frame_order_ticks_kernel, dim3(k), dim3(LPT_BUCKETS), 0, stream, a);
+}
+
 namespace {
 
-template <bool CHW>
+template <bool CHW, bool WHOLE = false>
 struct PixOutT {
+    static constexpr bool whole = WHOLE;
     __amdgpu_buffer_rsrc_t rsrc;
     int W, H, W4;
     bool edgeless;
     int plane;
 };
 typedef PixOutT<false> PixOut;
+template <class PO> __device__ __forceinline__ int col_in(const PO &po, int px) { return PO::whole ? px : min(px, po.W - 1); }
+template <class PO> __device__ __forceinline__ int row_in(const PO &po, int py) { return PO::whole ? py : min(py, po.H - 1); }
 #ifndef MV_PIXEL_PLAIN
 constexpr int PIXEL_AUX = 2;
 #else
@@ -276,10 +344,11 @@
     return po;
 }
 
-__device__ __forceinline__ void put_px(const PixOut &po, int px, int py, unsigned rgba)
+template <bool WHOLE>
+__device__ __forceinline__ void put_px(const PixOutT<false, WHOLE> &po, int px, int py, unsigned rgba)
 {
     const unsigned off = (unsigned)(__mul24(py, po.W4) + px * 4);
-    if (__builtin_expect(po.edgeless, 1)) __builtin_amdgcn_raw_buffer_store_b32(rgba, po.rsrc, off, 0, PIXEL_AUX);
+    if (WHOLE || __builtin_expect(po.edgeless, 1)) __builtin_amdgcn_raw_buffer_store_b32(rgba, po.rsrc, off, 0, PIXEL_AUX);
     else {
         asm volatile("" ::: "memory");
         if (px < po.W && py < po.H) __builtin_amdgcn_raw_buffer_store_b32(rgba, po.rsrc, off, 0, PIXEL_AUX);
@@ -572,6 +641,10 @@
     int wg_total;
     int tail_div, tail_split;
     int planar;
+    float sx, ox, sy, oy;
+    unsigned tilesXinv;
+    const float *ray_tab;
+    const int *order;
 };
 
 __device__ __forceinline__ void fast_publish(const FastArgs &fa, int blk)
@@ -584,6 +657,8 @@
     if (fa.stage_done[e]) fa.pub_true[i] = fa.stage_true[i];
     if (i < fa.pub_n / fa.num_agents) fa.pub_done[i] = fa.stage_done[i];
 }
+
+__device__ __forceinline__ unsigned div_magic(unsigned n, unsigned m) { return m ? __umulhi(n, m) : n; }
 
 __device__ __forceinline__ unsigned long long uniform_u64(unsigned long long v)
 {
@@ -776,12 +851,17 @@
             if (b < split * head) frames = head;
             else { b -= split * head; first = head; split = fa.tail_split; frames = q; }
         }
-        const int per = 8 * split, group = b / per, r = b - group * per;
+        const int per = 8 * split, group = b >> (__ffs(per) - 1), r = b - group * per;
         position = group * 8 + (r & 7); part = r >> 3;
         if (group * 8 + 8 > frames) { const int nf = frames - group * 8; position = group * 8 + r % nf; part = r / nf; }
         position += first;
     }
     __shared__ int s_wsum[4], s_frame, s_lastWG;
+    int frame;
+    if (fa.order) {
+        frame = __builtin_amdgcn_readfirstlane(fa.order[position]);
+        if (tid == 0) s_lastWG = 0;
+    } else {
     {
         static_assert(LPT_SUBS == 4, "the bin's counters are read as one int4");
         const bool binThread = NT == 256 || tid < LPT_BUCKETS;
@@ -813,8 +893,9 @@
 #else
     if (tid == 0) s_lastWG = fa.hist_done != nullptr && __hip_atomic_fetch_add(fa.hist_done, 1, __ATOMIC_RELAXED, __HIP_MEMORY_SCOPE_AGENT) == fa.wg_total - 1;
 #endif
-    const int frame = __builtin_amdgcn_readfirstlane(s_frame);
-    const int viewer = frame % A;
+    frame = __builtin_amdgcn_readfirstlane(s_frame);
+    }
+    const int viewer = A == 1 ? 0 : frame % A;
     const float *gh = reinterpret_cast<const float *>(fa.vis_hdr + (size_t)frame * FRAME_HDR_BYTES);
     const int nVis = __builtin_amdgcn_readfirstlane(min(__float_as_int(gh[FH_COUNT]), (int)MAXVIS));
 
@@ -831,15 +912,18 @@
         const short4 *rs = fa.vis_rects + (size_t)frame * fa.vis_stride;
         for (int i = tid; i < nVis; i += NT) s_rect[i] = rs[i];
         const float *c = gh + FH_CAM + FH_CAM_STRIDE * viewer + 3;
-        for (int i = tid; i < W; i += NT) {
-            const float dcx = (((float(i) + 0.5f) / float(W)) * 2.0f - 1.0f) * TAN_HALF_FOV;
-            s_col[i] = make_float4(dcx, c[0] * dcx, c[3] * dcx, c[6] * dcx);
-            s_colq[i] = dcx * dcx;
-        }
-        for (int j = tid; j < H; j += NT) {
-            const float dcy = (((float(j) + 0.5f) / float(H)) * 2.0f - 1.0f) * TAN_HALF_FOV_Y;
+        const float *rt = fa.ray_tab;
+        const auto col = [&](int i, float dcx) { s_col[i] = make_float4(dcx, c[0] * dcx, c[3] * dcx, c[6] * dcx); s_colq[i] = dcx * dcx; };
+        const auto row = [&](int j, float dcy) {
             s_row[j] = make_float4(dcy, c[1] * dcy, c[4] * dcy, c[7] * dcy);
             s_rowq[j] = make_float2(dcy * dcy + 1.0f, 4.0f * dcy - 2.0f);
+        };
+        if (rt) {
+            for (int i = tid; i < W; i += NT) col(i, rt[i]);
+            for (int j = tid; j < H; j += NT) row(j, rt[W + j]);
+        } else {
+            for (int i = tid; i < W; i += NT) col(i, (((float(i) + 0.5f) / float(W)) * 2.0f - 1.0f) * TAN_HALF_FOV);
+            for (int j = tid; j < H; j += NT) row(j, (((float(j) + 0.5f) / float(H)) * 2.0f - 1.0f) * TAN_HALF_FOV_Y);
         }
     }
     __syncthreads();
@@ -894,8 +978,8 @@
 enum : unsigned { TC_EMPTY = 0, TC_PLANAR = 1, TC_PLANAR_SPEC = 2, TC_OVERLAY = 3, TC_GENERAL = 4 };
 constexpr int CLS_MAX_TILES = 128;
 
-template <int TH, int NT>
-__device__ __forceinline__ void classify_tiles(uint4 *s_tile, float4 *s_line, const float4 *s_vis, const short4 *s_rect,
+template <int TH, int NT, bool WHOLE = false>
+__device__ __forceinline__ void classify_tiles(const FastArgs &fa, uint4 *s_tile, float4 *s_line, const float4 *s_vis, const short4 *s_rect,
                                                const float *s_hdr, const float *camv, int nVis, unsigned long long wb0,
                                                int W, int H, int part, int split, int tilesX, int numTiles,
                                                        int perWG, bool overlayOn, int *s_cnt, unsigned *s_txy, bool bulkClear)
@@ -905,8 +989,7 @@
     const int tid = threadIdx.x, lane = tid & 63, wave = __builtin_amdgcn_readfirstlane(tid >> 6);
     if (tid < CLS_MAX_TILES) s_tile[tid] = make_uint4(0u, 0u, 0u, 0u);
     if (tid < 8) s_cnt[tid] = 0;
-    const float sx = 2.0f * TAN_HALF_FOV / float(W), ox = (1.0f / float(W) - 1.0f) * TAN_HALF_FOV;
-    const float sy = 2.0f * TAN_HALF_FOV_Y / float(H), oy = (1.0f / float(H) - 1.0f) * TAN_HALF_FOV_Y;
+    const float sx = fa.sx, ox = fa.ox, sy = fa.sy, oy = fa.oy;
     const int q = lane & 15, es = lane >> 4;
     const int ek = min(q >> 2, 2);
     int em = ek + 1 + ((q >> 1) & 1);
@@ -926,9 +1009,9 @@
         const int u = 64 * c + lane;
         const int tile = ((u >> 2) * split + part) * 4 + (u & 3);
         tvalid[c] = u < perWG && tile < numTiles;
-        const int tyi = tile / tilesX, txi = tile - tyi * tilesX;
+        const int tyi = (int)div_magic((unsigned)tile, fa.tilesXinv), txi = tile - tyi * tilesX;
         tX0[c] = txi * TILE_W; tY0[c] = tyi * TH;
-        tX1[c] = min(tX0[c] + TILE_W, W) - 1; tY1[c] = min(tY0[c] + TH, H) - 1;
+        tX1[c] = (WHOLE ? tX0[c] + TILE_W : min(tX0[c] + TILE_W, W)) - 1; tY1[c] = (WHOLE ? tY0[c] + TH : min(tY0[c] + TH, H)) - 1;
         mlo[c] = mhi[c] = cover[c] = 0u;
     }
     for (int base = PPR * wave; base < nVis; base += 16) {
@@ -1080,7 +1163,6 @@
 __device__ __forceinline__ void planar_run(int pos, int k, int n, const float4 *s_vis, const float *s_hdr, const float4 *s_col, const float4 *s_row,
                                            const float2 *s_rowq, const float *s_colq, float nzk, int tx0, int ty0, int lane, const PO &po)
 {
-    const int W = po.W, H = po.H;
     const float lok = uniform_f32(reinterpret_cast<const float *>(s_vis)[8 * pos + k]),
                                   hik = uniform_f32(reinterpret_cast<const float *>(s_vis)[8 * pos + 4 + k]);
     const float plane = lok > 0.0f ? lok : hik;
@@ -1095,13 +1177,13 @@
     float2 rq[NP];
 #pragma unroll
     for (int j = 0; j < NP; ++j) {
-        const int pyc = min(py0 + TILE_H * j, H - 1);
+        const int pyc = row_in(po, py0 + TILE_H * j);
         rowk[j] = reinterpret_cast<const float *>(s_row)[4 * pyc + 1 + k];
         rq[j] = s_rowq[pyc];
     }
 #pragma unroll 1
     for (int q = 0; q < n; ++q) {
-        const int px = tx0 + TILE_W * q + lx, pxc = min(px, W - 1);
+        const int px = tx0 + TILE_W * q + lx, pxc = col_in(po, px);
         const float colk = reinterpret_cast<const float *>(s_col)[4 * pxc + 1 + k];
         const float cq = s_colq[pxc];
 #pragma unroll
@@ -1119,7 +1201,6 @@
 __device__ __forceinline__ void planar_tile(int pos, int k, const float4 *s_vis, const float *s_hdr, const float4 *s_col, const float4 *s_row,
                                             const float2 *s_rowq, const float *s_colq, float nzk, int px, int py0, const PO &po)
 {
-    const int W = po.W, H = po.H;
     const float lok = uniform_f32(reinterpret_cast<const float *>(s_vis)[8 * pos + k]),
                                   hik = uniform_f32(reinterpret_cast<const float *>(s_vis)[8 * pos + 4 + k]);
     const float plane = lok > 0.0f ? lok : hik;
@@ -1127,12 +1208,12 @@
     const float cr = float((color >> 16) & 255u), cg = float((color >> 8) & 255u), cb = float(color & 255u);
     const float lk = uniform_f32(s_hdr[FH_LREL + k]);
     const float lks = plane > 0.0f ? lk : 0.0f - lk;
-    const int pxc = min(px, W - 1);
+    const int pxc = col_in(po, px);
     const float colk = reinterpret_cast<const float *>(s_col)[4 * pxc + 1 + k];
     const float cq = s_colq[pxc];
 #pragma unroll
     for (int j = 0; j < NP; ++j) {
-        const int py = py0 + TILE_H * j, pyc = min(py, H - 1);
+        const int py = py0 + TILE_H * j, pyc = row_in(po, py);
         const float rowk = reinterpret_cast<const float *>(s_row)[4 * pyc + 1 + k];
         const float2 rq = s_rowq[pyc];
         const float dk = (colk + rowk) + nzk;
@@ -1144,16 +1225,16 @@
 }
 
 typedef unsigned v4u_t __attribute__((ext_vector_type(4)));
-template <int NP>
-__device__ __forceinline__ void clear_tile(const PixOut &po, int tx0, int ty0, int lane)
+template <int NP, bool WHOLE>
+__device__ __forceinline__ void clear_tile(const PixOutT<false, WHOLE> &po, int tx0, int ty0, int lane)
 {
     constexpr int TH = TILE_H * NP;
     unsigned c = 0xff000000u;
     asm volatile("" : "+v"(lane), "+v"(c));
-    if ((po.W & 3) == 0 && tx0 + TILE_W <= po.W) {
+    if (WHOLE || ((po.W & 3) == 0 && tx0 + TILE_W <= po.W)) {
         const int row = ty0 + (lane >> 2), col = tx0 + 4 * (lane & 3);
         const v4u_t v = {c, c, c, c};
-        if (lane < 4 * TH && row < po.H) __builtin_amdgcn_raw_buffer_store_b128(v, po.rsrc, (unsigned)(__mul24(row, po.W4) + col * 4), 0, PIXEL_AUX);
+        if (lane < 4 * TH && (WHOLE || row < po.H)) __builtin_amdgcn_raw_buffer_store_b128(v, po.rsrc, (unsigned)(__mul24(row, po.W4) + col * 4), 0, PIXEL_AUX);
         return;
     }
     const int px = tx0 + (lane & (TILE_W - 1)), py0 = ty0 + lane / TILE_W;
@@ -1185,7 +1266,6 @@
                                              const float4 *s_row, const float2 *s_rowq, const float *s_colq,
                                                      float nzm0, float nzm1, float nzm2, int px, int py0, const PO &po)
 {
-    const int W = po.W, H = po.H;
     const float lok = uniform_f32(reinterpret_cast<const float *>(s_vis)[8 * posA + k]),
                                   hik = uniform_f32(reinterpret_cast<const float *>(s_vis)[8 * posA + 4 + k]);
     const float plane = lok > 0.0f ? lok : hik;
@@ -1193,12 +1273,12 @@
     const float cr = float((color >> 16) & 255u), cg = float((color >> 8) & 255u), cb = float(color & 255u);
     const float lk = uniform_f32(s_hdr[FH_LREL + k]);
     const float lks = plane > 0.0f ? lk : 0.0f - lk;
-    const int pxc = min(px, W - 1);
+    const int pxc = col_in(po, px);
     const float4 cx = s_col[pxc];
     const float cq = s_colq[pxc];
 #pragma unroll
     for (int j = 0; j < NP; ++j) {
-        const int py = py0 + TILE_H * j, pyc = min(py, H - 1);
+        const int py = py0 + TILE_H * j, pyc = row_in(po, py);
         const float4 ry = s_row[pyc];
         const float2 rq = s_rowq[pyc];
         const V3 dw = v3((cx.y + ry.y) + nzm0, (cx.z + ry.z) + nzm1, (cx.w + ry.w) + nzm2);
@@ -1232,8 +1312,7 @@
                                              const float4 *s_row, const float2 *s_rowq, const float *s_colq,
                                                      float nzm0, float nzm1, float nzm2, int px, int py0, const PO &po)
 {
-    const int W = po.W, H = po.H;
-    const int pxc = min(px, W - 1);
+    const int pxc = col_in(po, px);
     const float4 cx = s_col[pxc];
     const float cq = s_colq[pxc];
     const float dcx = cx.x;
@@ -1242,7 +1321,7 @@
     unsigned best[NP];
 #pragma unroll
     for (int j = 0; j < NP; ++j) {
-        const int pyc = min(py0 + TILE_H * j, H - 1);
+        const int pyc = row_in(po, py0 + TILE_H * j);
         const float4 ry = s_row[pyc];
         const float2 rq = s_rowq[pyc];
         dcy[j] = ry.x;
@@ -1348,7 +1427,7 @@
                                        viewer, s_col, s_row, s_rowq, s_colq, nzm0, nzm1, nzm2, px, py0, po);
 }
 
-template <int MAXVIS, bool SHAPES, bool HEXF, int NP, bool CLS = true, int NT = 256, bool CHW = false>
+template <int MAXVIS, bool SHAPES, bool HEXF, int NP, bool CLS = true, int NT = 256, bool CHW = false, bool WHOLE = false>
 __device__ __forceinline__ void raster_fast_body(const FastArgs &fa, uint32_t *obs, int W, int H, int split, int blk, unsigned char *lds)
 {
     constexpr unsigned POS_MASK = MAXVIS - 1;
@@ -1383,12 +1462,13 @@
     uint32_t *out = obs + (size_t)frame * W * H;
     const int tilesX = (W + TILE_W - 1) / TILE_W, tilesY = (H + TH - 1) / TH;
     const int numTiles = tilesX * tilesY;
-    PixOutT<CHW> po;
+    static_assert(!(CHW && WHOLE), "the whole-tile variants are RGBA");
+    PixOutT<CHW, WHOLE> po;
     if constexpr (CHW) po = frame_out<true>(obs, frame, W, H, (W % TILE_W) == 0 && (H % TH) == 0);
     else {
         po.rsrc = __builtin_amdgcn_make_buffer_rsrc(out,  0, W * H * 4, 0x00020000);
         po.W = W; po.H = H; po.W4 = 4 * W;
-        po.edgeless = (W % TILE_W) == 0 && (H % TH) == 0;
+        po.edgeless = WHOLE || ((W % TILE_W) == 0 && (H % TH) == 0);
     }
 
     uint2 rr0 = make_uint2(0u, 0u);
@@ -1399,7 +1479,7 @@
     static_assert(!PLANAR || (MAXVIS == 256 && CLS_MAX_TILES == 128), "classification tables: 256 edge functions + 128 tiles = 192 records");
     float4 *s_line = s_vis + 2 * 64;
     uint4 *s_tile = reinterpret_cast<uint4 *>(s_vis + 2 * 64 + 256);
-    const int perWG = (numTiles - part * 4 + 4 * split - 1) / (4 * split) * 4;
+    const int perWG = ((numTiles - part * 4 + 4 * split - 1) >> (__ffs(4 * split) - 1)) * 4;
     const bool cls = PLANAR && fa.planar && nVis <= 64 && perWG <= CLS_MAX_TILES && perWG >= 32;
     __shared__ int s_next;
     __shared__ int s_cnt[8];
@@ -1411,11 +1491,11 @@
 #define MV_TILE_LIST 1
 #endif
     constexpr bool LISTED = PLANAR && MV_TILE_LIST != 0;
-    const bool bulk = LISTED && po.edgeless && (W & 3) == 0;
-    if (PLANAR && cls && !LISTED) classify_tiles<TH, NT>(s_tile, s_line, s_vis, s_rect, s_hdr, camv, nVis, wb0, W, H,
+    const bool bulk = LISTED && (WHOLE || (po.edgeless && (W & 3) == 0));
+    if (PLANAR && cls && !LISTED) classify_tiles<TH, NT, WHOLE>(fa, s_tile, s_line, s_vis, s_rect, s_hdr, camv, nVis, wb0, W, H,
         part, split, tilesX, numTiles, perWG, fa.planar != 2, s_cnt, s_txy, true);
     else if (PLANAR && cls) {
-        classify_tiles<TH, NT>(s_tile, s_line, s_vis, s_rect, s_hdr, camv, nVis, wb0, W, H, part, split,
+        classify_tiles<TH, NT, WHOLE>(fa, s_tile, s_line, s_vis, s_rect, s_hdr, camv, nVis, wb0, W, H, part, split,
                                tilesX, numTiles, perWG, fa.planar != 2, s_cnt, s_txy, bulk);
         const int c0 = s_cnt[0], c1 = s_cnt[1], c2 = s_cnt[2], c3 = s_cnt[3], nE = s_cnt[4];
         nList = __builtin_amdgcn_readfirstlane(c0 + c1 + c2 + c3 + (bulk ? 0 : nE));
@@ -1469,14 +1549,14 @@
             classified_tile<SHAPES, POS_MASK, NP, LISTED>(fa, u, (int)(txy & 0xffffu), (int)(txy >> 16), s_tile, s_vis, s_hdr,
                                                           camv, viewer, s_col, s_row, s_rowq, s_colq, nzm0, nzm1, nzm2, wb0, lane, po);
         }
-    const unsigned tilesXinv = (unsigned)((0x100000000ull + (unsigned)tilesX - 1u) / (unsigned)tilesX);
+    const unsigned tilesXinv = fa.tilesXinv;
     for (int u = wave; !(LISTED && cls); u = __builtin_amdgcn_readfirstlane(unext)) {
         const int tile = ((u >> 2) * split + part) * 4 + (u & 3);
         if (tile >= numTiles) break;
         if (lane == 0) unext = atomicAdd(&s_next, 1);
-        const int ty = (int)__umulhi((unsigned)tile, tilesXinv), tx = tile - ty * tilesX;
+        const int ty = (int)div_magic((unsigned)tile, tilesXinv), tx = tile - ty * tilesX;
         const int tx0 = tx * TILE_W, ty0 = ty * TH;
-        const int tx1 = min(tx0 + TILE_W, W) - 1, ty1 = min(ty0 + TH, H) - 1;
+        const int tx1 = (WHOLE ? tx0 + TILE_W : min(tx0 + TILE_W, W)) - 1, ty1 = (WHOLE ? ty0 + TH : min(ty0 + TH, H)) - 1;
         if (PLANAR && !LISTED && cls) {
             classified_tile<SHAPES, POS_MASK, NP, LISTED>(fa, u, tx0, ty0, s_tile, s_vis, s_hdr, camv, viewer,
                                                           s_col, s_row, s_rowq, s_colq, nzm0, nzm1, nzm2, wb0, lane, po);
@@ -1486,7 +1566,7 @@
         int lpx = lane;
         asm volatile("" : "+v"(lpx));
         const int px = tx0 + (lpx & (TILE_W - 1)), py0 = ty0 + lpx / TILE_W;
-        const int pxc = min(px, W - 1);
+        const int pxc = col_in(po, px);
         {
             int l2 = lane;
             asm volatile("" : "+v"(l2));
@@ -1532,7 +1612,7 @@
                 dcx = cx.x;
 #pragma unroll
                 for (int j = 0; j < NP; ++j) {
-                    const int pyc = min(py0 + TILE_H * j, H - 1);
+                    const int pyc = row_in(po, py0 + TILE_H * j);
                     const float4 ry = s_row[pyc];
                     const float2 rq = s_rowq[pyc];
                     dcy[j] = ry.x;
@@ -1844,11 +1924,11 @@
     raster_glist_body<MAXVIS, SHAPES, HEXF, NP, CHW>(fa, obs, W, H, split, (int)blockIdx.x, s_buf);
 }
 
-template <int MAXVIS, bool SHAPES, int WAVES, bool HEXF = false, int NP = 1, int NT = 256, bool CHW = false>
+template <int MAXVIS, bool SHAPES, int WAVES, bool HEXF = false, int NP = 1, int NT = 256, bool CHW = false, bool WHOLE = false>
 __global__ __launch_bounds__(NT, WAVES) void raster_fast_kernel(FastArgs fa, uint32_t *obs, int W, int H, int split)
 {
     __shared__ __attribute__((aligned(16))) unsigned char s_buf[fast_lds_bytes(MAXVIS)];
-    raster_fast_body<MAXVIS, SHAPES, HEXF, NP, true, NT, CHW>(fa, obs, W, H, split, (int)blockIdx.x, s_buf);
+    raster_fast_body<MAXVIS, SHAPES, HEXF, NP, true, NT, CHW, WHOLE>(fa, obs, W, H, split, (int)blockIdx.x, s_buf);
 }
 
 struct UnionRasterArgs {
@@ -1889,10 +1969,12 @@
     f.vis_prims = reinterpret_cast<const Prim *>(reinterpret_cast<const unsigned char *>(f.vis_prims) + d);
     f.vis_rects = reinterpret_cast<const short4 *>(reinterpret_cast<const unsigned char *>(f.vis_rects) + d);
     f.list = reinterpret_cast<const int *>(reinterpret_cast<const unsigned char *>(f.list) + d);
+    if (f.order) f.order = reinterpret_cast<const int *>(reinterpret_cast<const unsigned char *>(f.order) + d);
     f.stage_rewards = reinterpret_cast<const float *>(reinterpret_cast<const unsigned char *>(f.stage_rewards) + d);
     f.stage_true = reinterpret_cast<const float *>(reinterpret_cast<const unsigned char *>(f.stage_true) + d);
     f.stage_done += d;
-    const int par = (a.parity0 + t) % a.hists;
+    int par = a.parity0 + t;
+    while (par >= a.hists) par -= a.hists;
     f.hist = a.hist_base + par * (LPT_BUCKETS * LPT_SUBS);
     f.hist_done = a.done_base ? a.done_base + par : nullptr;
     f.pub_rewards = a.pub_rewards[t];
@@ -1900,7 +1982,7 @@
     return f;
 }
 
-template <int MAXVIS, bool SHAPES, int WAVES, int NP, int NT = 256, bool CHW = false>
+template <int MAXVIS, bool SHAPES, int WAVES, int NP, int NT = 256, bool CHW = false, bool WHOLE = false>
 __global__ __launch_bounds__(NT, WAVES) void raster_fast_batch_kernel(TicksRasterArgs a, int W, int H, int split)
 {
     int j = 0, r = (int)blockIdx.x;
@@ -1910,7 +1992,7 @@
     __shared__ __attribute__((aligned(16))) unsigned char s_buf[fast_lds_bytes(MAXVIS)];
     FastArgs fa = ticks_raster_args(a, j);
     fa.pub_n = 0;
-    raster_fast_body<MAXVIS, SHAPES, false, NP, true, NT, CHW>(fa, a.obs[j], W, H, split, r, s_buf);
+    raster_fast_body<MAXVIS, SHAPES, false, NP, true, NT, CHW, WHOLE>(fa, a.obs[j], W, H, split, r, s_buf);
 }
 
 template <int MAXVIS, bool SHAPES, int WAVES, bool HEXF, int NP, bool CHW = false>
@@ -2119,7 +2201,22 @@
 
 static void self_clear(struct FastArgs &fa, const GymView &gv, int workgroups);
 
-static FastArgs fast_args_of(const GymView &gv, const PublishTo *publish)
+RasterConsts raster_launch_consts(int W, int H)
+{
+    RasterConsts c;
+    c.sx = 2.0f * TAN_HALF_FOV / float(W); c.ox = (1.0f / float(W) - 1.0f) * TAN_HALF_FOV;
+    c.sy = 2.0f * TAN_HALF_FOV_Y / float(H); c.oy = (1.0f / float(H) - 1.0f) * TAN_HALF_FOV_Y;
+    c.tiles_x_inv = raster_div_magic((uint32_t)((W + TILE_W - 1) / TILE_W));
+    return c;
+}
+
+void raster_ray_table(int W, int H, float *out)
+{
+    for (int i = 0; i < W; ++i) out[i] = (((float(i) + 0.5f) / float(W)) * 2.0f - 1.0f) * TAN_HALF_FOV;
+    for (int j = 0; j < H; ++j) out[W + j] = (((float(j) + 0.5f) / float(H)) * 2.0f - 1.0f) * TAN_HALF_FOV_Y;
+}
+
+static FastArgs fast_args_of(const GymView &gv, const PublishTo *publish, int W, int H)
 {
     const int frames = gv.num_envs * gv.num_agents;
     FastArgs fa;
@@ -2134,6 +2231,10 @@
     fa.planar = pe && *pe ? atoi(pe) : 1;
     fa.tail_div = 0; fa.tail_split = 0;
     fa.hist_done = nullptr; fa.wg_total = 0;
+    const RasterConsts rc = raster_launch_consts(W, H);
+    fa.sx = rc.sx; fa.ox = rc.ox; fa.sy = rc.sy; fa.oy = rc.oy; fa.tilesXinv = rc.tiles_x_inv;
+    fa.ray_tab = gv.ray_tab && gv.ray_w == W && gv.ray_h == H ? gv.ray_tab : nullptr;
+    fa.order = gv.lpt_forder_on ? gv.lpt_forder : nullptr;
 #ifdef MV_RASTER_TIMING
     if (!g_rdbg && hipMalloc((void **)&g_rdbg, (size_t)(16384 * 4 * 8 + 64) * 8) == hipSuccess) { (void)hipMemset(g_rdbg,
         0, (size_t)(16384 * 4 * 8 + 64) * 8); atexit(rdbg_dump); }
@@ -2144,10 +2245,14 @@
 
 static void self_clear(FastArgs &fa, const GymView &gv, int workgroups)
 {
-    if (!gv.lpt_no_clear) return;
+    if (!gv.lpt_no_clear || fa.order) return;
     fa.hist_done = gv.lpt_hist + (size_t)gv.lpt_hists * (LPT_BUCKETS * LPT_SUBS) + gv.lpt_parity;
     fa.wg_total = workgroups;
 }
+
+static bool pow2_split(int split) { return split >= 1 && (split & (split - 1)) == 0; }
+
+static bool whole_tiles(int W, int H, int np) { return W % TILE_W == 0 && H % (TILE_H * np) == 0; }
 
 static int fast_pixels_per_lane(int W, int H, bool longList = false, bool batch = false)
 {
@@ -2164,6 +2269,7 @@
     int split = lo;
     while (split < hi && split < want) split <<= 1;
     while (split > 1 && ftiles < 4 * split * (longList ? 1 : 2)) split >>= 1;
+    if (!pow2_split(split)) split = 1;
     return split;
 }
 
@@ -2201,7 +2307,7 @@
                 if ((views[i].vis_stride > VIS_SMALL) != (large != 0)) continue;
                 a.u.first[a.u.n] = wgs;
                 a.u.obs[a.u.n] = obs[i];
-                a.u.fa[a.u.n] = fast_args_of(views[i], publish ? &publish[i] : nullptr);
+                a.u.fa[a.u.n] = fast_args_of(views[i], publish ? &publish[i] : nullptr, W, H);
                 a.large[a.u.n] = large;
                 wgs += views[i].num_envs * views[i].num_agents * (large ? a.split_large : a.split_small);
                 ++a.u.n;
@@ -2225,7 +2331,7 @@
             if (isLarge != (large != 0)) continue;
             ua.first[ua.n] = wgs;
             ua.obs[ua.n] = obs[i];
-            ua.fa[ua.n] = fast_args_of(views[i], publish ? &publish[i] : nullptr);
+            ua.fa[ua.n] = fast_args_of(views[i], publish ? &publish[i] : nullptr, W, H);
             wgs += views[i].num_envs * views[i].num_agents * split;
             ++ua.n;
         }
@@ -2272,7 +2378,7 @@
             const int frames = v0.num_envs * v0.num_agents, split = large ? a.split_large : a.split_small;
             a.first[q] = wgs;
             a.large[q] = large;
-            a.fa[q] = fast_args_of(v0, publish ? &publish[i] : nullptr);
+            a.fa[q] = fast_args_of(v0, publish ? &publish[i] : nullptr, W, H);
             a.fa[q].wg_total = frames * split;
             a.hists[q] = v0.lpt_hists; a.parity0[q] = v0.lpt_parity;
             a.hist_base[q] = v0.lpt_hist;
@@ -2318,8 +2424,9 @@
     a.hists = gv.lpt_hists; a.parity0 = gv.lpt_parity;
     a.slot_stride = slotStride;
     a.hist_base = gv.lpt_hist;
-    a.done_base = gv.lpt_no_clear ? gv.lpt_hist + (size_t)gv.lpt_hists * (LPT_BUCKETS * LPT_SUBS) : nullptr;
-    a.fa = fast_args_of(gv, publish ? &publish[0] : nullptr);
+    if (gv.lpt_hists < 1 || gv.lpt_parity < 0 || gv.lpt_parity >= gv.lpt_hists || !pow2_split(split)) return 1;
+    a.fa = fast_args_of(gv, publish ? &publish[0] : nullptr, W, H);
+    a.done_base = gv.lpt_no_clear && !a.fa.order ? gv.lpt_hist + (size_t)gv.lpt_hists * (LPT_BUCKETS * LPT_SUBS) : nullptr;
     a.fa.wg_total = frames * split;
     for (int j = 0; j < k; ++j) {
         a.obs[j] = obs[j];
@@ -2333,6 +2440,10 @@
         if (longList)
             return np == 2 ? (hexScen ? raster_glist_batch_kernel<VIS_XL, true, GLIST_WAVES_NP2, true, 2, C> : raster_glist_batch_kernel<VIS_LARGE, false, GLIST_WAVES_NP2, false, 2, C>)
                            : (hexScen ? raster_glist_batch_kernel<VIS_XL, true, GLIST_WAVES_NP1, true, 1, C> : raster_glist_batch_kernel<VIS_LARGE, false, GLIST_WAVES_NP1, false, 1, C>);
+        if constexpr (!C)
+            if (whole_tiles(W, H, np))
+                return np == 2 ? (shapes ? raster_fast_batch_kernel<VIS_SMALL, true, 6, 2, 256, false, true> : raster_fast_batch_kernel<VIS_SMALL, false, 7, 2, 256, false, true>)
+                               : (shapes ? raster_fast_batch_kernel<VIS_SMALL, true, 8, 1, 256, false, true> : raster_fast_batch_kernel<VIS_SMALL, false, 8, 1, 256, false, true>);
         return np == 2 ? (shapes ? raster_fast_batch_kernel<VIS_SMALL, true, 6, 2, 256, C> : raster_fast_batch_kernel<VIS_SMALL, false, 7, 2, 256, C>)
                        : (shapes ? raster_fast_batch_kernel<VIS_SMALL, true, 8, 1, 256, C> : raster_fast_batch_kernel<VIS_SMALL, false, 8, 1, 256, C>);
     });
@@ -2354,11 +2465,15 @@
         const int np = fast_pixels_per_lane(W, H, gv.vis_stride > VIS_SMALL);
         const int split = fast_split(W, H, np, frames, gv.vis_stride > VIS_SMALL);
         using KernelFn = void (*)(FastArgs, uint32_t *, int, int, int);
-        FastArgs fa = fast_args_of(gv, publish);
+        FastArgs fa = fast_args_of(gv, publish, W, H);
         const bool hexScen = gv.scenario == SCN_HEX_MEMORY || gv.scenario == SCN_HEX_EXPLORE;
         const bool shapes = gv.scenario == SCN_REARRANGE || gv.scenario == SCN_FOOTBALL, large = gv.vis_stride > VIS_SMALL;
         const KernelFn fn = by_layout(gv.obs_layout, [&](auto chw) -> KernelFn {
             constexpr bool C = decltype(chw)::value;
+            if constexpr (!C)
+                if (!hexScen && !large && whole_tiles(W, H, np))
+                    return np == 2 ? (shapes ? raster_fast_kernel<VIS_SMALL, true, 6, false, 2, 256, false, true> : raster_fast_kernel<VIS_SMALL, false, 7, false, 2, 256, false, true>)
+                                   : (shapes ? raster_fast_kernel<VIS_SMALL, true, 8, false, 1, 256, false, true> : raster_fast_kernel<VIS_SMALL, false, 8, false, 1, 256, false, true>);
             if (np == 2)
                 return hexScen ? raster_glist_kernel<VIS_XL, true, GLIST_WAVES_NP2, true, 2, C> : large ? raster_glist_kernel<VIS_LARGE, false, GLIST_WAVES_NP2, false, 2, C>
                      : shapes ? raster_fast_kernel<VIS_SMALL, true, 6, false, 2, 256, C> : raster_fast_kernel<VIS_SMALL, false, 7, false, 2, 256, C>;
@@ -2367,6 +2482,7 @@
         });
         const int ftiles = ((W + TILE_W - 1) / TILE_W) * ((H + TILE_H * np - 1) / (TILE_H * np));
         constexpr int TAIL_DIV = 8, TAIL_SPLIT = 8;
+        static_assert((TAIL_SPLIT & (TAIL_SPLIT - 1)) == 0, "fast_prologue: b / (8 split) is a shift");
         if (split <= 2 && gv.vis_stride <= VIS_SMALL && ftiles >= 16 * TAIL_SPLIT && tail_frames(frames, TAIL_DIV) > 0) {
             const int q = tail_frames(frames, TAIL_DIV);
             fa.tail_div = TAIL_DIV; fa.tail_split = TAIL_SPLIT;
diff --git a/megaverse_amd/csrc/mv_types.h b/megaverse_amd/csrc/mv_types.h
--- a/megaverse_amd/csrc/mv_types.h
+++ b/megaverse_amd/csrc/mv_types.h
@@ -153,6 +153,10 @@
     const uint8_t *step_mask;
     int32_t *budget;
     uint32_t *halted;
+    const float *ray_tab;
+    int32_t ray_w, ray_h;
+    int32_t *lpt_forder;
+    int32_t lpt_forder_on;
 };
 
 struct StepTicksArgs8 {
@@ -173,6 +177,7 @@
     v.lpt_order = (int32_t *)((uint8_t *)base.lpt_order + d);
     v.vis_hdr = base.vis_hdr + d;
     v.lpt_list = (int32_t *)((uint8_t *)base.lpt_list + d);
+    v.lpt_forder = base.lpt_forder ? (int32_t *)((uint8_t *)base.lpt_forder + d) : nullptr;
     v.rewards = (float *)((uint8_t *)base.rewards + d);
     v.done = base.done + d;
     v.true_objective = (float *)((uint8_t *)base.true_objective + d);
@@ -187,7 +192,8 @@
         const GymView w = tick_view(views[0], stride, j);
         if (views[j].vis_prims != w.vis_prims || views[j].vis_hdr != w.vis_hdr || views[j].lpt_list != w.lpt_list
             || views[j].rewards != w.rewards || views[j].done != w.done ||
-            views[j].true_objective != w.true_objective || views[j].lpt_parity != w.lpt_parity || views[j].lpt_no_clear != w.lpt_no_clear)
+            views[j].true_objective != w.true_objective || views[j].lpt_parity != w.lpt_parity || views[j].lpt_no_clear != w.lpt_no_clear
+            || views[j].lpt_forder != w.lpt_forder || views[j].lpt_forder_on != w.lpt_forder_on)
             return false;
     }
     return true;
diff --git a/megaverse_amd/extension.py b/megaverse_amd/extension.py
--- a/megaverse_amd/extension.py
+++ b/megaverse_amd/extension.py
@@ -89,6 +89,7 @@
     ("mv_episode_budget_device_ptr", _P, [_P]), ("mv_halted_count_device_ptr", _P, [_P]), ("mv_halted_count", C.c_int, [_P, C.POINTER(_I)]),
     ("mv_debug_episode_log_budget_host", C.c_int, [_P, _P, _P, _I, _I, _I, _I, _U, _P, _P, _P, C.POINTER(_U), C.POINTER(_U), _P, _P]),
     ("mv_debug_episode_budget_host", C.c_int, [_P, _P, _P, _I, _I, _P, _P]),
+    ("mv_debug_raster_consts_host", C.c_int, [_I, _I, _P, _P, _P, _P]), ("mv_debug_raster_div_host", C.c_int, [_U, _U, _P, _P]),
 ]
 
 EPISODE_RECORD_DTYPE = np.dtype({"names": ["agent", "length", "end_tick", "true_objective", "ret"],
```

Measured after the change: 30.02 million, median of 6. 1.04x the previous value.
